# shanghong/Multiband-RF-pulse-Design

Measured on AMD Instinct MI355X. Metric: FIR designs/sec, n=512 taps m=16384 arbitrary-phase SOCP (fir_ap_cvx form), higher is better.
Workload: dtype f64

## Files before the change

### multiband-rf-pulse-design_amd/csrc/solver.hip

```cpp
#include "dev_common.h"
#include <functional>
#include <mutex>
#include <thread>
#include "cone_dev.h"
#include "dd_dev.h"
#include "program.h"
#include "solver.h"
#include <algorithm>
#include <chrono>
#include <cmath>
#include <cstdlib>
#include <cstring>
#include <vector>

#include <dlfcn.h>
#include <rccl/rccl.h>

namespace mbfir {

struct RcclApi {
    ncclResult_t (*GetUniqueId)(ncclUniqueId*) = nullptr;
    ncclResult_t (*CommInitRank)(ncclComm_t*, int, ncclUniqueId, int) = nullptr;
    ncclResult_t (*CommDestroy)(ncclComm_t) = nullptr;
    ncclResult_t (*AllReduce)(const void*, void*, size_t, ncclDataType_t, ncclRedOp_t, ncclComm_t, hipStream_t) = nullptr;
    const char* (*GetErrorString)(ncclResult_t) = nullptr;
    bool ok = false;
    std::string err;
};
static void rccl_bind(RcclApi& api);
static RcclApi& rccl() {
    static RcclApi api;
    static std::once_flag once;
    std::call_once(once, [] { rccl_bind(api); });
    return api;
}
static void rccl_bind(RcclApi& api) {
    void* h = nullptr;
    const char* hinted = std::getenv("MBFIR_RCCL_PATH");
    if (hinted && *hinted) {
        h = dlopen(hinted, RTLD_NOW | RTLD_NOLOAD);
        if (!h) h = dlopen(hinted, RTLD_NOW | RTLD_GLOBAL);
    }
    for (const char* name : {"librccl.so", "librccl.so.1", "/opt/rocm/lib/librccl.so.1"}) {
        if (h) break;
        h = dlopen(name, RTLD_NOW | RTLD_NOLOAD);
    }
    for (const char* name : {"librccl.so", "librccl.so.1", "/opt/rocm/lib/librccl.so.1"}) {
        if (h) break;
        h = dlopen(name, RTLD_NOW | RTLD_GLOBAL);
    }
    if (!h) { api.err = "librccl not found"; return; }
    api.GetUniqueId = reinterpret_cast<decltype(api.GetUniqueId)>(dlsym(h, "ncclGetUniqueId"));
    api.CommInitRank = reinterpret_cast<decltype(api.CommInitRank)>(dlsym(h, "ncclCommInitRank"));
    api.CommDestroy = reinterpret_cast<decltype(api.CommDestroy)>(dlsym(h, "ncclCommDestroy"));
    api.AllReduce = reinterpret_cast<decltype(api.AllReduce)>(dlsym(h, "ncclAllReduce"));
    api.GetErrorString = reinterpret_cast<decltype(api.GetErrorString)>(dlsym(h, "ncclGetErrorString"));
    api.ok = api.GetUniqueId && api.CommInitRank && api.CommDestroy && api.AllReduce;
    if (!api.ok) api.err = "librccl lacks the expected symbols";
}

enum {
    S_TAU = 0, S_KAPPA, S_MU, S_SIGMA, S_ALPHA, S_ALPHA_A, S_DTAU, S_DKAP, S_DTAU_A, S_DKAP_A,
    S_RT, S_PCOST, S_DCOST, S_GAP, S_RELGAP, S_PRES, S_DRES, S_PINF, S_DINF, S_CX, S_HZ, S_SZ,
    S_DEN, S_ETAB, S_NRMH, S_NRMC, S_DEG, S_DKC, S_WB0, S_TMAX, S_BAD,
    S_CHOLFIX ,
    S_TAU0 , S_KAP0,
    S_ALPHA0, S_DTAU_C, S_DKAP_C, S_PICK, S_NCORR, S_NPICK,
    S_RNA = 40 , S_RNB = 49 ,
    S_CG_RZ = 58 , S_CG_ALPHA = 60 , S_CG_BETA = 62 ,
    S_RNC = 64 , S_SIGMAX = 76 , S_COUNT = 80
};
constexpr double STEP = 0.99;
constexpr double SIGMA_MAX = 0.25;
constexpr double SIGMA_MAX_CORR = 0.05;
constexpr double CORR_DELTA = 0.5, CORR_BMIN = 0.1, CORR_BMAX = 10.0, CORR_ACCEPT = 1.01, CORR_ETA = 1.0;
constexpr double POLISH = 1e-2;
constexpr int POLISH_MAX = 3, POLISH_SWEEPS = 1;
constexpr double POLISH_APPROACH = 30.0;
constexpr int NPART = 1024;
constexpr int SCAL_T = 256;
constexpr int MAX_SWEEPS = 8;
enum { KKT_ST_WBZ = 0, KKT_ST_GTWBZ, KKT_ST_HSOLVE, KKT_ST_GDX, KKT_ST_RESID, KKT_ST_START, KKT_ST_GP, KKT_ST_HP, KKT_ST_STEP, KKT_ST_RESTART };
struct KktObserver {
    std::function<void(int, int)> fn;
    bool two_launch_cg = false;
    void operator()(int stage, int sweep) const { fn(stage, sweep); }
};
enum { DD_ST_R1 = 0, DD_ST_R2, DD_ST_WBZ, DD_ST_GTW, DD_ST_RHS, DD_ST_Y, DD_ST_CAPW, DD_ST_ZETAC, DD_ST_SOLVE, DD_ST_GBH, DD_ST_WBZ2, DD_ST_ZETA,
       DD_ST_ACCUM };
static_assert(S_NPICK < S_RNA, "scalar slots: the auto-numbered slots run into S_RNA");
static_assert(S_RNA + MAX_SWEEPS + 1 <= S_RNB && S_RNB + MAX_SWEEPS + 1 <= S_CG_RZ && S_RNC + MAX_SWEEPS + 1 <= S_SIGMAX,
              "scalar slots: a block of residual norms overlaps the next slot");
static_assert(S_SIGMAX < S_COUNT, "scalar slots: S_COUNT too small");
constexpr int CAP_KMAX = 1024;
constexpr int MAX_LANES = 64, MASK_ROWS = MAX_SWEEPS + 4;
constexpr int ROW_BEST = MAX_SWEEPS + 1;
constexpr int ROW_DD = MAX_SWEEPS + 2;
constexpr int ROW_PL = MAX_SWEEPS + 3;
constexpr int WALL_ITERS = 3;
constexpr double REFTOL = 1e-11, REFETA = 1e-1 , INACC_FEAS = 1e-6, INACC_GAP = 1.22e-4 ;

struct LaneDims { int Mf, R, l, nyrows, nfold, nchunk, Nt, N, nq3, big, D1, seg, useg, Mown ; double tmin ; };
static_assert(sizeof(LaneDims) == 64, "LaneDims: 14 ints + one double");
struct DProg {
    int Nt, Ne, N, Mf, R, l, nq3, big, quad;
    int ld, Mpad, LDV, Rp, np;
    int Mown;
    const double *w, *col_tau, *col_scale, *psign, *c;
    const int *col_kind, *pcol;
    const int *freq, *col;
    const double *alpha, *beta, *ey, *h;
    const int *f_ptr, *f_rows;
    const int *c_ptr, *c_rows;
    const int *yrows; int nyrows;
    const int* rep; int own;
    __device__ __forceinline__ double row_weight(int r) const { return (own || !rep[r]) ? 1.0 : 0.0; }
    int trig, D1, LDL, seg, useg, nchunk, LDM;
    double tmin;
    const int *lat;
    const int *lat_col, *lat_qcol;
    const double *lat_scale, *lat_qscale;
    const int *ch_start, *ch_count;
    const int *fold_pos, *fold_neg;
    const double* wf; int nfold;
    int cgrp;
    int seeds_shared;
    const double *ch_w0, *ch_dw;
    const double4* seed_tau;
    const double4* seed_h;
    const double4* seed_eval;
    size_t lane_bytes;
    const int* mask;
    const int* dd_lane;
    const double* dl_plain;
    __device__ __forceinline__ bool plain_weights() const { return dd_lane && !dd_lane[blockIdx.z]; }
    const LaneDims* dims;
    __device__ __forceinline__ void load_dims(int lane) {
        const LaneDims d = dims[lane];
        Mf = d.Mf; R = d.R; l = d.l; nyrows = d.nyrows; nfold = d.nfold; nchunk = d.nchunk;
        Nt = d.Nt; N = d.N; nq3 = d.nq3; big = d.big; D1 = d.D1; seg = d.seg; useg = d.useg; Mown = d.Mown;
        tmin = d.tmin;
    }
    template <class T>
    __device__ __forceinline__ static void sh(const T*& p, size_t off) { p = reinterpret_cast<const T*>(reinterpret_cast<const char*>(p) + off); }
    __device__ __forceinline__ void shift(size_t off) {
        sh(w, off); sh(col_tau, off); sh(col_scale, off); sh(psign, off); sh(c, off); sh(col_kind, off); sh(pcol, off);
        sh(freq, off); sh(col, off); sh(alpha, off); sh(beta, off); sh(ey, off); sh(h, off);
        sh(f_ptr, off); sh(f_rows, off); sh(c_ptr, off); sh(c_rows, off); sh(yrows, off); sh(rep, off);
        sh(lat, off); sh(lat_col, off); sh(lat_qcol, off); sh(lat_scale, off); sh(lat_qscale, off);
        sh(ch_start, off); sh(ch_count, off); sh(ch_w0, off); sh(ch_dw, off); sh(fold_pos, off); sh(fold_neg, off); sh(wf, off);
        if (!seeds_shared) { sh(seed_tau, off); sh(seed_h, off); sh(seed_eval, off); }
        if (dl_plain) sh(dl_plain, off);
    }
};
template <class... Ptr>
__device__ __forceinline__ void lane_shift(size_t off, Ptr&... p) {
    ((p = p ? (Ptr)((const char*)p + off) : p), ...);
}
#define LANES(P, ...)                                                \
    if ((P).mask && !(P).mask[blockIdx.z]) return;                    \
    if ((P).dims) (P).load_dims(blockIdx.z);                          \
    if (blockIdx.z) {                                                 \
        const size_t loff_ = (size_t)blockIdx.z * (P).lane_bytes;     \
        (P).shift(loff_);                                             \
        lane_shift(loff_, __VA_ARGS__);                               \
    }
#define LANES_RAW(lane_bytes, mask, ...)                              \
    if ((mask) && !(mask)[blockIdx.z]) return;                        \
    if (blockIdx.z) lane_shift((size_t)blockIdx.z * (lane_bytes), __VA_ARGS__);
inline dim3 lane_grid(dim3 g, int nlanes) { g.z = nlanes; return g; }

__global__ void k_build_A1(DProg P, double* __restrict__ A1) {
    LANES(P, A1);
    int j = blockIdx.x * blockDim.x + threadIdx.x, i = blockIdx.y;
    if (j >= P.Nt || i >= P.Mf) return;
    double sn, cs;
    sincos(P.w[i] * P.col_tau[j], &sn, &cs);
    A1[(long)i * P.ld + j] = P.col_scale[j] * (P.col_kind[j] ? sn : cs);
}

template <int NV>
__global__ void k_make_xx(DProg P, const double* __restrict__ v, double* __restrict__ XX) {
    LANES(P, v, XX);
    int j = blockIdx.x * blockDim.x + threadIdx.x;
    if (j >= P.Nt) return;
#pragma unroll
    for (int q = 0; q < NV; ++q) {
        double val = v[(long)q * P.LDV + j];
        XX[(long)q * P.LDV + j] = val;
        if (P.quad) XX[(long)(NV + q) * P.LDV + P.pcol[j]] = P.psign[j] * val;
    }
}

template <int NVV>
__global__ __launch_bounds__(256) void k_amulti(const double* __restrict__ A1, int ld, int Mf,
                                                const double* __restrict__ XX, int ldv,
                                                double* __restrict__ UU, int Mpad, size_t lane_bytes, const int* __restrict__ lane_mask,
                                                const LaneDims* __restrict__ dims) {
    LANES_RAW(lane_bytes, lane_mask, A1, XX, UU);
    if (dims) Mf = dims[blockIdx.z].Mf;
    const int lane = threadIdx.x & 63, wv = threadIdx.x >> 6;
    const int row = blockIdx.x * 4 + wv;
    if (row >= Mf) return;
    const double* a = A1 + (long)row * ld;
    double acc[NVV];
#pragma unroll
    for (int v = 0; v < NVV; ++v) acc[v] = 0;
#pragma unroll 8
    for (int j = 2 * lane; j < ld; j += 128) {
        double2 t = *reinterpret_cast<const double2*>(a + j);
#pragma unroll
        for (int v = 0; v < NVV; ++v) {
            double2 xv = *reinterpret_cast<const double2*>(XX + (long)v * ldv + j);
            acc[v] += t.x * xv.x + t.y * xv.y;
        }
    }
#pragma unroll
    for (int v = 0; v < NVV; ++v) {
        double s = wave_sum(acc[v]);
        if (lane == 0) UU[(long)v * Mpad + row] = s;
    }
}

template <int NV>
__device__ __forceinline__ double row_value(const DProg& P, const double* __restrict__ UU, const double* __restrict__ X,
                                            int r, int v) {
    const int f = P.freq[r], cl = P.col[r];
    const double al = P.alpha[r], be = P.beta[r];
    double val = 0;
    if (f >= 0) {
        const int NVV = P.quad ? 2 * NV : NV;
        double u1 = 0, u2 = 0;
        for (int sg = 0; sg < P.useg; ++sg) {
            u1 += UU[((long)sg * NVV + v) * P.Mpad + f];
            if (P.quad) u2 += UU[((long)sg * NVV + NV + v) * P.Mpad + f];
        }
        val = al * u1 + be * u2;
    } else if (cl >= 0) {
        val = al * X[(long)v * P.LDV + cl];
    }
    for (int e = 0; e < P.Ne; ++e) val += P.ey[3 * r + e] * X[(long)v * P.LDV + P.Nt + e];
    return val;
}
template <int NV>
__global__ void k_rows_G(DProg P, const double* __restrict__ UU, const double* __restrict__ X,
                         double* __restrict__ out) {
    LANES(P, UU, X, out);
    int r = blockIdx.x * blockDim.x + threadIdx.x;
    if (r >= P.R) return;
    const int f = P.freq[r], cl = P.col[r];
    const double al = P.alpha[r], be = P.beta[r];
#pragma unroll
    for (int v = 0; v < NV; ++v) {
        double val = 0;
        if (f >= 0) {
            const int NVV = P.quad ? 2 * NV : NV;
            double u1 = 0, u2 = 0;
            for (int sg = 0; sg < P.useg; ++sg) {
                u1 += UU[((long)sg * NVV + v) * P.Mpad + f];
                if (P.quad) u2 += UU[((long)sg * NVV + NV + v) * P.Mpad + f];
            }
            val = al * u1 + be * u2;
        } else if (cl >= 0) {
            val = al * X[(long)v * P.LDV + cl];
        }
        for (int e = 0; e < P.Ne; ++e) val += P.ey[3 * r + e] * X[(long)v * P.LDV + P.Nt + e];
        out[(long)v * P.Rp + r] = val;
    }
}

constexpr int AT_ROWS = 128;
template <int NVV, bool AGG>
__global__ __launch_bounds__(256) void k_atmulti(DProg P, const double* __restrict__ A1, const double* __restrict__ src,
                                                 double* __restrict__ partial) {
    LANES(P, A1, src, partial);
    __shared__ double sh[4][NVV][128];
    __shared__ double pp[NVV][AT_ROWS];
    const int lane = threadIdx.x, wq = threadIdx.y, tid = wq * 64 + lane;
    const int col0 = blockIdx.x * 128 + 2 * lane, split = blockIdx.y;
    const int ld = P.ld, Mpad = P.Mpad;
    const int r0 = split * AT_ROWS, r1 = min(r0 + AT_ROWS, Mpad);
    if (tid < AT_ROWS) {
        const int i = r0 + tid;
        if (AGG) {
            constexpr int NV = NVV;
            const int nv = P.quad ? NVV / 2 : NVV;
            double p1[NV], p2[NV];
#pragma unroll
            for (int v = 0; v < NV; ++v) p1[v] = p2[v] = 0;
            if (i < P.Mf)
                for (int q = P.f_ptr[i]; q < P.f_ptr[i + 1]; ++q) {
                    const int r = P.f_rows[q];
                    const double al = P.alpha[r], be = P.beta[r];
#pragma unroll
                    for (int v = 0; v < NV; ++v)
                        if (v < nv) {
                            const double x = src[(long)v * P.Rp + r];
                            p1[v] += al * x;
                            p2[v] += be * x;
                        }
                }
#pragma unroll
            for (int v = 0; v < NV; ++v)
                if (v < nv) {
                    pp[v][tid] = p1[v];
                    if (P.quad) pp[nv + v][tid] = p2[v];
                }
        } else {
#pragma unroll
            for (int v = 0; v < NVV; ++v) pp[v][tid] = i < Mpad ? src[(long)v * Mpad + i] : 0.0;
        }
    }
    __syncthreads();
    double2 acc[NVV];
#pragma unroll
    for (int v = 0; v < NVV; ++v) acc[v] = make_double2(0, 0);
#pragma unroll 16
    for (int i = r0 + wq; i < r1; i += 4) {
        double2 t = *reinterpret_cast<const double2*>(A1 + (long)i * ld + col0);
#pragma unroll
        for (int v = 0; v < NVV; ++v) {
            const double p = pp[v][i - r0];
            acc[v].x += t.x * p;
            acc[v].y += t.y * p;
        }
    }
#pragma unroll
    for (int v = 0; v < NVV; ++v) {
        sh[wq][v][2 * lane] = acc[v].x;
        sh[wq][v][2 * lane + 1] = acc[v].y;
    }
    __syncthreads();
    for (int e = tid; e < NVV * 128; e += 256) {
        int v = e >> 7, cc = e & 127;
        double t = sh[0][v][cc] + sh[1][v][cc] + sh[2][v][cc] + sh[3][v][cc];
        partial[((long)split * NVV + v) * ld + blockIdx.x * 128 + cc] = t;
    }
}

constexpr int FPC = 16;
__global__ __launch_bounds__(FPC * 16) void k_fold_partials(const double* __restrict__ partial, int nsplit, int nvv, int ld,
                                                        int ldo, double* __restrict__ TT, size_t lane_bytes, const int* lane_mask,
                                                        const LaneDims* __restrict__ dims, int cgrp) {
    LANES_RAW(lane_bytes, lane_mask, partial, TT);
    if (dims) nsplit = cgrp > 0 ? (dims[blockIdx.z].nchunk + cgrp - 1) / cgrp : (dims[blockIdx.z].Mown - cgrp - 1) / -cgrp;
    __shared__ double sh[16][FPC + 1];
    const int c = threadIdx.x, sg = threadIdx.y, j = blockIdx.x * FPC + c, v = blockIdx.y;
    double t = 0;
    if (j < ld) {
        const double* p = partial + (long)v * ld + j;
        const long ss = (long)nvv * ld;
        int s = sg;
        for (; s + 48 < nsplit; s += 64) {
            const double a0 = p[s * ss], a1 = p[(s + 16) * ss], a2 = p[(s + 32) * ss], a3 = p[(s + 48) * ss];
            t += (a0 + a1) + (a2 + a3);
        }
        for (; s < nsplit; s += 16) t += p[s * ss];
    }
    sh[sg][c] = t;
    __syncthreads();
    if (sg == 0 && j < ld) {
        double a = 0;
#pragma unroll
        for (int q = 0; q < 16; ++q) a += sh[q][c];
        TT[(long)v * ldo + j] = a;
    }
}

constexpr int GTC = 32, GTG = 8;
struct GtResid { const double* bx; double* r; double* Sc; int slot; int* cnt; };
template <int NV>
__device__ __forceinline__ void gt_resid_tail(const DProg& P, const GtResid& F, const double* __restrict__ t, double* red) {
    __shared__ int s_last;
    const int tid = threadIdx.y * GTC + threadIdx.x;
    drain_stores();
    __syncthreads();
    if (tid == 0) s_last = __hip_atomic_fetch_add(F.cnt, 1, __ATOMIC_RELAXED, __HIP_MEMORY_SCOPE_AGENT) == (int)gridDim.x - 1;
    __syncthreads();
    if (!s_last) return;
    double m = 0;
    for (int v = 0; v < NV; ++v) {
        double a = 0;
        for (int j = tid; j < P.N; j += GTC * GTG) {
            const long o = (long)v * P.LDV + j;
            const double r = F.bx[o] - __hip_atomic_load(t + o, __ATOMIC_RELAXED, __HIP_MEMORY_SCOPE_AGENT);
            F.r[o] = r;
            a += r * r;
        }
        a = wave_sum(a);
        __syncthreads();
        if ((tid & 63) == 0) red[tid >> 6] = a;
        __syncthreads();
        if (tid == 0) {
            double s = 0;
            for (int w = 0; w < GTC * GTG / 64; ++w) s += red[w];
            red[16] = s;
        }
        __syncthreads();
        m = fmax(m, sqrt(red[16]));
    }
    if (tid == 0) { F.Sc[F.slot] = m; __hip_atomic_store(F.cnt, 0, __ATOMIC_RELAXED, __HIP_MEMORY_SCOPE_AGENT); }
}
template <int NV>
__global__ __launch_bounds__(GTC * GTG) void k_gt_finish(DProg P, const double* __restrict__ partial, int nsplit,
                                                    const double* __restrict__ val, double* __restrict__ out, GtResid F) {
    LANES(P, partial, val, out, F.bx, F.r, F.Sc, F.cnt);
    if (P.dims) nsplit = P.trig ? (P.nchunk + P.cgrp - 1) / P.cgrp : (P.Mown + AT_ROWS - 1) / AT_ROWS;
    __shared__ double sh[2 * NV][GTG][GTC + 1];
    __shared__ double red[17];
    const int c = threadIdx.x, sg = threadIdx.y;
    const int NVV = P.quad ? 2 * NV : NV;
    if ((int)blockIdx.x == (int)gridDim.x - 1) {
        const int tid = sg * GTC + c;
        for (int v = 0; v < NV; ++v)
            for (int e = 0; e < P.Ne; ++e) {
                double a = 0;
                for (int q = tid; q < P.nyrows; q += GTC * GTG) {
                    const int r = P.yrows[q];
                    a += P.row_weight(r) * (P.ey[3 * r + e] * val[(long)v * P.Rp + r]);
                }
                a = wave_sum(a);
                __syncthreads();
                if ((tid & 63) == 0) red[tid >> 6] = a;
                __syncthreads();
                if (tid == 0) {
                    double t = 0;
                    for (int w = 0; w < GTC * GTG / 64; ++w) t += red[w];
                    if (F.bx) __hip_atomic_store(out + (long)v * P.LDV + P.Nt + e, t, __ATOMIC_RELAXED, __HIP_MEMORY_SCOPE_AGENT);
                    else out[(long)v * P.LDV + P.Nt + e] = t;
                }
            }
        if (F.bx) gt_resid_tail<NV>(P, F, out, red);
        return;
    }
    const int j = blockIdx.x * GTC + c;
    const bool ok = j < P.Nt;
    const int pj = (ok && P.quad) ? P.pcol[j] : 0;
    long o1 = j, o2 = pj, st1 = P.ld;
    double f1 = 1.0, f2 = 1.0;
    if (P.trig && ok) {
        o1 = (long)P.col_kind[j] * P.LDM + P.lat[j]; o2 = (long)P.col_kind[pj] * P.LDM + P.lat[pj];
        st1 = 2L * P.LDM;
        f1 = P.col_scale[j]; f2 = P.col_scale[pj];
    }
#pragma unroll
    for (int v = 0; v < NV; ++v) {
        double t1 = 0, t2 = 0;
        if (ok) {
            const double* p1 = partial + (long)v * st1 + o1;
            const double* p2 = partial + (long)(NV + v) * st1 + o2;
            const long ss = (long)NVV * st1;
            int s = sg;
            for (; s + 3 * GTG < nsplit; s += 4 * GTG) {
                const double a0 = p1[s * ss], a1 = p1[(s + GTG) * ss], a2 = p1[(s + 2 * GTG) * ss], a3 = p1[(s + 3 * GTG) * ss];
                t1 += (a0 + a1) + (a2 + a3);
                if (P.quad) {
                    const double b0 = p2[s * ss], b1 = p2[(s + GTG) * ss], b2 = p2[(s + 2 * GTG) * ss], b3 = p2[(s + 3 * GTG) * ss];
                    t2 += (b0 + b1) + (b2 + b3);
                }
            }
            for (; s < nsplit; s += GTG) {
                t1 += p1[s * ss];
                if (P.quad) t2 += p2[s * ss];
            }
        }
        sh[v][sg][c] = f1 * t1;
        sh[NV + v][sg][c] = f2 * t2;
    }
    __syncthreads();
    if (sg == 0 && ok) {
#pragma unroll
        for (int v = 0; v < NV; ++v) {
            double t1 = 0, t2 = 0;
#pragma unroll
            for (int q = 0; q < GTG; ++q) { t1 += sh[v][q][c]; t2 += sh[NV + v][q][c]; }
            double g = t1 + (P.quad ? P.psign[j] * t2 : 0.0);
            if (P.own)
            for (int q = P.c_ptr[j]; q < P.c_ptr[j + 1]; ++q) {
                const int r = P.c_rows[q];
                g += P.alpha[r] * val[(long)v * P.Rp + r];
            }
            if (F.bx) __hip_atomic_store(out + (long)v * P.LDV + j, g, __ATOMIC_RELAXED, __HIP_MEMORY_SCOPE_AGENT);
            else out[(long)v * P.LDV + j] = g;
        }
    }
    if (F.bx) gt_resid_tail<NV>(P, F, out, red);
}

constexpr int CHK = 64;

constexpr int SEGMAX = 128;
template <int NV>
__global__ __launch_bounds__(256) void k_trig_eval(DProg P, const double* __restrict__ vin, double* __restrict__ UU) {
    LANES(P, vin, UU);
    constexpr int NVVMAX = 2 * NV;
    __shared__ double2 cf[NVVMAX][SEGMAX];
    const int k = blockIdx.x * 256 + threadIdx.x, sg = blockIdx.y;
    const int m0 = sg * P.seg, m1 = min(m0 + P.seg, P.D1);
    const int NVV = P.quad ? 2 * NV : NV;
    for (int e = threadIdx.x; e < 2 * (m1 - m0); e += 256) {
        const int kind = e & 1, m = m0 + (e >> 1), le = kind * P.D1 + m;
        const int j = P.lat_col[le], qj = P.quad ? P.lat_qcol[le] : -1;
        const double sc = P.lat_scale[le], qs = P.quad ? P.lat_qscale[le] : 0.0;
#pragma unroll
        for (int q = 0; q < NV; ++q) {
            const double c1 = j >= 0 ? sc * vin[(long)q * P.LDV + j] : 0.0;
            if (kind) cf[q][e >> 1].y = c1; else cf[q][e >> 1].x = c1;
            if (P.quad) {
                const double c2 = qj >= 0 ? qs * vin[(long)q * P.LDV + qj] : 0.0;
                if (kind) cf[NV + q][e >> 1].y = c2; else cf[NV + q][e >> 1].x = c2;
            }
        }
    }
    __syncthreads();
// ... 66 lines not shown
    for (int m0 = 0; m0 < n; m0 += 16) {
        double2 x[NL][NVVMAX];
#pragma unroll
        for (int L = 0; L < NL; ++L)
#pragma unroll
        for (int v = 0; v < NVC; ++v) x[L][v] = cf[L][v][m0 + (threadIdx.x & 15)];
        eval_steps16<NVVMAX, NL, NVC, 0>(x, ac, as, c, s, sd4.z, sd4.w);
    }
}
template <int NVVMAX, int NL, int NVC>
__device__ __forceinline__ void trig_eval_sum(const double2 (*cf)[NVVMAX][SEGMAX], int n, int NVV, const double4 sd4, double (&ac)[NL][NVVMAX], double (&as)[NL][NVVMAX]) {
    double c = sd4.x, s = sd4.y;
    const double cw = sd4.z, sw = sd4.w;
#pragma unroll
    for (int L = 0; L < NL; ++L)
#pragma unroll
    for (int v = 0; v < NVVMAX; ++v) ac[L][v] = as[L][v] = 0;
#pragma unroll (NVVMAX == 2 ? 8 / NL : 8)
    for (int m = 0; m < n; ++m) {
#pragma unroll
        for (int L = 0; L < NL; ++L)
#pragma unroll
        for (int v = 0; v < NVVMAX; ++v)
            if (NVC ? v < NVC : v < NVV) { const double2 x = cf[L][v][m]; ac[L][v] += x.x * c; as[L][v] += x.y * s; }
        rotate<0>(c, s, cw, sw);
    }
}
template <int NV, int NL>
__device__ __forceinline__ void trig_eval_lanes(const DProg& P, const double* const (&vin)[NL], double* const (&UU)[NL], double2 (*cf)[2 * NV][SEGMAX]) {
    constexpr int NVVMAX = 2 * NV;
    const int k = blockIdx.x * 256 + threadIdx.x, sg = blockIdx.y;
    const int m0 = sg * P.seg, m1 = min(m0 + P.seg, P.D1);
    const int NVV = P.quad ? 2 * NV : NV;
    for (int e = threadIdx.x; e < 2 * (m1 - m0); e += 256) {
        const int kind = e & 1, m = m0 + (e >> 1), le = kind * P.D1 + m;
        const int j = P.lat_col[le], qj = P.quad ? P.lat_qcol[le] : -1;
        const double sc = P.lat_scale[le], qs = P.quad ? P.lat_qscale[le] : 0.0;
#pragma unroll
        for (int L = 0; L < NL; ++L)
#pragma unroll
        for (int q = 0; q < NV; ++q) {
            const double c1 = j >= 0 ? sc * vin[L][(long)q * P.LDV + j] : 0.0;
            if (kind) cf[L][q][e >> 1].y = c1; else cf[L][q][e >> 1].x = c1;
            if (P.quad) {
                const double c2 = qj >= 0 ? qs * vin[L][(long)q * P.LDV + qj] : 0.0;
                if (kind) cf[L][NV + q][e >> 1].y = c2; else cf[L][NV + q][e >> 1].x = c2;
            }
        }
    }
    constexpr bool ROWB = NL == 2;
    if (ROWB)
        for (int e = 2 * (m1 - m0) + threadIdx.x; e < 2 * ((m1 - m0 + 15) & ~15); e += 256)
#pragma unroll
            for (int L = 0; L < NL; ++L)
#pragma unroll
            for (int v = 0; v < 2 * NV; ++v) { if (e & 1) cf[L][v][e >> 1].y = 0.0; else cf[L][v][e >> 1].x = 0.0; }
    __syncthreads();
    if ((ROWB ? k - (int)(threadIdx.x & 63) : k) >= P.nfold) return;
    const double4 sd4 = k < P.nfold ? P.seed_eval[(long)sg * P.Mpad + k] : make_double4(0.0, 0.0, 0.0, 0.0);
    double ac[NL][NVVMAX], as[NL][NVVMAX];
    if constexpr (!ROWB) trig_eval_sum<NVVMAX, NL, 0>(cf, m1 - m0, NVV, sd4, ac, as);
    else if (P.quad) trig_eval_sum_rows<NVVMAX, NL, NVVMAX>(cf, m1 - m0, sd4, ac, as);
    else trig_eval_sum_rows<NVVMAX, NL, NV>(cf, m1 - m0, sd4, ac, as);
    if (k >= P.nfold) return;
    const int ip = P.fold_pos[k], in = P.fold_neg[k];
#pragma unroll
    for (int L = 0; L < NL; ++L)
#pragma unroll
    for (int v = 0; v < NVVMAX; ++v)
        if (v < NVV) {
            double* u = UU[L] + ((long)sg * NVV + v) * P.Mpad;
            if (ip >= 0) u[ip] = ac[L][v] + as[L][v];
            if (in >= 0) u[in] = ac[L][v] - as[L][v];
        }
}
template <int NV>
__global__ __launch_bounds__(256, NV == 1 ? 8 : 4) void k_trig_eval_pair(DProg P, const double* __restrict__ vin, double* __restrict__ UU, int nlanes) {
    __shared__ double2 cf[2][2 * NV][SEGMAX];
    bool live[2];
    size_t off0;
    if (!pair_prologue(P, nlanes, live, off0)) return;
    const bool both = live[0] && live[1];
    const size_t off1 = (both || !live[0]) ? P.lane_bytes : 0;
    if (both) {
        const double* const v2[2] = {byte_shift(vin, off0), byte_shift(vin, off0 + off1)};
        double* const u2[2] = {byte_shift(UU, off0), byte_shift(UU, off0 + off1)};
        trig_eval_lanes<NV, 2>(P, v2, u2, cf);
    } else {
        const double* const v1[1] = {byte_shift(vin, off0 + off1)};
        double* const u1[1] = {byte_shift(UU, off0 + off1)};
        trig_eval_lanes<NV, 1>(P, v1, u1, cf);
    }
}

__global__ void k_build_seeds_m(DProg P, double ka, int na, double kb, int nb, double4* __restrict__ seeds) {
    LANES(P, seeds);
    if (P.dims) { na = P.D1; nb = nb ? 2 * P.D1 - 1 : 0; }
    const double t0a = ka * P.tmin, t0b = kb * P.tmin;
    const int m = blockIdx.x * blockDim.x + threadIdx.x, ch = blockIdx.y;
    if (m >= na + nb || ch >= P.nchunk) return;
    const double t = m < na ? t0a + m : t0b + (m - na);
    double s, c, sd, cd;
    sincos(P.ch_w0[ch] * t, &s, &c);
    sincos(P.ch_dw[ch] * t, &sd, &cd);
    seeds[(long)ch * (na + nb) + m] = make_double4(c, s, cd, sd);
}
__global__ void k_build_seeds_e(DProg P, double4* __restrict__ seeds) {
    LANES(P, seeds);
    const int i = blockIdx.x * blockDim.x + threadIdx.x, sg = blockIdx.y;
    if (i >= P.nfold) return;
    const double w = P.wf[i];
    double s, c, sw, cw;
    sincos(w * (P.tmin + sg * P.seg), &s, &c);
    sincos(w, &sw, &cw);
    seeds[(long)sg * P.Mpad + i] = make_double4(c, s, cw, sw);
}

constexpr int CGRP = 4;
constexpr int MPTS = 256;
template <int NV, bool AGG>
__device__ __forceinline__ void freq_operands(const DProg& P, const double* __restrict__ src, int i, double (&out)[NV]) {
#pragma unroll
    for (int v = 0; v < NV; ++v) out[v] = 0;
    if (i < 0) return;
    if (AGG) {
        const int nv = P.quad ? NV / 2 : NV;
        for (int qq = P.f_ptr[i]; qq < P.f_ptr[i + 1]; ++qq) {
            const int r = P.f_rows[qq];
            const double al = P.alpha[r], be = P.beta[r];
#pragma unroll
            for (int v = 0; v < NV; ++v)
                if (v < nv) {
                    const double x = src[(long)v * P.Rp + r];
                    out[v] += al * x;
                    if (P.quad) out[nv + v] += be * x;
                }
        }
    } else {
#pragma unroll
        for (int v = 0; v < NV; ++v) out[v] = src[(long)v * P.Mpad + i];
    }
}
template <int NV, bool AGG>
__global__ __launch_bounds__(256) void k_freq_fold(DProg P, const double* __restrict__ src, double2* __restrict__ out) {
    LANES(P, src, out);
    const int k = blockIdx.x * 256 + threadIdx.x;
    if (k >= P.nfold) return;
    double a[NV], b[NV];
    freq_operands<NV, AGG>(P, src, P.fold_pos[k], a);
    freq_operands<NV, AGG>(P, src, P.fold_neg[k], b);
#pragma unroll
    for (int v = 0; v < NV; ++v) out[(long)v * P.Mpad + k] = make_double2(a[v] + b[v], a[v] - b[v]);
}
template <int NV, bool FOLD = false>
__global__ __launch_bounds__(256) void k_trig_moments(DProg P, const double2* __restrict__ src, const double4* __restrict__ seeds,
                                                      int na, int nb, double* __restrict__ partial, const double* __restrict__ rows = nullptr) {
    if (!P.seeds_shared && blockIdx.z) seeds = reinterpret_cast<const double4*>(reinterpret_cast<const char*>(seeds) + (size_t)blockIdx.z * P.lane_bytes);
    LANES(P, src, partial, rows);
    if (P.dims) { na = P.D1; nb = nb ? 2 * P.D1 - 1 : 0; }
    __shared__ double2 pp[NV][CGRP][CHK];
    const int tid = threadIdx.x;
    const int ch0 = blockIdx.y * P.cgrp;
    for (int e = tid; e < P.cgrp * CHK; e += 256) {
        const int cc = e / CHK, q = e - cc * CHK, ch = ch0 + cc;
        const bool live = ch < P.nchunk && q < P.ch_count[ch < P.nchunk ? ch : 0];
        const int k = live ? P.ch_start[ch] + q : 0;
        if constexpr (FOLD) {
            double a[NV], b[NV];
            freq_operands<NV, true>(P, rows, live ? P.fold_pos[k] : -1, a);
            freq_operands<NV, true>(P, rows, live ? P.fold_neg[k] : -1, b);
#pragma unroll
            for (int v = 0; v < NV; ++v) pp[v][cc][q] = make_double2(a[v] + b[v], a[v] - b[v]);
        } else {
#pragma unroll
        for (int v = 0; v < NV; ++v) pp[v][cc][q] = live ? src[(long)v * P.Mpad + k] : make_double2(0.0, 0.0);
        }
    }
    __syncthreads();
    const int m = blockIdx.x * MPTS + tid;
    if (m >= na + nb) return;
    double ag[NV], as[NV];
#pragma unroll
    for (int v = 0; v < NV; ++v) ag[v] = as[v] = 0;
    for (int cl = 0; cl < P.cgrp; cl += 2) {
        const int cha = ch0 + cl, chb = cha + 1;
        if (cha >= P.nchunk) break;
        const bool two = cl + 1 < P.cgrp && chb < P.nchunk;
        const double4 sa = seeds[(long)cha * (na + nb) + m];
        const double4 sb = two ? seeds[(long)chb * (na + nb) + m] : make_double4(0.0, 0.0, 0.0, 0.0);
        double c0 = sa.x, s0 = sa.y, c1 = sb.x, s1 = sb.y;
        const int cnt = max(P.ch_count[cha], two ? P.ch_count[chb] : 0);
        const int clb = two ? cl + 1 : cl;
#pragma unroll 4
        for (int q = 0; q < cnt; ++q) {
#pragma unroll
            for (int v = 0; v < NV; ++v) {
                const double2 pa = pp[v][cl][q], pb = pp[v][clb][q];
                ag[v] += pa.x * c0; as[v] += pa.y * s0;
                ag[v] += pb.x * c1; as[v] += pb.y * s1;
            }
            const double n0 = c0 * sa.z - s0 * sa.w, n1 = c1 * sb.z - s1 * sb.w;
            s0 = s0 * sa.z + c0 * sa.w; s1 = s1 * sb.z + c1 * sb.w;
            c0 = n0; c1 = n1;
        }
    }
#pragma unroll
    for (int v = 0; v < NV; ++v) {
        partial[(((long)blockIdx.y * NV + v) * 2) * P.LDM + m] = ag[v];
        partial[(((long)blockIdx.y * NV + v) * 2 + 1) * P.LDM + m] = as[v];
    }
}

__device__ __forceinline__ double mul_rounded(double a, double b) {
#pragma clang fp contract(off)
    return a * b;
}
__device__ __forceinline__ double add_rounded(double a, double b) {
#pragma clang fp contract(off)
    return a + b;
}
template <int NV, int NL>
__device__ __forceinline__ void freq_operands_lanes(const DProg* const (&PL)[NL], const double* const (&rows)[NL], int kp, int kn, double (&out)[NL][2][NV]) {
    static_assert(NV <= 2, "freq_operands_lanes: the sums are spelt out for one and two operands");
    constexpr int NS = 2 * NL;
    const bool quad = PL[0]->quad;
    const int nv = quad ? NV / 2 : NV;
    int q0[NS], cnt[NS], nmax = 0;
#pragma unroll
    for (int z = 0; z < NS; ++z) {
        const int i = (z & 1) ? kn : kp;
        const int* fp = PL[z >> 1]->f_ptr;
        q0[z] = i >= 0 ? fp[i] : 0;
        cnt[z] = i >= 0 ? fp[i + 1] - q0[z] : 0;
        nmax = max(nmax, cnt[z]);
#pragma unroll
        for (int v = 0; v < NV; ++v) out[z >> 1][z & 1][v] = 0;
    }
    if (nv == 0) return;
    for (int t = 0; t < nmax; ++t) {
        int r[NS];
#pragma unroll
        for (int z = 0; z < NS; ++z) r[z] = PL[z >> 1]->f_rows[t < cnt[z] ? q0[z] + t : 0];
        double al[NS], be[NS], x[NS][NV];
#pragma unroll
        for (int z = 0; z < NS; ++z) {
            const DProg& Q = *PL[z >> 1];
            al[z] = Q.alpha[r[z]]; be[z] = Q.beta[r[z]];
#pragma unroll
            for (int v = 0; v < NV; ++v) x[z][v] = v < nv ? rows[z >> 1][(long)v * Q.Rp + r[z]] : 0.0;
        }
#pragma unroll
        for (int z = 0; z < NS; ++z) {
            const bool on = t < cnt[z];
            double (&o)[NV] = out[z >> 1][z & 1];
            const double a0 = fma(al[z], x[z][0], o[0]);
            o[0] = on ? a0 : o[0];
            if constexpr (NV == 2) {
                const double p = quad ? mul_rounded(be[z], x[z][0]) : mul_rounded(al[z], x[z][1]);
                const double a1 = add_rounded(o[1], p);
                o[1] = on ? a1 : o[1];
            }
        }
    }
}
template <int NV, int NL, int I>
__device__ __forceinline__ void moment_steps16(const double2 (&pa)[NL][NV], const double2 (&pb)[NL][NV], double (&ag)[NL][NV], double (&as)[NL][NV],
                                               double& c0, double& s0, double& c1, double& s1, const double4& sa, const double4& sb) {
    if constexpr (I < 16) {
#pragma unroll
        for (int L = 0; L < NL; ++L)
#pragma unroll
        for (int v = 0; v < NV; ++v) {
            fmac_row<I>(ag[L][v], pa[L][v].x, c0); fmac_row<I>(as[L][v], pa[L][v].y, s0);
            fmac_row<I>(ag[L][v], pb[L][v].x, c1); fmac_row<I>(as[L][v], pb[L][v].y, s1);
        }
        rotate<1>(c0, s0, sa.z, sa.w);
        rotate<1>(c1, s1, sb.z, sb.w);
        moment_steps16<NV, NL, I + 1>(pa, pb, ag, as, c0, s0, c1, s1, sa, sb);
    }
}
template <int NV, int NL, bool FOLD>
__device__ __forceinline__ void trig_moments_lanes(const DProg& P, const DProg* const (&PL)[NL], const double2* const (&src)[NL], const double4* __restrict__ seeds, int na, int nb,
                                                   double* const (&partial)[NL], const double* const (&rows)[NL], double2 (*pp)[NV][CGRP][CHK]) {
    const int tid = threadIdx.x;
    const int ch0 = blockIdx.y * P.cgrp;
    const int m = blockIdx.x * MPTS + tid;
    const auto seed = [&](int cc) {
        return (m < na + nb && cc < P.cgrp && ch0 + cc < P.nchunk) ? seeds[(long)(ch0 + cc) * (na + nb) + m] : make_double4(0.0, 0.0, 0.0, 0.0);
    };
    double4 sa = seed(0), sb = seed(1);
    for (int e = tid; e < P.cgrp * CHK; e += 256) {
        const int cc = e / CHK, q = e - cc * CHK, ch = ch0 + cc;
        const bool live = ch < P.nchunk && q < P.ch_count[ch < P.nchunk ? ch : 0];
        const int k = live ? P.ch_start[ch] + q : 0;
        if constexpr (FOLD) {
            double ab[NL][2][NV];
            freq_operands_lanes<NV, NL>(PL, rows, live ? P.fold_pos[k] : -1, live ? P.fold_neg[k] : -1, ab);
#pragma unroll
            for (int L = 0; L < NL; ++L)
#pragma unroll
            for (int v = 0; v < NV; ++v) pp[L][v][cc][q] = make_double2(ab[L][0][v] + ab[L][1][v], ab[L][0][v] - ab[L][1][v]);
        } else {
#pragma unroll
            for (int L = 0; L < NL; ++L)
#pragma unroll
            for (int v = 0; v < NV; ++v) pp[L][v][cc][q] = live ? src[L][(long)v * P.Mpad + k] : make_double2(0.0, 0.0);
        }
    }
    __syncthreads();
    constexpr bool ROWB = NV <= 2;
    if ((ROWB ? m - (tid & 63) : m) >= na + nb) return;
    double ag[NL][NV], as[NL][NV];
#pragma unroll
    for (int L = 0; L < NL; ++L)
#pragma unroll
    for (int v = 0; v < NV; ++v) ag[L][v] = as[L][v] = 0;
    for (int cl = 0; cl < P.cgrp; cl += 2) {
        const int cha = ch0 + cl, chb = cha + 1;
        if (cha >= P.nchunk) break;
        const bool two = cl + 1 < P.cgrp && chb < P.nchunk;
        const double4 na4 = seed(cl + 2), nb4 = seed(cl + 3);
        double c0 = sa.x, s0 = sa.y, c1 = sb.x, s1 = sb.y;
        const int cnt = max(P.ch_count[cha], two ? P.ch_count[chb] : 0);
        const int clb = two ? cl + 1 : cl;
        if constexpr (ROWB) {
            for (int q0 = 0; q0 < cnt; q0 += 16) {
                double2 pa[NL][NV], pb[NL][NV];
#pragma unroll
                for (int L = 0; L < NL; ++L)
#pragma unroll
                for (int v = 0; v < NV; ++v) { pa[L][v] = pp[L][v][cl][q0 + (tid & 15)]; pb[L][v] = pp[L][v][clb][q0 + (tid & 15)]; }
                moment_steps16<NV, NL, 0>(pa, pb, ag, as, c0, s0, c1, s1, sa, sb);
            }
        } else {
#pragma unroll (NV * NL > 4 ? 2 : 4)
        for (int q = 0; q < cnt; ++q) {
#pragma unroll
            for (int L = 0; L < NL; ++L)
#pragma unroll
            for (int v = 0; v < NV; ++v) {
                const double2 pa = pp[L][v][cl][q], pb = pp[L][v][clb][q];
                ag[L][v] += pa.x * c0; as[L][v] += pa.y * s0;
                ag[L][v] += pb.x * c1; as[L][v] += pb.y * s1;
            }
            rotate<1>(c0, s0, sa.z, sa.w);
            rotate<1>(c1, s1, sb.z, sb.w);
        }
        }
        sa = na4; sb = nb4;
    }
    if (m >= na + nb) return;
#pragma unroll
    for (int L = 0; L < NL; ++L)
#pragma unroll
    for (int v = 0; v < NV; ++v) {
        partial[L][(((long)blockIdx.y * NV + v) * 2) * P.LDM + m] = ag[L][v];
        partial[L][(((long)blockIdx.y * NV + v) * 2 + 1) * P.LDM + m] = as[L][v];
    }
}
template <int NV, bool FOLD = true>
__global__ __launch_bounds__(256, 4) void k_trig_moments_pair(DProg P, const double2* __restrict__ src, const double4* __restrict__ seeds, int na, int nb,
                                                                       double* __restrict__ partial, const double* __restrict__ rows, int nlanes) {
    static_assert(!FOLD || NV <= 2, "k_trig_moments_pair: G'v of one or two operands");
    __shared__ double2 pp[2][NV][CGRP][CHK];
    bool live[2];
    size_t off0;
    if (!pair_prologue(P, nlanes, live, off0)) return;
    const bool both = live[0] && live[1];
    const size_t off1 = (both || !live[0]) ? P.lane_bytes : 0;
    DProg Q = P;
    Q.shift(off1);
    if (both) {
        const DProg* const p2[2] = {&P, &Q};
        const double2* const s2[2] = {FOLD ? nullptr : byte_shift(src, off0), FOLD ? nullptr : byte_shift(src, off0 + off1)};
        double* const o2[2] = {byte_shift(partial, off0), byte_shift(partial, off0 + off1)};
        const double* const r2[2] = {FOLD ? byte_shift(rows, off0) : nullptr, FOLD ? byte_shift(rows, off0 + off1) : nullptr};
        trig_moments_lanes<NV, 2, FOLD>(P, p2, s2, seeds, na, nb, o2, r2, pp);
    } else {
        const DProg* const p1[1] = {&Q};
        const double2* const s1[1] = {FOLD ? nullptr : byte_shift(src, off0 + off1)};
        double* const o1[1] = {byte_shift(partial, off0 + off1)};
        const double* const r1[1] = {FOLD ? byte_shift(rows, off0 + off1) : nullptr};
        trig_moments_lanes<NV, 1, FOLD>(P, p1, s1, seeds, na, nb, o1, r1, pp);
    }
}

template <int NC>
__device__ __forceinline__ void block_partials(double vals[NC], double* __restrict__ part, bool is_max) {
    __shared__ double sh[17];
#pragma unroll
    for (int c = 0; c < NC; ++c) {
        double s = is_max ? block_max(vals[c], sh) : block_sum(vals[c], sh);
        if (threadIdx.x == 0) part[(long)blockIdx.x * NC + c] = s;
    }
}
__device__ __forceinline__ double fold_partials(const double* part, int nb, int nc, int c, bool is_max, double* sh) {
    double a = is_max ? -1e300 : 0.0;
    for (int b = threadIdx.x; b < nb; b += blockDim.x) {
        double v = part[(long)b * nc + c];
        a = is_max ? fmax(a, v) : a + v;
    }
    return is_max ? block_max(a, sh) : block_sum(a, sh);
}

struct BigW {
    double eta, w0;
};
__device__ __forceinline__ double big_dot(const double* a, const double* b, int n, double* sh) {
    double t = 0;
    for (int i = threadIdx.x; i < n; i += blockDim.x) t += a[i] * b[i];
    return block_sum(t, sh);
}

__global__ __launch_bounds__(1024) void k_big_scaling(DProg P, const double* __restrict__ s,
                                                      const double* __restrict__ z, double* __restrict__ wbb,
                                                      double* __restrict__ lam, double* __restrict__ Sc) {
    LANES(P, s, z, wbb, lam, Sc);
    __shared__ double sh[17];
    const long ob = P.l + 3L * P.nq3;
    s += ob; z += ob; lam += ob;
    const int big = P.big, n1 = big - 1;
    double ns = sqrt(big_dot(s + 1, s + 1, n1, sh)), nz = sqrt(big_dot(z + 1, z + 1, n1, sh));
    double a = sqrt(jres(s[0], ns)), b = sqrt(jres(z[0], nz));
    double sz1 = big_dot(s + 1, z + 1, n1, sh);
    double gamma = sqrt((1.0 + (s[0] * z[0] + sz1) / (a * b)) / 2.0);
    double w0 = (s[0] / a + z[0] / b) / (2 * gamma);
    double eta = sqrt(a / b);
    for (int i = threadIdx.x; i < n1; i += blockDim.x) wbb[1 + i] = (s[1 + i] / a - z[1 + i] / b) / (2 * gamma);
    if (threadIdx.x == 0) { wbb[0] = w0; Sc[S_ETAB] = eta; Sc[S_WB0] = w0; }
    __syncthreads();
    double dot = big_dot(wbb + 1, z + 1, n1, sh);
    double f = z[0] + dot / (1 + w0);
    for (int i = threadIdx.x; i < n1; i += blockDim.x) lam[1 + i] = (z[1 + i] + f * wbb[1 + i]) * eta;
    if (threadIdx.x == 0) lam[0] = (w0 * z[0] + dot) * eta;
}

__device__ __forceinline__ void big_apply(int big, const double* wbb, double eta, const double* u, double* out,
                                          bool inverse, double* sh) {
    const int n1 = big - 1;
    const double w0 = wbb[0], u0 = u[0];
    double dot = big_dot(wbb + 1, u + 1, n1, sh);
    if (inverse) {
        double f = -u0 + dot / (1 + w0);
        for (int i = threadIdx.x; i < n1; i += blockDim.x) out[1 + i] = (u[1 + i] + f * wbb[1 + i]) / eta;
        __syncthreads();
        if (threadIdx.x == 0) out[0] = (w0 * u0 - dot) / eta;
    } else {
        double f = u0 + dot / (1 + w0);
        for (int i = threadIdx.x; i < n1; i += blockDim.x) out[1 + i] = (u[1 + i] + f * wbb[1 + i]) * eta;
        __syncthreads();
        if (threadIdx.x == 0) out[0] = (w0 * u0 + dot) * eta;
    }
    __syncthreads();
}
__device__ __forceinline__ void big_inv2(int big, const double* wbb, double eta, const double* v, const double* sub,
                                         double* out, int mode, double* sh) {
    const int n1 = big - 1;
    const double u0 = wbb[0], e2 = 1.0 / (eta * eta), v0 = v[0];
    double uv = u0 * v0 - big_dot(wbb + 1, v + 1, n1, sh);
    for (int i = threadIdx.x; i < n1; i += blockDim.x) {
        double t = (2 * (-wbb[1 + i]) * uv + v[1 + i]) * e2;
        if (mode == 0) out[1 + i] = t - (sub ? sub[1 + i] : 0.0);
        else out[1 + i] += t;
    }
    __syncthreads();
    if (threadIdx.x == 0) {
        double t = (2 * u0 * uv - v0) * e2;
        if (mode == 0) out[0] = t - (sub ? sub[0] : 0.0);
        else out[0] += t;
    }
    __syncthreads();
}
__device__ __forceinline__ double big_step(int big, const double* lam, const double* d, double* sh) {
    const int n1 = big - 1;
    double nl = sqrt(big_dot(lam + 1, lam + 1, n1, sh));
    double a = sqrt(jres(lam[0], nl));
    double lb0 = lam[0] / a;
    double dot = big_dot(lam + 1, d + 1, n1, sh) / a;
    double rho0 = (lb0 * d[0] - dot) / a;
    double f = -d[0] + dot / (1 + lb0);
    double t = 0;
    for (int i = threadIdx.x; i < n1; i += blockDim.x) {
        double r = (d[1 + i] + f * lam[1 + i] / a) / a;
        t += r * r;
    }
    t = block_sum(t, sh);
    return sqrt(t) - rho0;
}

__global__ void k_scaling(DProg P, const double* __restrict__ s, const double* __restrict__ z,
                          double* __restrict__ dl, double* __restrict__ wl, double* __restrict__ w3,
                          double* __restrict__ lam, const double* __restrict__ bz2, double* __restrict__ wbz2) {
    LANES(P, s, z, dl, wl, w3, lam, bz2, wbz2);
    int t = blockIdx.x * blockDim.x + threadIdx.x;
    if (t < P.l) {
        double sv = s[t], zv = z[t];
        const double dd = zv / sv;
        dl[t] = dd;
        wl[t] = sqrt(sv / zv);
        lam[t] = sqrt(sv * zv);
        if (bz2) { wbz2[t] = dd * bz2[t]; wbz2[P.Rp + t] = dd * bz2[P.Rp + t]; }
    } else if (t < P.l + P.nq3) {
        int c = t - P.l, r = P.l + 3 * c;
        double ss[3] = {s[r], s[r + 1], s[r + 2]}, zz[3] = {z[r], z[r + 1], z[r + 2]}, ll[3];
        Soc3 W = soc3_scaling(ss, zz);
        soc3_apply(W, zz, ll, false);
        w3[4 * c] = W.eta; w3[4 * c + 1] = W.w0; w3[4 * c + 2] = W.w1; w3[4 * c + 3] = W.w2;
        lam[r] = ll[0]; lam[r + 1] = ll[1]; lam[r + 2] = ll[2];
        if (bz2)
            for (int v = 0; v < 2; ++v) {
                const long o = (long)v * P.Rp + r;
                double vv[3] = {bz2[o], bz2[o + 1], bz2[o + 2]}, rr[3];
                soc3_inv2_apply(W, vv, rr);
                wbz2[o] = rr[0]; wbz2[o + 1] = rr[1]; wbz2[o + 2] = rr[2];
            }
    }
}
__device__ __forceinline__ Soc3 load_w3(const double* w3, int c) {
    Soc3 W;
    W.eta = w3[4 * c]; W.w0 = w3[4 * c + 1]; W.w1 = w3[4 * c + 2]; W.w2 = w3[4 * c + 3];
    return W;
}

template <int NV>
__global__ void k_winv2(DProg P, const double* __restrict__ dl, const double* __restrict__ w3,
                        const double* __restrict__ in, const double* __restrict__ sub, double* __restrict__ out,
                        int mode) {
    LANES(P, dl, w3, in, sub, out);
    int t = blockIdx.x * blockDim.x + threadIdx.x;
    if (t < P.l) {
#pragma unroll
        for (int v = 0; v < NV; ++v) {
            long o = (long)v * P.Rp + t;
            double val = dl[t] * in[o];
            if (mode == 0) out[o] = val - (sub ? sub[o] : 0.0);
            else out[o] += val;
        }
    } else if (t < P.l + P.nq3) {
        int c = t - P.l;
        Soc3 W = load_w3(w3, c);
#pragma unroll
        for (int v = 0; v < NV; ++v) {
            long o = (long)v * P.Rp + P.l + 3 * c;
            double vv[3] = {in[o], in[o + 1], in[o + 2]}, rr[3];
            soc3_inv2_apply(W, vv, rr);
            for (int a = 0; a < 3; ++a) {
                if (mode == 0) out[o + a] = rr[a] - (sub ? sub[o + a] : 0.0);
                else out[o + a] += rr[a];
            }
        }
    }
}
template <int NV>
__global__ void k_rows_winv2(DProg P, const double* __restrict__ UU, const double* __restrict__ X,
                             const double* __restrict__ dl, const double* __restrict__ w3,
                             const double* __restrict__ sub, double* __restrict__ gout, double* __restrict__ out) {
    LANES(P, UU, X, dl, w3, sub, gout, out);
    int t = blockIdx.x * blockDim.x + threadIdx.x;
    if (t < P.l) {
#pragma unroll
        for (int v = 0; v < NV; ++v) {
            const long o = (long)v * P.Rp + t;
            const double gv = row_value<NV>(P, UU, X, t, v);
            gout[o] = gv;
            out[o] = dl[t] * gv - (sub ? sub[o] : 0.0);
        }
    } else if (t < P.l + P.nq3) {
        const int c = t - P.l;
        const Soc3 W = load_w3(w3, c);
#pragma unroll
        for (int v = 0; v < NV; ++v) {
            const long o = (long)v * P.Rp + P.l + 3 * c;
            double vv[3], rr[3];
            for (int a = 0; a < 3; ++a) { vv[a] = row_value<NV>(P, UU, X, P.l + 3 * c + a, v); gout[o + a] = vv[a]; }
            soc3_inv2_apply(W, vv, rr);
            for (int a = 0; a < 3; ++a) out[o + a] = rr[a] - (sub ? sub[o + a] : 0.0);
        }
    }
}
template <int NV>
__global__ __launch_bounds__(1024) void k_big_winv2(DProg P, const double* __restrict__ wbb,
                                                    const double* __restrict__ Sc, const double* __restrict__ in,
                                                    const double* __restrict__ sub, double* __restrict__ out, int mode) {
    LANES(P, wbb, Sc, in, sub, out);
    __shared__ double sh[17];
    const long ob = P.l + 3L * P.nq3;
    for (int v = 0; v < NV; ++v) {
        long o = (long)v * P.Rp + ob;
        big_inv2(P.big, wbb, Sc[S_ETAB], in + o, sub ? sub + o : nullptr, out + o, mode, sh);
    }
}

__global__ __launch_bounds__(256) void k_resid_rows(DProg P, const double* __restrict__ Gx, const double* __restrict__ s,
                                                    const double* __restrict__ z, const double* __restrict__ Sc,
                                                    double* __restrict__ rz, double* __restrict__ bz2,
                                                    double* __restrict__ part, const double* __restrict__ UU,
                                                    const double* __restrict__ X) {
    LANES(P, Gx, s, z, Sc, rz, bz2, part, UU, X);
    int r = blockIdx.x * blockDim.x + threadIdx.x;
    double v[4] = {0, 0, 0, 0};
    if (r < P.R) {
        double tau = Sc[S_TAU], gx = UU ? row_value<1>(P, UU, X, r, 0) : Gx[r], sv = s[r], zv = z[r], hv = P.h[r];
        double res = gx + sv - hv * tau;
        rz[r] = res;
        bz2[r] = hv;
        bz2[P.Rp + r] = sv - res;
        const double wr = P.row_weight(r);
        v[0] = wr * (res * res); v[1] = wr * (sv * zv); v[2] = wr * (hv * zv); v[3] = wr * ((gx + sv) * (gx + sv));
    }
    block_partials<4>(v, part, false);
}
__global__ __launch_bounds__(1024) void k_scal_resid(DProg P, double* __restrict__ Sc, const double* __restrict__ GTz,
                                                     const double* __restrict__ x, double* __restrict__ rx,
                                                     double* __restrict__ bx2, const double* __restrict__ partR, int nbR,
                                                     double* __restrict__ RB, int phase, const int* __restrict__ flag) {
    LANES(P, Sc, GTz, x, rx, bx2, partR, RB, flag);
    __shared__ double sh[17];
    double rz2, sz, hz, gxs2;
    if (phase != 1) {
        rz2 = fold_partials(partR, nbR, 4, 0, false, sh);
        sz = fold_partials(partR, nbR, 4, 1, false, sh);
        hz = fold_partials(partR, nbR, 4, 2, false, sh);
        gxs2 = fold_partials(partR, nbR, 4, 3, false, sh);
        if (phase == 0) {
            if (threadIdx.x == 0) { RB[0] = rz2; RB[1] = sz; RB[2] = hz; RB[3] = gxs2; RB[4] = flag ? double(flag[0]) : 0.0; }
            return;
        }
    } else {
        rz2 = RB[0]; sz = RB[1]; hz = RB[2]; gxs2 = RB[3];
    }
    const double tau0 = Sc[S_TAU];
    double a0 = 0, a1 = 0, a2 = 0;
    for (int j = threadIdx.x; j < P.N; j += blockDim.x) {
        double g = GTz[j], cv = P.c[j];
        double res = g + cv * tau0;
        rx[j] = res;
        bx2[j] = -cv;
        bx2[P.LDV + j] = -res;
        a0 += res * res; a1 += cv * x[j]; a2 += g * g;
    }
    double rx2 = block_sum(a0, sh);
    double cx = block_sum(a1, sh);
    double gtz2 = block_sum(a2, sh);
    if (threadIdx.x == 0) {
        double tau = Sc[S_TAU], kap = Sc[S_KAPPA];
        Sc[S_RT] = kap + cx + hz;
        Sc[S_MU] = (sz + kap * tau) / (Sc[S_DEG] + 1.0);
        Sc[S_CX] = cx; Sc[S_HZ] = hz; Sc[S_SZ] = sz;
        double pcost = cx / tau, dcost = -hz / tau, gap = sz / (tau * tau);
        Sc[S_PCOST] = pcost; Sc[S_DCOST] = dcost; Sc[S_GAP] = gap;
        Sc[S_PRES] = sqrt(rz2) / tau / Sc[S_NRMH];
        Sc[S_DRES] = sqrt(rx2) / tau / Sc[S_NRMC];
        double den = fmax(fabs(pcost), fabs(dcost));
        Sc[S_RELGAP] = den > 0 ? gap / den : 1e300;
        Sc[S_PINF] = hz < 0 ? sqrt(gtz2) / (-hz) : 1e300;
        Sc[S_DINF] = cx < 0 ? sqrt(gxs2) / (-cx) : 1e300;
        Sc[S_CHOLFIX] = phase == 1 ? RB[4] : (flag ? double(flag[0]) : 0.0);
    }
}

template <int NV>
__global__ __launch_bounds__(1024) void k_resid_norm(DProg P, const double* __restrict__ bx, const double* __restrict__ t,
                                                     double* __restrict__ out, double* __restrict__ Sc, int slot) {
    LANES(P, bx, t, out, Sc);
    __shared__ double sh[17];
    double m = 0;
    for (int v = 0; v < NV; ++v) {
        double a = 0;
        for (int j = threadIdx.x; j < P.N; j += blockDim.x) {
            long o = (long)v * P.LDV + j;
            double r = bx[o] - t[o];
            out[o] = r;
            a += r * r;
        }
        m = fmax(m, sqrt(block_sum(a, sh)));
    }
    if (threadIdx.x == 0) Sc[slot] = m;
}
template <int NV>
__global__ __launch_bounds__(1024) void k_cg_start(DProg P, double* __restrict__ Sc, const double* __restrict__ r,
                                                   const double* __restrict__ z, double* __restrict__ p, int first) {
    LANES(P, Sc, r, z, p);
    __shared__ double sh[17];
    for (int v = 0; v < NV; ++v) {
        double a = 0;
        for (int j = threadIdx.x; j < P.N; j += blockDim.x) a += r[(long)v * P.LDV + j] * z[(long)v * P.LDV + j];
        const double rz_new = block_sum(a, sh);
        const double rz_old = Sc[S_CG_RZ + v];
        const double beta = first ? 0.0 : (rz_old > 0 ? rz_new / rz_old : 0.0);
        for (int j = threadIdx.x; j < P.N; j += blockDim.x) {
            long o = (long)v * P.LDV + j;
            p[o] = first ? z[o] : z[o] + beta * p[o];
        }
        __syncthreads();
        if (threadIdx.x == 0) Sc[S_CG_RZ + v] = rz_new;
    }
}
template <int NV>
__global__ __launch_bounds__(1024) void k_fold_cg_start(DProg P, double* __restrict__ Sc, const double* __restrict__ r,
                                                        const double* __restrict__ part, double* __restrict__ p, int first) {
    LANES(P, Sc, r, part, p);
    __shared__ double zs[NV][1024];
    __shared__ double sh[17];
    const int t = threadIdx.x;
#pragma unroll
    for (int v = 0; v < NV; ++v) {
        double x[HS_PARTS];
#pragma unroll
        for (int g = 0; g < HS_PARTS; ++g) x[g] = t < P.np ? part[((long)g * NV + v) * P.np + t] : 0.0;
        double s = 0;
#pragma unroll
        for (int g = 0; g < HS_PARTS; ++g) s += x[g];
        zs[v][t] = s;
    }
    __syncthreads();
    const bool act = t < SCAL_T;
    const int lane = t & 63, wv = t >> 6;
    for (int v = 0; v < NV; ++v) {
        double a = 0;
        if (act) for (int j = t; j < P.N; j += SCAL_T) a += r[(long)v * P.LDV + j] * zs[v][j];
        a = wave_sum(a);
        __syncthreads();
        if (act && lane == 0) sh[wv] = a;
        __syncthreads();
        if (t == 0) { double q = 0; for (int i = 0; i < SCAL_T / 64; ++i) q += sh[i]; sh[16] = q; }
        __syncthreads();
        const double rz_new = sh[16];
        const double rz_old = Sc[S_CG_RZ + v];
        const double beta = first ? 0.0 : (rz_old > 0 ? rz_new / rz_old : 0.0);
        if (act) for (int j = t; j < P.N; j += SCAL_T) {
            const long o = (long)v * P.LDV + j;
            p[o] = first ? zs[v][j] : zs[v][j] + beta * p[o];
        }
        __syncthreads();
        if (t == 0) Sc[S_CG_RZ + v] = rz_new;
    }
}
template <int NV>
__global__ __launch_bounds__(1024) void k_cg_step(DProg P, double* __restrict__ Sc, const double* __restrict__ p,
                                                  const double* __restrict__ Hp, double* __restrict__ dx,
                                                  double* __restrict__ r, int slot) {
    LANES(P, Sc, p, Hp, dx, r);
    __shared__ double sh[17];
    double m = 0;
    for (int v = 0; v < NV; ++v) {
        double a = 0;
        for (int j = threadIdx.x; j < P.N; j += blockDim.x) a += p[(long)v * P.LDV + j] * Hp[(long)v * P.LDV + j];
        const double pHp = block_sum(a, sh);
        const double al = pHp > 0 ? Sc[S_CG_RZ + v] / pHp : 0.0;
        double rr2 = 0;
        for (int j = threadIdx.x; j < P.N; j += blockDim.x) {
            long o = (long)v * P.LDV + j;
            dx[o] += al * p[o];
            double rr = r[o] - al * Hp[o];
            r[o] = rr;
            rr2 += rr * rr;
        }
        m = fmax(m, sqrt(block_sum(rr2, sh)));
        if (threadIdx.x == 0) Sc[S_CG_ALPHA + v] = al;
    }
    if (threadIdx.x == 0) Sc[slot] = m;
}
template <int NV>
__global__ void k_cg_update_r(DProg P, const double* __restrict__ Sc, const double* __restrict__ Gp,
                              const double* __restrict__ Wp, double* __restrict__ gdx, double* __restrict__ dz) {
    LANES(P, Sc, Gp, Wp, gdx, dz);
    int t = blockIdx.x * blockDim.x + threadIdx.x;
    if (t >= P.R) return;
#pragma unroll
    for (int q = 0; q < NV; ++q) {
        long o = (long)q * P.Rp + t;
        double al = Sc[S_CG_ALPHA + q];
        gdx[o] += al * Gp[o];
        dz[o] += al * Wp[o];
    }
}
template <int NV>
__global__ __launch_bounds__(256) void k_cg_step_update(DProg P, double* __restrict__ Sc, const double* __restrict__ p,
                                                        const double* __restrict__ Hp, double* __restrict__ dx,
                                                        double* __restrict__ r, int slot, const double* __restrict__ Gp,
                                                        const double* __restrict__ Wp, double* __restrict__ gdx,
                                                        double* __restrict__ dz) {
    LANES(P, Sc, p, Hp, dx, r, Gp, Wp, gdx, dz);
    __shared__ double sh[17];
    double al[NV];
#pragma unroll
    for (int v = 0; v < NV; ++v) {
        double a = 0;
        for (int j = threadIdx.x; j < P.N; j += blockDim.x) a += p[(long)v * P.LDV + j] * Hp[(long)v * P.LDV + j];
        const double pHp = block_sum(a, sh);
        al[v] = pHp > 0 ? Sc[S_CG_RZ + v] / pHp : 0.0;
    }
    const int t = blockIdx.x * blockDim.x + threadIdx.x;
    if (t < P.R) {
#pragma unroll
        for (int q = 0; q < NV; ++q) {
            const long o = (long)q * P.Rp + t;
            gdx[o] += al[q] * Gp[o];
            dz[o] += al[q] * Wp[o];
        }
    }
    if (blockIdx.x != 0) return;
    double m = 0;
#pragma unroll
    for (int v = 0; v < NV; ++v) {
        double rr2 = 0;
        for (int j = threadIdx.x; j < P.N; j += blockDim.x) {
            const long o = (long)v * P.LDV + j;
            dx[o] += al[v] * p[o];
            const double rr = r[o] - al[v] * Hp[o];
            r[o] = rr;
            rr2 += rr * rr;
        }
        m = fmax(m, sqrt(block_sum(rr2, sh)));
        if (threadIdx.x == 0) Sc[S_CG_ALPHA + v] = al[v];
    }
    if (threadIdx.x == 0) Sc[slot] = m;
}
__global__ __launch_bounds__(256) void k_dots_r(DProg P, const double* __restrict__ wl, const double* __restrict__ w3,
                                                const double* __restrict__ z1, const double* __restrict__ z2,
                                                double* __restrict__ part) {
    LANES(P, wl, w3, z1, z2, part);
    int t = blockIdx.x * blockDim.x + threadIdx.x;
    double v[3] = {0, 0, 0};
    if (t < P.l) {
        v[0] = P.h[t] * z1[t]; v[1] = P.h[t] * z2[t];
        double wz = wl[t] * z1[t];
        v[2] = wz * wz;
        if (!P.own && P.rep[t]) v[0] = v[1] = v[2] = 0.0;
    } else if (t < P.l + P.nq3) {
        int c = t - P.l, r = P.l + 3 * c;
        Soc3 W = load_w3(w3, c);
        double zz[3] = {z1[r], z1[r + 1], z1[r + 2]}, wz[3];
        soc3_apply(W, zz, wz, false);
        for (int a = 0; a < 3; ++a) { v[0] += P.h[r + a] * z1[r + a]; v[1] += P.h[r + a] * z2[r + a]; v[2] += wz[a] * wz[a]; }
        if (!P.own && P.rep[r]) v[0] = v[1] = v[2] = 0.0;
    }
    block_partials<3>(v, part + (P.big ? 3 : 0), false);
}
__global__ __launch_bounds__(1024) void k_big_dots(DProg P, const double* __restrict__ wbb, const double* __restrict__ Sc,
                                                   const double* __restrict__ z1, const double* __restrict__ z2,
                                                   double* __restrict__ scratch, double* __restrict__ part_row) {
    LANES(P, wbb, Sc, z1, z2, scratch, part_row);
    __shared__ double sh[17];
    const long ob = P.l + 3L * P.nq3;
    double a = big_dot(P.h + ob, z1 + ob, P.big, sh);
    double b = big_dot(P.h + ob, z2 + ob, P.big, sh);
    big_apply(P.big, wbb, Sc[S_ETAB], z1 + ob, scratch, false, sh);
    double c = big_dot(scratch, scratch, P.big, sh);
    if (threadIdx.x == 0) { const double wo = P.own ? 1.0 : 0.0; part_row[0] = wo * a; part_row[1] = wo * b; part_row[2] = wo * c; }
}

__global__ __launch_bounds__(1024) void k_scal_dtau(DProg P, double* __restrict__ Sc, const double* __restrict__ x1,
                                                    const double* __restrict__ x2, const double* __restrict__ partR,
                                                    int nbR, int mode, double* __restrict__ RB, int phase) {
    LANES(P, Sc, x1, x2, partR, RB);
    __shared__ double sh[17];
    double hz1, hz2, wz1;
    if (phase != 1) {
        hz1 = fold_partials(partR, nbR, 3, 0, false, sh);
        hz2 = fold_partials(partR, nbR, 3, 1, false, sh);
        wz1 = fold_partials(partR, nbR, 3, 2, false, sh);
        if (phase == 0) {
            if (threadIdx.x == 0) { RB[0] = hz1; RB[1] = hz2; RB[2] = wz1; }
            return;
        }
    } else {
        hz1 = RB[0]; hz2 = RB[1]; wz1 = RB[2];
    }
    double a1 = 0, a2 = 0;
    for (int j = threadIdx.x; j < P.N; j += blockDim.x) { a1 += P.c[j] * x1[j]; a2 += P.c[j] * x2[j]; }
    double cx1 = block_sum(a1, sh);
    double cx2 = block_sum(a2, sh);
    if (threadIdx.x == 0) {
        double tau = Sc[S_TAU], kap = Sc[S_KAPPA];
        double den = kap / tau + wz1;
        (void)cx1; (void)hz1;
        if (mode == 0) {
            double dkc = -kap * tau, bt = -Sc[S_RT];
            Sc[S_DTAU_A] = (dkc / tau - bt + cx2 + hz2) / den;
            Sc[S_DKAP_A] = (dkc - kap * Sc[S_DTAU_A]) / tau;
        } else {
            double sigma = Sc[S_SIGMA];
            double dkc = sigma * Sc[S_MU] - kap * tau - Sc[S_DKAP_A] * Sc[S_DTAU_A];
            double bt = -(1 - sigma) * Sc[S_RT];
            const double dt = (dkc / tau - bt + cx2 + hz2) / den;
            Sc[mode == 3 ? S_DTAU_C : S_DTAU] = dt;
            Sc[mode == 3 ? S_DKAP_C : S_DKAP] = (dkc - kap * dt) / tau;
        }
    }
}

__global__ __launch_bounds__(256) void k_dir_post(DProg P, const double* __restrict__ wl, const double* __restrict__ w3,
                                                  const double* __restrict__ lam, const double* __restrict__ z1,
                                                  const double* __restrict__ z2, const double* __restrict__ g1,
                                                  const double* __restrict__ g2, const double* __restrict__ rz,
                                                  double* __restrict__ Sc, double* __restrict__ outA,
                                                  double* __restrict__ outB, double* __restrict__ part, int mode,
                                                  const double* __restrict__ dpart, int ndp, const double* __restrict__ x2) {
    LANES(P, wl, w3, lam, z1, z2, g1, g2, rz, Sc, outA, outB, part, dpart, x2);
    int t = blockIdx.x * blockDim.x + threadIdx.x;
    double dtau;
    if (dpart) {
        __shared__ double sh[17];
        const double hz2 = fold_partials(dpart, ndp, 3, 1, false, sh);
        const double wz1 = fold_partials(dpart, ndp, 3, 2, false, sh);
        double a2 = 0;
        for (int j = threadIdx.x; j < P.N; j += blockDim.x) a2 += P.c[j] * x2[j];
        const double cx2 = block_sum(a2, sh);
        const double tau = Sc[S_TAU], kap = Sc[S_KAPPA], den = kap / tau + wz1;
        double dkc, bt;
        if (mode == 0) { dkc = -kap * tau; bt = -Sc[S_RT]; }
        else {
            const double sigma = Sc[S_SIGMA];
            dkc = sigma * Sc[S_MU] - kap * tau - Sc[S_DKAP_A] * Sc[S_DTAU_A];
            bt = -(1 - sigma) * Sc[S_RT];
        }
        dtau = (dkc / tau - bt + cx2 + hz2) / den;
        if (blockIdx.x == 0 && threadIdx.x == 0) {
            Sc[mode == 0 ? S_DTAU_A : mode == 3 ? S_DTAU_C : S_DTAU] = dtau;
            Sc[mode == 0 ? S_DKAP_A : mode == 3 ? S_DKAP_C : S_DKAP] = (dkc - kap * dtau) / tau;
            if (mode == 1) { Sc[S_TAU0] = tau; Sc[S_KAP0] = kap; }
        }
    } else {
        dtau = mode == 0 ? Sc[S_DTAU_A] : mode == 3 ? Sc[S_DTAU_C] : Sc[S_DTAU];
    }
    const double oms = mode == 0 ? 1.0 : 1.0 - Sc[S_SIGMA];
    double v[2] = {-1e300, -1e300};
    if (t < P.l) {
        double dz = z2[t] + dtau * z1[t], l = lam[t];
        double ds = -oms * rz[t] - g2[t] - dtau * (g1[t] - P.h[t]);
        double wdz = wl[t] * dz, dss = ds / wl[t];
        if (mode == 0) { outA[t] = dss; outB[t] = wdz; } else { outA[t] = ds; outB[t] = dz; }
        v[0] = -dss / l; v[1] = -wdz / l;
    } else if (t < P.l + P.nq3) {
        int c = t - P.l, r = P.l + 3 * c;
        Soc3 W = load_w3(w3, c);
        double dz[3], ds[3], wdz[3], dss[3], ll[3];
        for (int a = 0; a < 3; ++a) {
            dz[a] = z2[r + a] + dtau * z1[r + a];
            ds[a] = -oms * rz[r + a] - g2[r + a] - dtau * (g1[r + a] - P.h[r + a]);
            ll[a] = lam[r + a];
        }
        soc3_apply(W, dz, wdz, false);
        soc3_apply(W, ds, dss, true);
        for (int a = 0; a < 3; ++a) {
            if (mode == 0) { outA[r + a] = dss[a]; outB[r + a] = wdz[a]; } else { outA[r + a] = ds[a]; outB[r + a] = dz[a]; }
        }
        v[0] = soc3_step(ll, dss); v[1] = soc3_step(ll, wdz);
    }
    block_partials<2>(v, part + (P.big ? 2 : 0), true);
}
__global__ __launch_bounds__(1024) void k_big_dir_post(DProg P, const double* __restrict__ wbb, const double* __restrict__ lam,
                                                       const double* __restrict__ z1, const double* __restrict__ z2,
                                                       const double* __restrict__ g1, const double* __restrict__ g2,
                                                       const double* __restrict__ rz, const double* __restrict__ Sc,
                                                       double* __restrict__ outA, double* __restrict__ outB,
                                                       double* __restrict__ scratch, double* __restrict__ part_row, int mode) {
    LANES(P, wbb, lam, z1, z2, g1, g2, rz, Sc, outA, outB, scratch, part_row);
    __shared__ double sh[17];
    const long ob = P.l + 3L * P.nq3;
    const double dtau = mode == 0 ? Sc[S_DTAU_A] : mode == 3 ? Sc[S_DTAU_C] : Sc[S_DTAU];
    const double oms = mode == 0 ? 1.0 : 1.0 - Sc[S_SIGMA];
    double* dzv = scratch;
    double* dsv = scratch + P.big;
    double* wdz = scratch + 2 * P.big;
    double* dss = scratch + 3 * P.big;
    for (int i = threadIdx.x; i < P.big; i += blockDim.x) {
        dzv[i] = z2[ob + i] + dtau * z1[ob + i];
        dsv[i] = -oms * rz[ob + i] - g2[ob + i] - dtau * (g1[ob + i] - P.h[ob + i]);
    }
    __syncthreads();
    big_apply(P.big, wbb, Sc[S_ETAB], dzv, wdz, false, sh);
    big_apply(P.big, wbb, Sc[S_ETAB], dsv, dss, true, sh);
    for (int i = threadIdx.x; i < P.big; i += blockDim.x) {
        if (mode == 0) { outA[ob + i] = dss[i]; outB[ob + i] = wdz[i]; } else { outA[ob + i] = dsv[i]; outB[ob + i] = dzv[i]; }
    }
    __syncthreads();
    double a = big_step(P.big, lam + ob, dss, sh);
    double b = big_step(P.big, lam + ob, wdz, sh);
    if (threadIdx.x == 0) { part_row[0] = a; part_row[1] = b; }
}
__global__ __launch_bounds__(1024) void k_scal_step(DProg P, double* __restrict__ Sc, const double* __restrict__ part, int nb,
                                                    int mode, const double* __restrict__ rx, double* __restrict__ bxc,
                                                    double* __restrict__ RB, int phase) {
    LANES(P, Sc, part, rx, bxc, RB);
    __shared__ double sh[17];
    double ts, tz;
    if (phase != 1) {
        ts = fold_partials(part, nb, 2, 0, true, sh);
        tz = fold_partials(part, nb, 2, 1, true, sh);
        if (phase == 0) {
            if (threadIdx.x == 0) { RB[0] = ts; RB[1] = tz; }
            return;
        }
    } else {
        ts = RB[0]; tz = RB[1];
    }
    if (threadIdx.x == 0) {
        double tau = Sc[S_TAU], kap = Sc[S_KAPPA];
        double dtau = mode == 0 ? Sc[S_DTAU_A] : mode >= 3 ? Sc[S_DTAU_C] : Sc[S_DTAU];
        double dkap = mode == 0 ? Sc[S_DKAP_A] : mode >= 3 ? Sc[S_DKAP_C] : Sc[S_DKAP];
        double t = fmax(0.0, fmax(fmax(ts, tz), fmax(-dtau / tau, -dkap / kap)));
        Sc[S_TMAX] = t;
        if (mode == 0) {
            double a = t == 0.0 ? 1.0 : fmin(1.0, 1.0 / t);
            Sc[S_ALPHA_A] = a;
            Sc[S_SIGMA] = fmin((1 - a) * (1 - a) * (1 - a), Sc[S_SIGMAX]);
            sh[16] = Sc[S_SIGMA];
        } else if (mode == 2) {
            Sc[S_ALPHA0] = t == 0.0 ? 1.0 : fmin(1.0, STEP / t);
        } else {
            double a = t == 0.0 ? 1.0 : fmin(1.0, STEP / t);
            if (mode >= 3) {
                const double a0 = Sc[S_ALPHA0];
                const double tolk = fmax(REFTOL * Sc[S_NRMC], CORR_ETA * Sc[S_DRES] * tau * Sc[S_NRMC]);
                const bool pick = a >= CORR_ACCEPT * a0 && (mode == 4 || Sc[S_RNC] <= tolk);
                Sc[S_PICK] = pick ? 1.0 : 0.0;
                Sc[S_NCORR] += 1.0;
                if (pick) { Sc[S_DTAU] = dtau; Sc[S_DKAP] = dkap; Sc[S_NPICK] += 1.0; }
                else { a = a0; dtau = Sc[S_DTAU]; dkap = Sc[S_DKAP]; }
            }
            Sc[S_ALPHA] = a;
            Sc[S_TAU] = tau + a * dtau;
            Sc[S_KAPPA] = kap + a * dkap;
        }
    }
    if (mode == 0) {
        __syncthreads();
        const double oms = 1.0 - sh[16];
        for (int j = threadIdx.x; j < P.N; j += blockDim.x) bxc[j] = -oms * rx[j];
    }
}

__global__ __launch_bounds__(256) void k_comb_rhs(DProg P, const double* __restrict__ wl, const double* __restrict__ w3,
                           const double* __restrict__ lam, const double* __restrict__ dssa,
                           const double* __restrict__ wdza, const double* __restrict__ rz,
                           double* __restrict__ Sc, double* __restrict__ lds, double* __restrict__ bz,
                           const double* __restrict__ spart, int nsp, const double* __restrict__ rx,
                           double* __restrict__ bxc, const double* __restrict__ dl, double* __restrict__ wbz) {
    LANES(P, wl, w3, lam, dssa, wdza, rz, Sc, lds, bz, spart, rx, bxc, dl, wbz);
    int t = blockIdx.x * blockDim.x + threadIdx.x;
    double sigma;
    if (spart) {
        __shared__ double sh[17];
        const double ts = fold_partials(spart, nsp, 2, 0, true, sh);
        const double tz = fold_partials(spart, nsp, 2, 1, true, sh);
        const double tau = Sc[S_TAU], kap = Sc[S_KAPPA];
        const double tt = fmax(0.0, fmax(fmax(ts, tz), fmax(-Sc[S_DTAU_A] / tau, -Sc[S_DKAP_A] / kap)));
        const double a = tt == 0.0 ? 1.0 : fmin(1.0, 1.0 / tt);
        sigma = fmin((1 - a) * (1 - a) * (1 - a), Sc[S_SIGMAX]);
        if (blockIdx.x == 0) {
            if (threadIdx.x == 0) { Sc[S_TMAX] = tt; Sc[S_ALPHA_A] = a; Sc[S_SIGMA] = sigma; }
            for (int j = threadIdx.x; j < P.N; j += blockDim.x) bxc[j] = -(1.0 - sigma) * rx[j];
        }
    } else {
        sigma = Sc[S_SIGMA];
    }
    const double smu = sigma * Sc[S_MU];
    if (t < P.l) {
        double l = lam[t];
        double dsc = smu - l * l - dssa[t] * wdza[t];
        double q = dsc / l;
        lds[t] = q;
        const double b = -(1 - sigma) * rz[t] - wl[t] * q;
        bz[t] = b;
        if (wbz) wbz[t] = dl[t] * b;
    } else if (t < P.l + P.nq3) {
        int c = t - P.l, r = P.l + 3 * c;
        Soc3 W = load_w3(w3, c);
        double ll[3] = {lam[r], lam[r + 1], lam[r + 2]}, a3[3] = {dssa[r], dssa[r + 1], dssa[r + 2]},
               b3[3] = {wdza[r], wdza[r + 1], wdza[r + 2]}, p1[3], p2[3], dsc[3], q[3], wq[3];
        soc3_prod(ll, ll, p1);
        soc3_prod(a3, b3, p2);
        dsc[0] = smu - p1[0] - p2[0]; dsc[1] = -p1[1] - p2[1]; dsc[2] = -p1[2] - p2[2];
        soc3_div(ll, dsc, q);
        soc3_apply(W, q, wq, false);
        double bb[3], wb[3];
        for (int a = 0; a < 3; ++a) { lds[r + a] = q[a]; bb[a] = -(1 - sigma) * rz[r + a] - wq[a]; bz[r + a] = bb[a]; }
        if (wbz) {
            soc3_inv2_apply(W, bb, wb);
            for (int a = 0; a < 3; ++a) wbz[r + a] = wb[a];
        }
    }
}
__global__ __launch_bounds__(1024) void k_big_comb_rhs(DProg P, const double* __restrict__ wbb, const double* __restrict__ lam,
                                                       const double* __restrict__ dssa, const double* __restrict__ wdza,
                                                       const double* __restrict__ rz, const double* __restrict__ Sc,
                                                       double* __restrict__ lds, double* __restrict__ bz,
                                                       double* __restrict__ scratch) {
    LANES(P, wbb, lam, dssa, wdza, rz, Sc, lds, bz, scratch);
    __shared__ double sh[17];
    const long ob = P.l + 3L * P.nq3;
    const int n1 = P.big - 1;
    const double sigma = Sc[S_SIGMA], smu = sigma * Sc[S_MU];
    const double* L = lam + ob;
    const double* A = dssa + ob;
    const double* B = wdza + ob;
    double ll = big_dot(L, L, P.big, sh), ab = big_dot(A, B, P.big, sh);
    double l0 = L[0], a0 = A[0], b0 = B[0];
    for (int i = threadIdx.x; i < n1; i += blockDim.x)
        scratch[1 + i] = -(2 * l0 * L[1 + i]) - (a0 * B[1 + i] + b0 * A[1 + i]);
    if (threadIdx.x == 0) scratch[0] = smu - ll - ab;
    __syncthreads();
    double nl = sqrt(big_dot(L + 1, L + 1, n1, sh));
    double a = jres(l0, nl);
    double ld = big_dot(L + 1, scratch + 1, n1, sh);
    double q0 = (l0 * scratch[0] - ld) / a;
    for (int i = threadIdx.x; i < n1; i += blockDim.x) lds[ob + 1 + i] = (scratch[1 + i] - q0 * L[1 + i]) / l0;
    if (threadIdx.x == 0) lds[ob] = q0;
    __syncthreads();
    big_apply(P.big, wbb, Sc[S_ETAB], lds + ob, scratch, false, sh);
    for (int i = threadIdx.x; i < P.big; i += blockDim.x) bz[ob + i] = -(1 - sigma) * rz[ob + i] - scratch[i];
}
__global__ __launch_bounds__(256) void k_update(DProg P, double* __restrict__ Sc, const double* __restrict__ x1,
                         const double* __restrict__ x2, double* __restrict__ x, const double* __restrict__ ds,
                         const double* __restrict__ dz, double* __restrict__ s, double* __restrict__ z,
                         const double* __restrict__ part, int nb) {
    LANES(P, Sc, x1, x2, x, ds, dz, s, z, part);
    int t = blockIdx.x * blockDim.x + threadIdx.x;
    if (part) {
        __shared__ double sh[17];
        const double ts = fold_partials(part, nb, 2, 0, true, sh), tz = fold_partials(part, nb, 2, 1, true, sh);
        const double tau = Sc[S_TAU0], kap = Sc[S_KAP0], dtau = Sc[S_DTAU], dkap = Sc[S_DKAP];
        const double tm = fmax(0.0, fmax(fmax(ts, tz), fmax(-dtau / tau, -dkap / kap)));
        const double a = tm == 0.0 ? 1.0 : fmin(1.0, STEP / tm);
        if (blockIdx.x == 0 && threadIdx.x == 0) { Sc[S_TMAX] = tm; Sc[S_ALPHA] = a; Sc[S_TAU] = tau + a * dtau; Sc[S_KAPPA] = kap + a * dkap; }
        if (t < P.N) x[t] += a * (x2[t] + dtau * x1[t]);
        if (t < P.R) { s[t] += a * ds[t]; z[t] += a * dz[t]; }
        return;
    }
    const double a = Sc[S_ALPHA], dtau = Sc[S_DTAU];
    if (t < P.N) x[t] += a * (x2[t] + dtau * x1[t]);
    if (t < P.R) { s[t] += a * ds[t]; z[t] += a * dz[t]; }
}
__global__ __launch_bounds__(256) void k_update_pick(DProg P, const double* __restrict__ Sc, const double* __restrict__ x1,
                         const double* __restrict__ x2, const double* __restrict__ x2k, double* __restrict__ x,
                         const double* __restrict__ ds, const double* __restrict__ dz, const double* __restrict__ dsk,
                         const double* __restrict__ dzk, double* __restrict__ s, double* __restrict__ z) {
    LANES(P, Sc, x1, x2, x2k, x, ds, dz, dsk, dzk, s, z);
    int t = blockIdx.x * blockDim.x + threadIdx.x;
    const double a = Sc[S_ALPHA], dtau = Sc[S_DTAU];
    const bool pick = Sc[S_PICK] != 0.0;
    if (t < P.N) x[t] += a * ((pick ? x2k[t] : x2[t]) + dtau * x1[t]);
    if (t < P.R) { s[t] += a * (pick ? dsk[t] : ds[t]); z[t] += a * (pick ? dzk[t] : dz[t]); }
}
__device__ __forceinline__ void corr_target(double e1, double e2, double mut, double& d1, double& d2) {
    d1 = fmax(fmin(fmax(e1, CORR_BMIN * mut), CORR_BMAX * mut) - e1, -CORR_BMAX * mut);
    d2 = fmax(fmin(fmax(e2, CORR_BMIN * mut), CORR_BMAX * mut) - e2, -CORR_BMAX * mut);
}
__global__ __launch_bounds__(256) void k_corr_rhs(DProg P, const double* __restrict__ wl, const double* __restrict__ dl,
                                                  const double* __restrict__ lam, const double* __restrict__ ds,
                                                  const double* __restrict__ dz, const double* __restrict__ Sc,
                                                  double* __restrict__ bz, double* __restrict__ wbz) {
    LANES(P, wl, dl, lam, ds, dz, Sc, bz, wbz);
    int t = blockIdx.x * blockDim.x + threadIdx.x;
    if (t < P.l) {
        const double at = fmin(1.0, Sc[S_ALPHA0] + CORR_DELTA), mut = Sc[S_SIGMA] * Sc[S_MU];
        const double l = lam[t], w = wl[t];
        const double dss = ds[t] / w, wdz = w * dz[t];
        const double v = (l + at * dss) * (l + at * wdz);
        double tt = fmin(fmax(v, CORR_BMIN * mut), CORR_BMAX * mut) - v;
        tt = fmax(tt, -CORR_BMAX * mut);
        const double b = -w * (tt / l);
        bz[t] = b; wbz[t] = dl[t] * b;
    } else if (t < P.l + P.nq3) {
        const int r = P.l + 3 * (t - P.l);
        for (int a = 0; a < 3; ++a) { bz[r + a] = 0.0; wbz[r + a] = 0.0; }
    }
}
__global__ __launch_bounds__(1024) void k_big_corr_rhs(DProg P, const double* __restrict__ wbb, const double* __restrict__ lam,
                                                       const double* __restrict__ ds, const double* __restrict__ dz,
                                                       const double* __restrict__ Sc, double* __restrict__ bz,
                                                       double* __restrict__ scratch, int on, const int* __restrict__ dd_mask) {
    LANES(P, wbb, lam, ds, dz, Sc, bz, scratch);
    __shared__ double sh[17];
    const long ob = P.l + 3L * P.nq3;
    const int big = P.big, n1 = big - 1;
    if (!on || (dd_mask && dd_mask[blockIdx.z])) {
        for (int i = threadIdx.x; i < big; i += blockDim.x) bz[ob + i] = 0.0;
        return;
    }
    const double at = fmin(1.0, Sc[S_ALPHA0] + CORR_DELTA), mut = Sc[S_SIGMA] * Sc[S_MU];
    const double* L = lam + ob;
    double* u = scratch;
    double* w = scratch + big;
    double* v = scratch + 2 * big;
    double* q = scratch + 3 * big;
    big_apply(big, wbb, Sc[S_ETAB], ds + ob, u, true, sh);
    big_apply(big, wbb, Sc[S_ETAB], dz + ob, w, false, sh);
    for (int i = threadIdx.x; i < big; i += blockDim.x) { u[i] = L[i] + at * u[i]; w[i] = L[i] + at * w[i]; }
    __syncthreads();
    const double v0 = big_dot(u, w, big, sh), u0 = u[0], w0 = w[0];
    for (int i = threadIdx.x; i < n1; i += blockDim.x) v[1 + i] = u0 * w[1 + i] + w0 * u[1 + i];
    __syncthreads();
    const double nv = sqrt(big_dot(v + 1, v + 1, n1, sh));
    double d1, d2;
    corr_target(v0 + nv, v0 - nv, mut, d1, d2);
    const double f = 0.5 * (d1 - d2) / (nv > 0 ? nv : 1.0), t0 = 0.5 * (d1 + d2);
    for (int i = threadIdx.x; i < n1; i += blockDim.x) v[1 + i] *= f;
    __syncthreads();
    const double l0 = L[0], nl = sqrt(big_dot(L + 1, L + 1, n1, sh)), a = jres(l0, nl), ld = big_dot(L + 1, v + 1, n1, sh);
    const double q0 = (l0 * t0 - ld) / a;
    for (int i = threadIdx.x; i < n1; i += blockDim.x) q[1 + i] = (v[1 + i] - q0 * L[1 + i]) / l0;
    if (threadIdx.x == 0) q[0] = q0;
    __syncthreads();
    big_apply(big, wbb, Sc[S_ETAB], q, v, false, sh);
    for (int i = threadIdx.x; i < big; i += blockDim.x) bz[ob + i] = -v[i];
}
__global__ __launch_bounds__(256) void k_corr_add(DProg P, const double* __restrict__ x2, const double* __restrict__ z2,
                                                  const double* __restrict__ g2, double* __restrict__ xk, double* __restrict__ zk,
                                                  double* __restrict__ gk) {
    LANES(P, x2, z2, g2, xk, zk, gk);
    int t = blockIdx.x * blockDim.x + threadIdx.x;
    if (t < P.N) xk[t] = x2[t] + xk[t];
    if (t < P.R) { zk[t] = z2[t] + zk[t]; gk[t] = g2[t] + gk[t]; }
}

__device__ __forceinline__ void load_m3(const double* __restrict__ w3, const double* __restrict__ m3c, int c, double m[6]) {
    if (m3c) { for (int q = 0; q < 6; ++q) m[q] = m3c[6L * c + q]; }
    else soc3_inv2(load_w3(w3, c), m);
}
__device__ __forceinline__ void freq_block_at(const DProg& P, const double* __restrict__ dl, const double* __restrict__ w3,
                                              const double* __restrict__ m3c, int i, double (&v)[9]) {
    double d11 = 0, d12 = 0, d22 = 0, b1[3] = {0, 0, 0}, b2[3] = {0, 0, 0};
    if (i >= 0)
    for (int q = P.f_ptr[i]; q < P.f_ptr[i + 1]; ++q) {
        int r = P.f_rows[q];
        if (r < P.l) {
            double d = dl[r], al = P.alpha[r], be = P.beta[r];
            d11 += d * al * al; d12 += d * al * be; d22 += d * be * be;
            for (int e = 0; e < P.Ne; ++e) { b1[e] += d * al * P.ey[3 * r + e]; b2[e] += d * be * P.ey[3 * r + e]; }
        } else {
            int c = (r - P.l) / 3, a = (r - P.l) - 3 * c;
            if (a != 1) continue;
            int r0 = P.l + 3 * c;
            double m[6];
            load_m3(w3, m3c, c, m);
            double al[3] = {0, P.alpha[r0 + 1], P.alpha[r0 + 2]}, be[3] = {0, P.beta[r0 + 1], P.beta[r0 + 2]};
            for (int p = 1; p < 3; ++p)
                for (int s = 1; s < 3; ++s) {
                    double mm = sym3(m, p, s);
                    d11 += mm * al[p] * al[s]; d12 += mm * al[p] * be[s]; d22 += mm * be[p] * be[s];
                }
            for (int e = 0; e < P.Ne; ++e) {
                for (int p = 1; p < 3; ++p) {
                    double t = 0;
                    for (int s = 0; s < 3; ++s) t += sym3(m, p, s) * P.ey[3 * (r0 + s) + e];
                    b1[e] += al[p] * t; b2[e] += be[p] * t;
                }
            }
        }
    }
    int o = 0;
    v[o++] = d11;
    if (P.quad) { v[o++] = d12; v[o++] = d22; }
    for (int e = 0; e < P.Ne; ++e) v[o++] = b1[e];
    if (P.quad) for (int e = 0; e < P.Ne; ++e) v[o++] = b2[e];
}
__global__ void k_freq_blocks(DProg P, const double* __restrict__ dl, const double* __restrict__ w3,
                              double* __restrict__ Dw, double* __restrict__ BB, const double* __restrict__ m3c) {
    LANES(P, dl, w3, Dw, BB, m3c);
    if (P.plain_weights()) { dl = P.dl_plain; m3c = nullptr; }
    int i = blockIdx.x * blockDim.x + threadIdx.x;
    if (i >= P.Mf) return;
    double v[9];
    freq_block_at(P, dl, w3, m3c, i, v);
    int o = 0;
    Dw[i] = v[o++];
    if (P.quad) { Dw[P.Mpad + i] = v[o++]; Dw[2L * P.Mpad + i] = v[o++]; }
    for (int e = 0; e < P.Ne; ++e) BB[(long)e * P.Mpad + i] = v[o++];
    if (P.quad) for (int e = 0; e < P.Ne; ++e) BB[(long)(P.Ne + e) * P.Mpad + i] = v[o++];
}
__global__ __launch_bounds__(256) void k_freq_blocks_fold(DProg P, const double* __restrict__ dl, const double* __restrict__ w3,
                                                          const double* __restrict__ m3c, int nv, double2* __restrict__ out) {
    LANES(P, dl, w3, m3c, out);
    if (P.plain_weights()) { dl = P.dl_plain; m3c = nullptr; }
    const int k = blockIdx.x * 256 + threadIdx.x;
    if (k >= P.nfold) return;
    double a[9], b[9];
    freq_block_at(P, dl, w3, m3c, P.fold_pos[k], a);
    freq_block_at(P, dl, w3, m3c, P.fold_neg[k], b);
    for (int v = 0; v < nv; ++v) out[(long)v * P.Mpad + k] = make_double2(a[v] + b[v], a[v] - b[v]);
}

__global__ void k_assemble_H(DProg P, const double* __restrict__ T, const double* __restrict__ TT,
                             double* __restrict__ H, double pad_diag) {
    LANES(P, T, TT, H);
    int k = blockIdx.x * blockDim.x + threadIdx.x, j = blockIdx.y;
    if (k >= P.np || j >= P.np) return;
    double v = 0;
    const long ld = P.ld, ld2 = ld * ld;
    if (j < P.Nt && k < P.Nt) {
        v = T[j * ld + k];
        if (P.quad) {
            int pj = P.pcol[j], pk = P.pcol[k];
            double sj = P.psign[j], sk = P.psign[k];
            v += sj * sk * T[2 * ld2 + pj * ld + pk] + sk * T[ld2 + j * ld + pk] + sj * T[ld2 + pj * ld + k];
        }
    } else if (j < P.N && k < P.N) {
        int jj = j < k ? j : k, kk = j < k ? k : j;
        if (jj < P.Nt) {
            int e = kk - P.Nt;
            v = TT[(long)e * P.LDV + jj];
            if (P.quad) v += P.psign[jj] * TT[(long)(P.Ne + e) * P.LDV + P.pcol[jj]];
        }
    } else if (j == k) {
        v = pad_diag;
    }
    H[(long)j * P.np + k] = v;
}
// ... 559 lines not shown
    double *XX, *UU, *PP, *partial, *TT, *TT2, *Dw, *BB, *qv;
    double2* PPf = nullptr;
    double *Mom, *MomB;
    double *tmpN, *tmpN2, *rhsN, *yN, *tmpR, *wbz, *pN, *wpR;
    double *bx2, *bz2, *dx2, *dz2, *gdx2, *gdxc, *xbest, *rx, *rz, *GTz, *Gx;
    double *dssa, *wdza, *lds, *bxc, *bzc, *dxc, *dzc, *ds, *dz, *scratch;
    double *kbx, *kbz, *kx, *kz, *kg, *kds, *kdz;
    SolveSwitches sw;
    bool ar_overlap = false;
    std::vector<GramChunk> gchunks;
    const int* chunk_tab = nullptr;
    double* Tp = nullptr;
    hipStream_t st2 = nullptr;
    std::vector<hipEvent_t> ovev;
    double *partR, *partR2, *partN, *xout, *hout, *sfwork;
    int nbR = 0, nbN = 0, nbC = 0;
    DDev D{};
    double *ddB = nullptr, *ddtS = nullptr, *ddzeta = nullptr, *ddri = nullptr, *ddd0 = nullptr;
    double* ddinv = nullptr;
    int* ddflags = nullptr;
    int dd_epoch = 0;
    bool cap_form = true;
    int dd_passes = 2;
    double *capYt = nullptr, *capZt = nullptr, *capS = nullptr, *capMs = nullptr, *capW1 = nullptr, *capw = nullptr, *capPart = nullptr;
    int* capflag = nullptr;
    int dd_k = 0;

    void ensure_arena(size_t bytes) {
        if (bytes <= ar.cap) { ar.reset(); return; }
        if (ar.base) MBFIR_HIP(hipFree(ar.base));
        ar.base = nullptr; ar.cap = 0;
        if (hipMalloc(&ar.base, bytes) != hipSuccess) {
            (void)hipGetLastError();
            ar.base = nullptr;
            throw ResourceError("arena of " + std::to_string(bytes >> 20) + " MiB not available on the device");
        }
        ar.cap = bytes;
        ar.reset();
    }
    char* stage = nullptr;
    size_t stage_cap = 0, stage_lo = 0, stage_hi = 0;
    size_t meas_lo = 0, meas_hi = 0;
    template <class T, class F>
    T* upload(F get) {
        size_t n0 = 0;
        for (int b = 0; b < nlanes; ++b) n0 = std::max(n0, get(b).size());
        T* p = ar.get<T>(std::max<size_t>(n0, 1));
        const size_t off = size_t(reinterpret_cast<char*>(p) - ar.base), bytes = n0 * sizeof(T);
        if (ar.measuring) {
            if (meas_hi == meas_lo) meas_lo = meas_hi = off;
            meas_hi = std::max(meas_hi, off + std::max<size_t>(bytes, sizeof(T)));
            return p;
        }
        if (stage_hi == stage_lo) {
            stage_lo = stage_hi = off;
            if (off != meas_lo) throw HipError("upload: the layout differs from its measuring pass");
        }
        if (off < stage_hi || off + bytes > meas_hi) throw HipError("upload: arrays out of order");
        pend.push_back({off, bytes, stage_hi, [get](int b, size_t& nb) -> const void* { nb = get(b).size() * sizeof(T); return get(b).data(); }});
        stage_hi = off + bytes;
        return p;
    }
    struct Pend { size_t off, bytes, prev_end; std::function<const void*(int, size_t&)> src; };
    std::vector<Pend> pend;
    void flush_uploads() {
        if (pend.empty()) return;
        const size_t region = meas_hi - meas_lo, need = region * nlanes;
        if (need > stage_cap) {
            if (stage) hipHostFree(stage);
            stage_cap = std::max(need * 2, size_t(1) << 22);
            MBFIR_HIP(hipHostMalloc(reinterpret_cast<void**>(&stage), stage_cap));
        }
        const int nth = need >= (size_t(4) << 20) ? std::min(nlanes, 4) : 1;
        std::vector<hipError_t> rc(nth, hipSuccess);
        auto fill = [&](int t) {
            if (t > 0) rc[t] = hipSetDevice(device);
            for (int b = t; b < nlanes && rc[t] == hipSuccess; b += nth) {
                char* img = stage + region * b;
                for (const Pend& q : pend) {
                    if (q.off > q.prev_end) std::memset(img + (q.prev_end - stage_lo), 0, q.off - q.prev_end);
                    if (q.bytes) {
                        size_t nb = 0;
                        const void* src = q.src(b, nb);
                        if (nb > q.bytes) nb = q.bytes;
                        if (nb) std::memcpy(img + (q.off - stage_lo), src, nb);
                        if (nb < q.bytes) std::memset(img + (q.off - stage_lo) + nb, 0, q.bytes - nb);
                    }
                }
                const size_t filled = stage_hi - stage_lo;
                if (region > filled) std::memset(img + filled, 0, region - filled);
                rc[t] = hipMemcpyAsync(ar.base + stage_lo + (size_t)b * lane_bytes, img, region, hipMemcpyHostToDevice, st);
            }
        };
        std::vector<std::thread> th;
        for (int t = 1; t < nth; ++t) th.emplace_back(fill, t);
        fill(0);
        for (auto& t : th) t.join();
        for (hipError_t e : rc) MBFIR_HIP(e);
        pend.clear();
        stage_lo = stage_hi = 0;
    }
    void memset_lanes(void* p, size_t bytes) {
        if ((bytes & 15) == 0 && (reinterpret_cast<size_t>(p) & 15) == 0 && (lane_bytes & 15) == 0)
            hipLaunchKernelGGL(k_zero_lanes, dim3(std::min<size_t>(2048, cdiv((long)(bytes / 16), 256)), nlanes), dim3(256), 0, st,
                               reinterpret_cast<double2*>(p), bytes / 16, lane_bytes);
        else if (nlanes > 1) hipMemset2DAsync(p, lane_bytes, 0, bytes, nlanes, st);
        else hipMemsetAsync(p, 0, bytes, st);
    }
    void copy_lanes(void* dst, const void* src, size_t bytes) {
        if (nlanes > 1) MBFIR_HIP(hipMemcpy2DAsync(dst, lane_bytes, src, lane_bytes, bytes, nlanes, hipMemcpyDeviceToDevice, st));
        else MBFIR_HIP(hipMemcpyAsync(dst, src, bytes, hipMemcpyDeviceToDevice, st));
    }

    bool lane_pairs() const { return sw.lanepair && nlanes >= 2 && P.seeds_shared && !P.dims && shard_size == 1 && !dd_unit; }
    template <int NV>
    void trig_eval(const double* v) {
        const dim3 g(cdiv(P.nfold, 256), P.useg);
        if (lane_pairs()) {
            ++n_pair;
            hipLaunchKernelGGL(k_trig_eval_pair<NV>, lane_grid(g, cdiv(nlanes, 2)), dim3(256), 0, st, P, v, UU, nlanes);
        } else hipLaunchKernelGGL(k_trig_eval<NV>, lane_grid(g, nlanes), dim3(256), 0, st, P, v, UU);
    }
    template <int NV>
    void apply_G(const double* v, double* out) {
        const int NVV = P.quad ? 2 * NV : NV;
        ++n_gv;
        if (P.trig) {
            trig_eval<NV>(v);
            hipLaunchKernelGGL(k_rows_G<NV>, lane_grid(dim3(cdiv(P.R, 256)), nlanes), dim3(256), 0, st, P, UU, v, out);
            return;
        }
        const double* xx = v;
        if (P.quad) {
            hipLaunchKernelGGL(k_make_xx<NV>, lane_grid(dim3(cdiv(P.Nt, 256)), nlanes), dim3(256), 0, st, P, v, XX);
            xx = XX;
        }
        dim3 g(cdiv(P.Mf, 4));
        if (NVV == 1) hipLaunchKernelGGL(k_amulti<1>, lane_grid(g, nlanes), dim3(256), 0, st, A1, P.ld, P.Mf, xx, P.LDV, UU, P.Mpad, lane_bytes, P.mask, P.dims);
        else if (NVV == 2) hipLaunchKernelGGL(k_amulti<2>, lane_grid(g, nlanes), dim3(256), 0, st, A1, P.ld, P.Mf, xx, P.LDV, UU, P.Mpad, lane_bytes, P.mask, P.dims);
        else hipLaunchKernelGGL(k_amulti<4>, lane_grid(g, nlanes), dim3(256), 0, st, A1, P.ld, P.Mf, xx, P.LDV, UU, P.Mpad, lane_bytes, P.mask, P.dims);
        hipLaunchKernelGGL(k_rows_G<NV>, lane_grid(dim3(cdiv(P.R, 256)), nlanes), dim3(256), 0, st, P, UU, v, out);
    }
    template <int NV>
    void apply_G_winv2(const double* v, double* gout, const double* sub, double* wout) {
        if (P.trig && !P.big) {
            ++n_gv;
            trig_eval<NV>(v);
            hipLaunchKernelGGL(k_rows_winv2<NV>, lane_grid(dim3(cdiv(P.l + P.nq3, 256)), nlanes), dim3(256), 0, st, P, UU, v, dl, w3, sub, gout, wout);
            return;
        }
        apply_G<NV>(v, gout);
        winv2<NV>(gout, sub, wout, 0);
    }
    void moments_array(int nv, const double* pp, const double4* seeds, int na, int nb, double* out) {
        dim3 g(cdiv(na + nb, MPTS), cdiv(P.nchunk, P.cgrp)), b(256), gf(cdiv(P.nfold, 256));
        const bool pair = lane_pairs();
        if (pair) ++n_pair;
        switch (nv) {
#define MOM_CASE(NVX)                                                                                                          \
            case NVX:                                                                                                          \
                if (pp) hipLaunchKernelGGL((k_freq_fold<NVX, false>), lane_grid(gf, nlanes), b, 0, st, P, pp, PPf);            \
                if (pair) hipLaunchKernelGGL((k_trig_moments_pair<NVX, false>), lane_grid(g, cdiv(nlanes, 2)), b, 0, st, P, PPf, seeds, na, nb, partial, (const double*)nullptr, nlanes); \
                else hipLaunchKernelGGL((k_trig_moments<NVX>), lane_grid(g, nlanes), b, 0, st, P, PPf, seeds, na, nb, partial); \
                break;
            MOM_CASE(1) MOM_CASE(2) MOM_CASE(3) MOM_CASE(4) MOM_CASE(6)
#undef MOM_CASE
            default: throw HipError("moments: unsupported vector count");
        }
        hipLaunchKernelGGL(k_fold_partials, lane_grid(dim3(cdiv(P.LDM, FPC), 2 * nv), nlanes), dim3(FPC, 16), 0, st, partial, cdiv(P.nchunk, P.cgrp), 2 * nv, P.LDM, P.LDM, out, lane_bytes, P.mask, P.dims, P.cgrp);
    }
    void atmulti_array(int nvv, const double* pp) {
        dim3 g(P.ld / 128, nsplit_at), b(64, 4);
        switch (nvv) {
            case 1: hipLaunchKernelGGL((k_atmulti<1, false>), lane_grid(g, nlanes), b, 0, st, P, A1, pp, partial); break;
            case 2: hipLaunchKernelGGL((k_atmulti<2, false>), lane_grid(g, nlanes), b, 0, st, P, A1, pp, partial); break;
            case 3: hipLaunchKernelGGL((k_atmulti<3, false>), lane_grid(g, nlanes), b, 0, st, P, A1, pp, partial); break;
            case 4: hipLaunchKernelGGL((k_atmulti<4, false>), lane_grid(g, nlanes), b, 0, st, P, A1, pp, partial); break;
            case 6: hipLaunchKernelGGL((k_atmulti<6, false>), lane_grid(g, nlanes), b, 0, st, P, A1, pp, partial); break;
            default: throw HipError("atmulti: unsupported vector count");
        }
    }
    template <int NV>
    void apply_GT(const double* val, double* out, int tail = 0, const double* rn_bx = nullptr, double* rn_r = nullptr, int rn_slot = 0) {
        ++n_gtv;
        if (P.trig) {
            dim3 g(cdiv(P.D1, MPTS), cdiv(P.nchunk, P.cgrp)), b(256);
            const dim3 gf(cdiv(P.nfold, 256));
            constexpr bool PAIR1 = NV <= 2, PAIR2 = 2 * NV <= 2;
            if (sw.fuse && lane_pairs() && (P.quad ? PAIR2 : PAIR1)) {
                const dim3 g2 = lane_grid(g, cdiv(nlanes, 2));
                ++n_pair;
                if constexpr (PAIR2) if (P.quad) hipLaunchKernelGGL(k_trig_moments_pair<2 * NV>, g2, b, 0, st, P, (const double2*)nullptr, P.seed_tau, P.D1, 0, partial, val, nlanes);
                if constexpr (PAIR1) if (!P.quad) hipLaunchKernelGGL(k_trig_moments_pair<NV>, g2, b, 0, st, P, (const double2*)nullptr, P.seed_tau, P.D1, 0, partial, val, nlanes);
            } else if (sw.fuse) {
                if (P.quad) hipLaunchKernelGGL((k_trig_moments<2 * NV, true>), lane_grid(g, nlanes), b, 0, st, P, (const double2*)nullptr, P.seed_tau, P.D1, 0, partial, val);
                else hipLaunchKernelGGL((k_trig_moments<NV, true>), lane_grid(g, nlanes), b, 0, st, P, (const double2*)nullptr, P.seed_tau, P.D1, 0, partial, val);
            } else if (P.quad) {
                hipLaunchKernelGGL((k_freq_fold<2 * NV, true>), lane_grid(gf, nlanes), b, 0, st, P, val, PPf);
                hipLaunchKernelGGL((k_trig_moments<2 * NV>), lane_grid(g, nlanes), b, 0, st, P, PPf, P.seed_tau, P.D1, 0, partial);
            } else {
                hipLaunchKernelGGL((k_freq_fold<NV, true>), lane_grid(gf, nlanes), b, 0, st, P, val, PPf);
                hipLaunchKernelGGL((k_trig_moments<NV>), lane_grid(g, nlanes), b, 0, st, P, PPf, P.seed_tau, P.D1, 0, partial);
            }
        } else {
            dim3 g(P.ld / 128, nsplit_at), b(64, 4);
            if (P.quad) hipLaunchKernelGGL((k_atmulti<2 * NV, true>), lane_grid(g, nlanes), b, 0, st, P, A1, val, partial);
            else hipLaunchKernelGGL((k_atmulti<NV, true>), lane_grid(g, nlanes), b, 0, st, P, A1, val, partial);
        }
        hipLaunchKernelGGL(k_gt_finish<NV>, lane_grid(dim3(cdiv(P.Nt, GTC) + 1), nlanes), dim3(GTC, GTG), 0, st, P, partial, P.trig ? cdiv(P.nchunk, P.cgrp) : nsplit_at, val, out,
                           GtResid{rn_bx, rn_r, Sc, rn_slot, gt_cnt});
        allreduce(out, (long)NV * P.LDV + tail, 0);
    }
    template <int NV>
    void winv2(const double* in, const double* sub, double* out, int mode) {
        hipLaunchKernelGGL(k_winv2<NV>, lane_grid(dim3(cdiv(P.l + P.nq3, 256)), nlanes), dim3(256), 0, st, P, dl, w3, in, sub, out, mode);
        if (P.big) hipLaunchKernelGGL(k_big_winv2<NV>, lane_grid(dim3(1), nlanes), dim3(1024), 0, st, P, wbb, Sc, in, sub, out, mode);
    }
    bool lead_factor() const { return shard_size > 1 && P.trig; }
    int* gt_cnt = nullptr;
    template <int NV>
    void hsolve(const double* rhs, double* out, const double* rhs2 = nullptr) {
        if (fused_hsolve) {
            hsolve_launch(M, P.np, rhs, rhs2, out, partial, NV, P.LDV, st, nlanes, lane_bytes, P.mask);
        } else {
            trigemv_launch(M, P.np, 0, rhs, yN, NV, P.LDV, st, rhs2, nlanes, lane_bytes, P.mask);
            trigemv_launch(Mt, P.np, 1, yN, out, NV, P.LDV, st, nullptr, nlanes, lane_bytes, P.mask);
        }
    }
    template <int NV>
    void kkt_solve(const double* bx, const double* bz, double* dx, double* dz, double* gdx, int nsweep, int slot,
                   bool wbz_ready = false, const KktObserver* obs = nullptr) {
        const dim3 gR = lane_grid(dim3(cdiv(P.R, 256)), nlanes), g1 = lane_grid(dim3(1), nlanes), b256(256);
        if (!wbz_ready) winv2<NV>(bz, nullptr, wbz, 0);
        else if (P.big) hipLaunchKernelGGL(k_big_winv2<NV>, g1, dim3(1024), 0, st, P, wbb, Sc, bz, nullptr, wbz, 0);
        if (obs) (*obs)(KKT_ST_WBZ, 0);
        apply_GT<NV>(wbz, tmpN);
        if (obs) (*obs)(KKT_ST_GTWBZ, 0);
        hsolve<NV>(bx, dx, tmpN);
        if (obs) (*obs)(KKT_ST_HSOLVE, 0);
        apply_G_winv2<NV>(dx, gdx, wbz, dz);
        if (obs) (*obs)(KKT_ST_GDX, 0);
        double* r = rhsN;
        if (sw.fuse && shard_size <= 1) apply_GT<NV>(dz, tmpN, 0, bx, r, slot);
        else {
        apply_GT<NV>(dz, tmpN);
        hipLaunchKernelGGL(k_resid_norm<NV>, g1, dim3(SCAL_T), 0, st, P, bx, tmpN, r, Sc, slot);
        }
        if (obs) (*obs)(KKT_ST_RESID, 0);
        if (nsweep <= 0) return;
        const int* live = P.mask;
        P.mask = mask_row(1);
        auto z_and_start = [&](int first) {
            if (sw.fuse && fused_hsolve) {
                hsolve_launch(M, P.np, r, nullptr, tmpN2, partial, NV, P.LDV, st, nlanes, lane_bytes, P.mask, false);
                hipLaunchKernelGGL(k_fold_cg_start<NV>, g1, dim3(1024), 0, st, P, Sc, r, partial, pN, first);
            } else {
                hsolve<NV>(r, tmpN2);
                hipLaunchKernelGGL(k_cg_start<NV>, g1, dim3(SCAL_T), 0, st, P, Sc, r, tmpN2, pN, first);
            }
        };
        z_and_start(1);
        if (obs) (*obs)(KKT_ST_START, 0);
        const bool one_launch = shard_size == 1 && !(obs && obs->two_launch_cg);
        for (int it = 0; it < nsweep; ++it) {
            P.mask = mask_row(it + 1);
            apply_G_winv2<NV>(pN, tmpR, nullptr, wpR);
            if (obs) (*obs)(KKT_ST_GP, it);
            apply_GT<NV>(wpR, tmpN);
            if (obs) (*obs)(KKT_ST_HP, it);
            if (one_launch) {
                hipLaunchKernelGGL(k_cg_step_update<NV>, gR, b256, 0, st, P, Sc, pN, tmpN, dx, r, slot + it + 1, tmpR, wpR, gdx, dz);
            } else {
                hipLaunchKernelGGL(k_cg_step<NV>, g1, dim3(SCAL_T), 0, st, P, Sc, pN, tmpN, dx, r, slot + it + 1);
                hipLaunchKernelGGL(k_cg_update_r<NV>, gR, b256, 0, st, P, Sc, tmpR, wpR, gdx, dz);
            }
            if (obs) (*obs)(KKT_ST_STEP, it);
            if (it + 1 < nsweep) { P.mask = mask_row(it + 2); z_and_start(0); if (obs) (*obs)(KKT_ST_RESTART, it); }
        }
        P.mask = live;
    }
    int dd_prep_launch() {
        hipLaunchKernelGGL(k_dd_prep, lane_grid(dim3(std::max(nbC, 1)), nlanes), dim3(256), 0, st, P, dl, w3, D, partR);
        if (P.big) hipLaunchKernelGGL(k_dd_prep_big, lane_grid(dim3(1), nlanes), dim3(1024), 0, st, P, wbb, Sc, D, partR);
        return std::max(nbC, 1) + (P.big ? 1 : 0);
    }
    int dd_prepare_lanes(const double theta0, int* ks, const bool* live) {
        const int nb = std::max(nbC, 1), nbp = dd_prep_launch();
        for (int b = 0; b < nlanes; ++b) hostTheta[b] = theta0;
        const int kmax_fit = cap_form ? CAP_KMAX : DD_KMAX;
        for (int attempt = 0; attempt < 8; ++attempt) {
            if (attempt > 0) memset_lanes(D.kcnt, sizeof(int));
            MBFIR_HIP(hipMemcpyAsync(ddtheta, hostTheta, sizeof(double) * nlanes, hipMemcpyHostToDevice, st));
            hipLaunchKernelGGL(k_dd_select, lane_grid(dim3(nb), nlanes), dim3(256), 0, st, P, dl, D, partR, nbp, theta0, (const double*)ddtheta);
            hipLaunchKernelGGL(k_dd_order, lane_grid(dim3(1), nlanes), dim3(1024), 0, st, P, D);
            MBFIR_HIP(hipMemcpy2DAsync(hostFlag + MAX_LANES, sizeof(int), D.kcnt, lane_bytes, sizeof(int), nlanes, hipMemcpyDeviceToHost, st));
            MBFIR_HIP(hipStreamSynchronize(st));
            bool fits = true;
            int kmax = 0;
            for (int b = 0; b < nlanes; ++b) {
                ks[b] = live[b] ? hostFlag[MAX_LANES + b] : 0;
                if (ks[b] > kmax_fit) { fits = false; hostTheta[b] *= 100.0; }
                kmax = std::max(kmax, ks[b]);
            }
            dd_attempts = attempt + 1;
            if (fits) return kmax;
        }
        throw HipError("extended-precision solve: strong set does not fit");
    }
    double hostTheta[MAX_LANES];
    int dd_attempts = 0;
    double* ddtheta = nullptr;
    bool dd_unit = false;
    int dd_kp = 0;
    int dd_prepare(double theta) {
        const int nb = std::max(nbC, 1), nbp = dd_prep_launch();
        for (int attempt = 0; attempt < 8; ++attempt) {
            if (attempt > 0) hipMemsetAsync(D.kcnt, 0, sizeof(int), st);
            hipLaunchKernelGGL(k_dd_select, lane_grid(dim3(nb), nlanes), dim3(256), 0, st, P, dl, D, partR, nbp, theta, (const double*)nullptr);
            hipLaunchKernelGGL(k_dd_order, dim3(1), dim3(1024), 0, st, P, D);
            MBFIR_HIP(hipMemcpyAsync(hostFlag + 1, D.kcnt, sizeof(int), hipMemcpyDeviceToHost, st));
            MBFIR_HIP(hipStreamSynchronize(st));
            hostTheta[0] = theta; dd_attempts = attempt + 1;
            if (hostFlag[1] <= (cap_form ? CAP_KMAX : DD_KMAX)) return hostFlag[1];
            theta *= 100.0;
        }
        throw HipError("extended-precision solve: strong set does not fit");
    }
    template <int NV>
    void kkt_solve_dd(const double* bx, const double* bz, double* dx, double* dz, double* gdx, int slot, const KktObserver* obs = nullptr) {
        const dim3 gC(std::max(nbC, 1)), b256(256);
        const int k = dd_unit ? dd_kp : dd_k;
        const int* kcnt = dd_unit ? D.kcnt : nullptr;
        double *Bh = ddB, *Bl = ddB + 2L * P.LDV;
        hipLaunchKernelGGL(k_zero3, lane_grid(dim3(cdiv(NV * std::max<long>(P.LDV, P.Rp), 256)), nlanes), dim3(256), 0, st, dx, long(NV) * P.LDV, dz, long(NV) * P.Rp, gdx, long(NV) * P.Rp,
                           lane_bytes, P.mask);
        for (int it = 0; it < dd_passes; ++it) {
            apply_GT<NV>(dz, tmpN);
            hipLaunchKernelGGL(k_resid_norm<NV>, lane_grid(dim3(1), nlanes), dim3(SCAL_T), 0, st, P, bx, tmpN, rhsN, Sc, slot + it);
            if (obs) (*obs)(DD_ST_R1, it);
            hipLaunchKernelGGL(k_dd_r2<NV>, lane_grid(gC, nlanes), b256, 0, st, P, D, dl, bz, gdx, dz, tmpR, ddtS);
            if (P.big) hipLaunchKernelGGL(k_dd_r2_big<NV>, lane_grid(dim3(1), nlanes), dim3(1024), 0, st, P, D, bz, gdx, dz, tmpR, ddtS, scratch);
            if (obs) (*obs)(DD_ST_R2, it);
            hipLaunchKernelGGL(k_dd_winv2c<NV>, lane_grid(gC, nlanes), b256, 0, st, P, D, tmpR, (const double*)nullptr, wbz);
            if (P.big) hipLaunchKernelGGL(k_dd_winv2c_big<NV>, lane_grid(dim3(1), nlanes), dim3(1024), 0, st, P, D, tmpR, (const double*)nullptr, wbz, scratch);
            if (obs) (*obs)(DD_ST_WBZ, it);
            apply_GT<NV>(wbz, tmpN2);
            if (obs) (*obs)(DD_ST_GTW, it);
            if (cap_form) {
                int kp = int(round_up(k, 64));
                if (!dd_unit) kp = std::max(kp, sw.test_cap_kp);
                cap_add_launch(rhsN, tmpN2, Bl, P.N, P.np, P.LDV, NV, st, nlanes, lane_bytes, P.mask);
                if (obs) (*obs)(DD_ST_RHS, it);
                double* yv = tmpN2;
                hsolve<NV>(Bl, yv);
                if (obs) (*obs)(DD_ST_Y, it);
                cap_uy_launch(D.U, k, kp, P.N, P.np, yv, P.LDV, ddtS, capw, DD_KMAX, NV, st, nlanes, lane_bytes, P.mask, kcnt);
                if (obs) (*obs)(DD_ST_CAPW, it);
                hsolve_launch(capMs, kp, capw, nullptr, ddzeta, partial, NV, DD_KMAX, st, nlanes, lane_bytes, P.mask);
                if (obs) (*obs)(DD_ST_ZETAC, it);
                cap_dx_launch(capZt, k, P.N, P.np, ddzeta, DD_KMAX, yv, Bh, P.LDV, NV, st, nlanes, lane_bytes, P.mask, kcnt);
            } else {
            hipLaunchKernelGGL(k_dd_rhs<NV>, lane_grid(dim3(cdiv(P.np, 16)), nlanes), b256, 0, st, P, D, k, rhsN, tmpN2, ddtS, Bh, Bl);
            if (obs) (*obs)(DD_ST_RHS, it);
            dd_trsv_launch(H, M, Mt, W1, ddri, ddri + P.np, P.np, Bh, Bl, NV, P.LDV, st, ddflags, ++dd_epoch, flag, ddinv);
            }
            if (obs) (*obs)(DD_ST_SOLVE, it);
            apply_G<NV>(Bh, wpR);
            if (obs) (*obs)(DD_ST_GBH, it);
            hipLaunchKernelGGL(k_dd_winv2c<NV>, lane_grid(gC, nlanes), b256, 0, st, P, D, wpR, tmpR, wbz);
            if (P.big) hipLaunchKernelGGL(k_dd_winv2c_big<NV>, lane_grid(dim3(1), nlanes), dim3(1024), 0, st, P, D, wpR, tmpR, wbz, scratch);
            if (obs) (*obs)(DD_ST_WBZ2, it);
            if (!cap_form) hipLaunchKernelGGL(k_dd_zeta<NV>, lane_grid(dim3(k), nlanes), dim3(64), 0, st, P, D, Bh, Bl, ddtS, ddzeta);
            if (obs && !cap_form) (*obs)(DD_ST_ZETA, it);
            hipLaunchKernelGGL(k_dd_accum<NV>, lane_grid(gC, nlanes), b256, 0, st, P, D, wbz, wpR, ddzeta, dz, gdx);
            if (P.big) hipLaunchKernelGGL(k_dd_accum_big<NV>, lane_grid(dim3(1), nlanes), dim3(1024), 0, st, P, D, wbz, wpR, ddzeta, dz, gdx);
            hipLaunchKernelGGL(k_dd_accum_x<NV>, lane_grid(dim3(nbN), nlanes), b256, 0, st, P, Bh, dx);
            if (obs) (*obs)(DD_ST_ACCUM, it);
        }
    }
    bool timing = true;
    std::vector<hipEvent_t> evpool;
    size_t evused = 0;
    std::vector<hipEvent_t> capev;
    size_t capev_used = 0;
    double cap_flop_sum = 0;
    hipEvent_t next_cap_event() {
        if (capev_used == capev.size()) {
            hipEvent_t e;
            MBFIR_HIP(hipEventCreate(&e));
            capev.push_back(e);
        }
        return capev[capev_used++];
    }
    hipEvent_t next_event() {
        if (evused == evpool.size()) {
            hipEvent_t e;
            MBFIR_HIP(hipEventCreate(&e));
            evpool.push_back(e);
        }
        return evpool[evused++];
    }
    double* H_keep = nullptr;
    bool h_one_pass = false;
    double* capS_keep = nullptr;
    void build_H(int ddk = 0) {
        double* yy_sum = nullptr;
        const double* dlw = ddk > 0 ? D.dlc : dl;
        const double* m3c = ddk > 0 ? D.m3c : nullptr;
        const int* live_mask = P.mask;
        P.dd_lane = (dd_unit && ddk > 0) ? mask_row(ROW_DD) : nullptr;
        P.dl_plain = P.dd_lane ? dl : nullptr;
        const int nwv = P.quad ? 3 : 1, nvb = P.quad ? 2 * P.Ne : P.Ne;
        const bool one_pass = P.trig && P.Ne > 0 && P.tmin == 0.0 && nwv + nvb <= 4;
        h_one_pass = one_pass;
        if (!one_pass) hipLaunchKernelGGL(k_freq_blocks, lane_grid(dim3(cdiv(P.Mf, 256)), nlanes), dim3(256), 0, st, P, dlw, w3, Dw, BB, m3c);
        hipEvent_t g0 = timing ? next_event() : nullptr, g1 = timing ? next_event() : nullptr;
        if (P.trig) {
            if (g0) hipEventRecord(g0, st);
            const double* momb = MomB;
            if (one_pass) {
                hipLaunchKernelGGL(k_freq_blocks_fold, lane_grid(dim3(cdiv(P.nfold, 256)), nlanes), dim3(256), 0, st, P, dlw, w3, m3c, nwv + nvb, PPf);
                moments_array(nwv + nvb, nullptr, P.seed_h, P.D1, 2 * P.D1 - 1, Mom);
                momb = Mom + 2L * nwv * P.LDM;
            } else {
                moments_array(nwv, Dw, P.seed_h, P.D1, 2 * P.D1 - 1, Mom);
                if (P.Ne > 0) moments_array(nvb, BB, P.seed_tau, P.D1, 0, MomB);
            }
            if (lead_factor()) {
                yy_sum = nullptr;
                if (momb == MomB) {
                    allreduce(Mom, 2L * nwv * P.LDM, 0);
                    if (P.Ne > 0) allreduce(MomB, 2L * nvb * P.LDM, 0);
                } else {
                    long cnt = 2L * (nwv + nvb) * P.LDM;
                    if (P.Ne > 0 && cnt + 16 <= 18L * P.LDM) {
                        yy_sum = Mom + cnt;
                        hipMemsetAsync(yy_sum, 0, sizeof(double) * 9, st);
                        if (P.nyrows > 0) hipLaunchKernelGGL(k_H_yy, lane_grid(dim3(1), nlanes), dim3(256), 0, st, P, dlw, w3, yy_sum, 3L, 0L, m3c);
                        cnt += 9;
                    }
                    allreduce(Mom, cnt, 0);
                }
            }
            hipLaunchKernelGGL(k_assemble_H_lat, lane_grid(dim3((P.np / 64) * (P.np / 64 + 1) / 2, 16), nlanes), dim3(256), 0, st, P, Mom, momb, H, 1.0);
            if (g1) hipEventRecord(g1, st);
        } else {
        if (ar_overlap) {
            if (g0) hipEventRecord(g0, st);
            if (!st2) MBFIR_HIP(hipStreamCreateWithFlags(&st2, hipStreamNonBlocking));
            while (ovev.size() < 2 * gchunks.size()) { hipEvent_t e; MBFIR_HIP(hipEventCreateWithFlags(&e, hipEventDisableTiming)); ovev.push_back(e); }
            for (size_t c = 0; c < gchunks.size(); ++c) {
                const GramChunk& ck = gchunks[c];
                gram_chunk_launch(gps[0], ck, A1, Dw, slab, tile_ij, chunk_tab, Tp, st);
                if (shard_size > 1) {
                    MBFIR_HIP(hipEventRecord(ovev[2 * c], st));
                    MBFIR_HIP(hipStreamWaitEvent(st2, ovev[2 * c], 0));
                    allreduce(Tp + (size_t)ck.plo * 16384, (long)(ck.phi - ck.plo) * 16384, 0, st2);
                    MBFIR_HIP(hipEventRecord(ovev[2 * c + 1], st2));
                }
            }
            if (g1) hipEventRecord(g1, st);
        } else if (nlanes == 1) gram_launch(gps[0], A1, Dw, slab, T, tile_ij, st, g0, g1, P.Mpad);
        else {
        if (g0) hipEventRecord(g0, st);
        for (int b = 0; b < nlanes; ++b) {
            if (nlanes > 1 && !lane_live[b]) continue;
            const size_t off = (size_t)b * lane_bytes;
            auto at = [&](double* p) { return reinterpret_cast<double*>(reinterpret_cast<char*>(p) + off); };
            gram_launch(gps[b], at(A1), at(Dw), at(slab), at(T), reinterpret_cast<const int*>(reinterpret_cast<const char*>(tile_ij) + off), st, nullptr, nullptr, P.Mpad);
        }
        if (g1) hipEventRecord(g1, st);
        }
        if (P.Ne > 0) {
            int nvv = P.quad ? 2 * P.Ne : P.Ne;
            atmulti_array(nvv, BB);
            hipLaunchKernelGGL(k_fold_partials, lane_grid(dim3(cdiv(P.ld, FPC), nvv), nlanes), dim3(FPC, 16), 0, st, partial, nsplit_at, nvv, P.ld, P.LDV, TT, lane_bytes, P.mask, P.dims, -AT_ROWS);
        }
        if (ar_overlap) {
            if (P.Ne > 0) {
                yy_sum = TT + (size_t)P.Ne * P.LDV;
                hipMemsetAsync(yy_sum, 0, sizeof(double) * 9, st);
                if (P.nyrows > 0) hipLaunchKernelGGL(k_H_yy, lane_grid(dim3(1), nlanes), dim3(256), 0, st, P, dlw, w3, yy_sum, 3L, 0L, m3c);
            }
            if (shard_size > 1) {
                MBFIR_HIP(hipStreamWaitEvent(st, ovev[2 * gchunks.size() - 1], 0));
                if (P.Ne > 0) allreduce(TT, (long)P.Ne * P.LDV + 9, 0);
            }
            gram_unpack_launch(gps[0], Tp, tile_ij, chunk_tab, T, st);
        }
        hipLaunchKernelGGL(k_assemble_H, lane_grid(dim3(cdiv(P.np, 256), P.np), nlanes), dim3(256), 0, st, P, T, TT, H, (ar_overlap || shard_rank == 0) ? 1.0 : 0.0);
        }
        const bool summed = shard_size > 1 && !lead_factor() && !ar_overlap;
        if (ar_overlap && P.Ne > 0) hipLaunchKernelGGL(k_H_yy_add, lane_grid(dim3(1), nlanes), dim3(16), 0, st, P, yy_sum, H);
        if (lead_factor() && P.Ne > 0) {
            const double* yy = yy_sum;
            if (!yy) {
                hipMemsetAsync(RB, 0, sizeof(double) * 9, st);
                if (P.nyrows > 0) hipLaunchKernelGGL(k_H_yy, lane_grid(dim3(1), nlanes), dim3(256), 0, st, P, dlw, w3, RB, 3L, 0L, m3c);
                allreduce(RB, 9, 0);
                yy = RB;
            }
            hipLaunchKernelGGL(k_H_yy_add, lane_grid(dim3(1), nlanes), dim3(16), 0, st, P, yy, H);
        }
        {
            const int yy_too = (!lead_factor() && !ar_overlap && P.Ne > 0 && P.nyrows > 0) ? 1 : 0;
            hipLaunchKernelGGL(k_H_identity, lane_grid(dim3(cdiv(P.Nt, 256) + yy_too), nlanes), dim3(256), 0, st, P, dlw, w3, H, m3c, yy_too, summed ? 1 : 0);
            if (P.big && (!summed || shard_rank == 0)) {
                memset_lanes(qv, sizeof(double) * 3 * P.LDV);
                if (ddk > 0) {
                    if (dd_unit) P.mask = mask_row(ROW_DD);
                    hipLaunchKernelGGL(k_big_q_dd, lane_grid(dim3(cdiv(P.big, 256)), nlanes), dim3(256), 0, st, P, D, qv, qv + P.LDV, qv + 2L * P.LDV);
                    hipLaunchKernelGGL(k_H_big_dd, lane_grid(dim3(cdiv(P.N, 256), P.N), nlanes), dim3(256), 0, st, P, D, qv, qv + P.LDV, qv + 2L * P.LDV, H);
                }
                if (ddk <= 0 || dd_unit) {
                    if (dd_unit && ddk > 0) P.mask = mask_row(ROW_PL);
                    hipLaunchKernelGGL(k_big_q, lane_grid(dim3(cdiv(P.big, 256)), nlanes), dim3(256), 0, st, P, wbb, qv, qv + P.LDV);
                    hipLaunchKernelGGL(k_H_big, lane_grid(dim3(cdiv(P.N, 256), P.N), nlanes), dim3(256), 0, st, P, qv, qv + P.LDV, Sc, H);
                }
                P.mask = live_mask;
            }
        }
        if (!lead_factor() && !ar_overlap && shard_size > 1) {
            const long nb = P.np / 64, ntile = nb * (nb + 1) / 2;
            hipLaunchKernelGGL(k_pack_tril, dim3((unsigned)ntile), dim3(256), 0, st, H, P.np, M, 0);
            const int chunks = int(std::min<long>(sw.ar_chunks > 0 ? sw.ar_chunks : 4, ntile));
            for (int c = 0; c < chunks; ++c) {
                const long lo = ntile * c / chunks, hi = ntile * (c + 1) / chunks;
                allreduce(M + lo * 4096, (hi - lo) * 4096, 0);
            }
            hipLaunchKernelGGL(k_pack_tril, dim3((unsigned)ntile), dim3(256), 0, st, H, P.np, M, 1);
        }
        if (H_keep) MBFIR_HIP(hipMemcpy2DAsync(H_keep, sizeof(double) * P.np * P.np, H, nlanes > 1 ? lane_bytes : sizeof(double) * P.np * P.np,
                                               sizeof(double) * P.np * P.np, nlanes, hipMemcpyDeviceToDevice, st));
        hipEvent_t c0 = timing ? next_event() : nullptr, c1 = timing ? next_event() : nullptr;
        P.dd_lane = nullptr; P.dl_plain = nullptr;
        if (ddk > 0 && cap_form) {
            const int kp = dd_unit ? dd_kp : std::max(int(round_up(ddk, 64)), sw.test_cap_kp);
            const size_t lb = dd_unit ? lane_bytes : 0;
            const int* mdd = mask_row(ROW_DD);
            chol_launch_count += chol_inv_launch(H, M, fused_hsolve ? nullptr : Mt, W1, P.np, flag, st, sw.chol_split, sw.poison, nullptr, c0, nullptr, nlanes, lb, P.mask);
            P.mask = mdd;
            hipLaunchKernelGGL(k_dd_rows, lane_grid(dim3(kp), nlanes), dim3(256), 0, st, P, D, P.np, dd_unit ? -1 : ddk);
            P.mask = live_mask;
            hipEvent_t b0 = timing ? next_cap_event() : nullptr, b1 = timing ? next_cap_event() : nullptr;
            if (b0) hipEventRecord(b0, st);
            cap_build_launch(D.U, dd_unit ? kp : ddk, kp, P.np, M, D.sX, capYt, capZt, capS, capPart, st, nlanes, lb, mdd, dd_unit ? D.kcnt : nullptr);
            if (b1) hipEventRecord(b1, st);
            if (capS_keep) MBFIR_HIP(hipMemcpy2DAsync(capS_keep, sizeof(double) * kp * kp, capS, nlanes > 1 ? lane_bytes : sizeof(double) * kp * kp,
                                                      sizeof(double) * kp * kp, nlanes, hipMemcpyDeviceToDevice, st));
            cap_flop_sum += 2.0 * (double(kp) * P.np * P.np + 0.5 * double(kp) * kp * P.np);
            chol_inv_launch(capS, capMs, nullptr, capW1, kp, capflag, st, sw.chol_split, sw.poison, nullptr, nullptr, c1, nlanes, lb, mdd);
            cap_flag_add_launch(flag, capflag, st, nlanes, lb, mdd);
        } else if (ddk > 0) {
            if (c0) hipEventRecord(c0, st);
            hipLaunchKernelGGL(k_dd_rows, lane_grid(dim3(ddk), nlanes), dim3(256), 0, st, P, D, P.np, ddk);
            dd_syrk_launch(D.U, P.np, D.sX, D.kcnt, P.np, H, M, st);
            dd_chol_launch(H, M, Mt, W1, ddri, ddri + P.np, ddd0, P.np, DD_PIVTOL, flag, st, ddinv);
            if (c1) hipEventRecord(c1, st);
        } else {
            chol_launch_count += chol_inv_launch(H, M, fused_hsolve ? nullptr : Mt, W1, P.np, flag, st, sw.chol_split, sw.poison, nullptr, c0, c1, nlanes, lane_bytes, P.mask);
        }
    }
    void prepare_lanes(const std::vector<const TrigProgram*>& Qs, const SolveOpts& o, std::vector<LaneHost>& LH) {
        shard_rank = o.shard_size > 1 ? o.shard_rank : 0;
        shard_size = o.shard_size > 1 ? o.shard_size : 1;
        if (shard_size > 1 && !ar_fn && !comm) throw HipError("row-sharded solve without a communicator or an all-reduce hook");
        if (comm && shard_size > 1 && (comm_size != shard_size || comm_rank != shard_rank))
            throw HipError("row-sharded solve: shard_rank / shard_size differ from the RCCL communicator's");
        n_collectives = 0; collective_bytes = 0;
        n_gv = 0; n_gtv = 0; n_pair = 0;
        if (shard_size > 1 && nlanes > 1) throw ShapeError("row-sharded solves run one design at a time");
        for (int b = 0; b < nlanes; ++b) {
            LaneHost& L = LH[b];
            const TrigProgram& Qfull = *Qs[b];
            if (shard_size > 1) { L.local = shard_program(Qfull, shard_rank, shard_size); L.Q = &L.local; }
// ... 174 lines not shown
            D.kcnt = ar.get<int>(1); D.skind = ar.get<int>(DD_KMAX); D.sidx = ar.get<int>(DD_KMAX); D.sdir = ar.get<int>(DD_KMAX);
            ddtheta = ar.get<double>(MAX_LANES);
            D.sX = ar.get<double>(DD_KMAX); D.U = ar.get<double>((size_t)DD_KMAX * np);
            ddB = ar.get<double>(4 * LDV); ddtS = ar.get<double>(2 * (size_t)DD_KMAX); ddzeta = ar.get<double>(2 * (size_t)DD_KMAX);
            ddri = ar.get<double>(2 * np); ddd0 = ar.get<double>(np);
            ddflags = ar.get<int>(2 * np / 32 + 8);
            ddinv = ar.get<double>(2 * np * 64);
            if (!sw.dd_blockinv) ddinv = nullptr;
            if (cap_form) {
                capYt = ar.get<double>((size_t)CAP_KMAX * np); capZt = ar.get<double>((size_t)CAP_KMAX * np);
                capS = ar.get<double>((size_t)CAP_KMAX * CAP_KMAX); capMs = ar.get<double>((size_t)CAP_KMAX * CAP_KMAX);
                capW1 = ar.get<double>((size_t)CAP_KMAX * CAP_KMAX + 65 * (size_t)CAP_KMAX); capw = ar.get<double>(2 * (size_t)DD_KMAX);
                capflag = ar.get<int>(4);
                capPart = ar.get<double>(cap_part_doubles(CAP_KMAX, int(np)));
            }
        }
        hout = ar.get<double>(2 * (size_t)U.n_max + 8);
        sfwork = ar.get<double>(6 * (size_t)std::max(U.lp, 1));
        zero_bytes = size_t(ar.base + ar.off - zero_from);
        slab = ar.get<double>(P.trig ? 0 : gp.slab_doubles);
        };
        ar.measuring = true; ar.reset(); meas_lo = meas_hi = 0;
        { char* keep = ar.base; ar.base = nullptr; place(); ar.base = keep; }
        lane_bytes = (ar.off + 4095) & ~size_t(4095); ar.measuring = false;
        ensure_arena(lane_bytes * nlanes + 4096);
        pend.clear(); stage_lo = stage_hi = 0;
        place();
        P.lane_bytes = lane_bytes;
        memset_lanes(zero_from, zero_bytes);
    }
    std::vector<int> mask_dev, mask_new;
    void push_masks(const std::vector<LaneHost>& LH) {
        if (nlanes == 1) return;
        for (int b = 0; b < nlanes; ++b) {
            mask_new[b] = LH[b].live ? 1 : 0;
            lane_live[b] = LH[b].live;
            for (int q = 1; q <= MAX_SWEEPS; ++q) mask_new[q * MAX_LANES + b] = (LH[b].live && LH[b].dd_k == 0 && LH[b].nsweep >= q) ? 1 : 0;
            mask_new[ROW_DD * MAX_LANES + b] = (LH[b].live && LH[b].dd_k > 0) ? 1 : 0;
            mask_new[ROW_PL * MAX_LANES + b] = (LH[b].live && LH[b].dd_k == 0) ? 1 : 0;
        }
        auto send = [&](size_t off, size_t ints) {
            if (std::memcmp(mask_new.data() + off, mask_dev.data() + off, sizeof(int) * ints) == 0) return;
            std::memcpy(hostMask + off, mask_new.data() + off, sizeof(int) * ints);
            MBFIR_HIP(hipMemcpyAsync(maskT + off, hostMask + off, sizeof(int) * ints, hipMemcpyHostToDevice, st));
            std::memcpy(mask_dev.data() + off, mask_new.data() + off, sizeof(int) * ints);
        };
        send(0, size_t(MAX_SWEEPS + 1) * MAX_LANES);
        if (dd_unit) send(size_t(ROW_DD) * MAX_LANES, 2 * size_t(MAX_LANES));
    }
    void start_lanes(const std::vector<LaneHost>& LH) {
        if (!P.trig) hipLaunchKernelGGL(k_build_A1, lane_grid(dim3(cdiv(P.Nt, 256), P.Mf), nlanes), dim3(256), 0, st, P, A1);
        else {
            const int seed_lanes = P.seeds_shared ? 1 : nlanes;
            hipLaunchKernelGGL(k_build_seeds_m, lane_grid(dim3(cdiv(P.D1, 256), P.nchunk), seed_lanes), dim3(256), 0, st, P, 1.0, P.D1, 0.0, 0,
                               const_cast<double4*>(P.seed_tau));
            hipLaunchKernelGGL(k_build_seeds_m, lane_grid(dim3(cdiv(3 * P.D1 - 1, 256), P.nchunk), seed_lanes), dim3(256), 0, st, P, 0.0, P.D1, 2.0,
                               2 * P.D1 - 1, const_cast<double4*>(P.seed_h));
            hipLaunchKernelGGL(k_build_seeds_e, lane_grid(dim3(cdiv(P.nfold, 256), P.useg), seed_lanes), dim3(256), 0, st, P, const_cast<double4*>(P.seed_eval));
        }
        std::vector<double> sc0((size_t)S_COUNT * nlanes, 0.0);
        for (int b = 0; b < nlanes; ++b) {
            double* q = sc0.data() + (size_t)b * S_COUNT;
            q[S_NRMH] = LH[b].nrm_h; q[S_NRMC] = LH[b].nrm_c; q[S_DEG] = LH[b].degree; q[S_TAU] = 1.0; q[S_KAPPA] = 1.0;
            q[S_SIGMAX] = (sw.corrector && LH[b].Q->l > 0 && LH[b].Q->big == 0) ? SIGMA_MAX_CORR : SIGMA_MAX;
            MBFIR_HIP(hipMemcpyAsync(reinterpret_cast<char*>(Sc) + (size_t)b * lane_bytes, q, sizeof(double) * S_COUNT, hipMemcpyHostToDevice, st));
        }
    }
    UnitPlan setup_unit(const std::vector<const TrigProgram*>& Qs, const SolveOpts& o, std::vector<LaneHost>& LH) {
        nlanes = int(Qs.size());
        sw = read_switches();
        chol_set_lose_step(sw.test_lose_flag, st);
        prepare_lanes(Qs, o, LH);
        const UnitPlan U = plan_unit(LH, o);
        layout_arena(LH, U);
        mask_dev.assign(size_t(MASK_ROWS) * MAX_LANES, -1); mask_new.assign(size_t(MASK_ROWS) * MAX_LANES, 0);
        push_masks(LH);
        P.mask = mask_row(0);
        start_lanes(LH);
        return U;
    }
    void cone_shift(double* v) {
        const int nb = std::max(nbC, 1);
        hipLaunchKernelGGL(k_cone_resid, lane_grid(dim3(nb), nlanes), dim3(256), 0, st, P, v, partR);
        if (P.big) hipLaunchKernelGGL(k_big_cone_resid, lane_grid(dim3(1), nlanes), dim3(1024), 0, st, P, v, partR);
        hipLaunchKernelGGL(k_cone_fold, lane_grid(dim3(1), nlanes), dim3(256), 0, st, partR, nb + (P.big ? 1 : 0), RB, lane_bytes, P.mask);
        allreduce(RB, 1, 1);
        allreduce(RB + 1, 1, 0);
        hipLaunchKernelGGL(k_cone_shift, lane_grid(dim3(64), nlanes), dim3(256), 0, st, P, v, RB);
    }
    void initial_point(int nsweep, const KktObserver* obs = nullptr) {
        hipLaunchKernelGGL(k_unit_scaling, lane_grid(dim3(cdiv(std::max(std::max(P.l, P.nq3), std::max(P.big, 1)), 256)), nlanes), dim3(256), 0, st,
                           P, dl, wl, w3, wbb, Sc);
        build_H();
        hipLaunchKernelGGL(k_init_rhs, lane_grid(dim3(cdiv(std::max(P.N, P.R), 256)), nlanes), dim3(256), 0, st, P, bx2, bz2);
        kkt_solve<2>(bx2, bz2, dx2, dz2, gdx2, nsweep, S_RNA, false, obs);
        copy_lanes(x, dx2, sizeof(double) * P.LDV);
        hipLaunchKernelGGL(k_neg_copy_r, lane_grid(dim3(cdiv(P.R, 256)), nlanes), dim3(256), 0, st, P, dz2, s, -1.0);
        cone_shift(s);
        hipLaunchKernelGGL(k_neg_copy_r, lane_grid(dim3(cdiv(P.R, 256)), nlanes), dim3(256), 0, st, P, dz2 + P.Rp, z, 1.0);
        cone_shift(z);
    }
    void launch_residuals(int two = -1) {
        const bool sharded = two_phase(two);
        double* rmail = sharded ? GTz + P.LDV : RB;
        if (P.trig) {
            ++n_gv;
            trig_eval<1>(x);
            hipLaunchKernelGGL(k_resid_rows, lane_grid(dim3(nbR), nlanes), dim3(256), 0, st, P, nullptr, s, z, Sc, rz, bz2, partR, UU, x);
        } else {
            apply_G<1>(x, Gx);
            hipLaunchKernelGGL(k_resid_rows, lane_grid(dim3(nbR), nlanes), dim3(256), 0, st, P, Gx, s, z, Sc, rz, bz2, partR, nullptr, nullptr);
        }
        if (sharded) hipLaunchKernelGGL(k_scal_resid, lane_grid(dim3(1), nlanes), dim3(SCAL_T), 0, st, P, Sc, GTz, x, rx, bx2, partR, nbR, rmail, 0, (const int*)flag);
        apply_GT<1>(z, GTz, sharded ? 5 : 0);
        hipLaunchKernelGGL(k_scal_resid, lane_grid(dim3(1), nlanes), dim3(SCAL_T), 0, st, P, Sc, GTz, x, rx, bx2, partR, nbR, rmail, sharded ? 1 : 2, (const int*)flag);
    }
    void launch_scaling() {
        hipLaunchKernelGGL(k_scaling, lane_grid(dim3(std::max(nbC, 1)), nlanes), dim3(256), 0, st, P, s, z, dl, wl, w3, lam, bz2, wbz);
        if (P.big) hipLaunchKernelGGL(k_big_scaling, lane_grid(dim3(1), nlanes), dim3(1024), 0, st, P, s, z, wbb, lam, Sc);
    }
    void launch_head(std::vector<LaneHost>& LH, const SolveOpts& o) {
        launch_scaling();
        int ks[MAX_LANES];
        if (dd_unit) {
            bool lv[MAX_LANES];
            for (int b = 0; b < nlanes; ++b) lv[b] = LH[b].live;
            dd_k = dd_prepare_lanes(o.ddkkt_theta, ks, lv);
            dd_kp = int(round_up(std::max(dd_k, 1), 64));
        } else {
            ks[0] = dd_k = (o.ddkkt_theta > 0 && shard_size <= 1) ? dd_prepare(o.ddkkt_theta) : 0;
        }
        for (int b = 0; b < (dd_unit ? nlanes : 1); ++b) {
            LH[b].dd_k = ks[b];
            if (ks[b] > 0) { LH[b].dd_iters += 1; LH[b].dd_kmax = std::max(LH[b].dd_kmax, ks[b]); }
        }
        if (dd_unit) push_masks(LH);
        build_H(dd_k);
    }
    template <int NV>
    void solve_modes(bool dd_any, bool pl_any, const double* bx, const double* bz, double* dx, double* dz, double* gdx, int slot, int nsweep,
                     const KktObserver* dd_obs = nullptr) {
        const int* live_row = P.mask;
        if (dd_any) {
            if (dd_unit) P.mask = mask_row(ROW_DD);
            kkt_solve_dd<NV>(bx, bz, dx, dz, gdx, slot, dd_obs);
        }
        if (pl_any) {
            if (dd_unit) P.mask = mask_row(ROW_PL);
            kkt_solve<NV>(bx, bz, dx, dz, gdx, nsweep, slot, true);
        }
        P.mask = live_row;
    }
    bool two_phase(int two) const { return two < 0 ? shard_size > 1 : two != 0; }
    int dots(const double* xx2, const double* zz2, int mode, int two = -1) {
        hipLaunchKernelGGL(k_dots_r, lane_grid(dim3(std::max(nbC, 1)), nlanes), dim3(256), 0, st, P, wl, w3, dz2, zz2, partR);
        int nb = std::max(nbC, 1);
        if (P.big) {
            hipLaunchKernelGGL(k_big_dots, lane_grid(dim3(1), nlanes), dim3(1024), 0, st, P, wbb, Sc, dz2, zz2, scratch, partR);
            nb += 1;
        }
        if (two_phase(two)) {
            hipLaunchKernelGGL(k_scal_dtau, lane_grid(dim3(1), nlanes), dim3(SCAL_T), 0, st, P, Sc, dx2, xx2, partR, nb, mode, RB, 0);
            allreduce(RB, 3, 0);
            hipLaunchKernelGGL(k_scal_dtau, lane_grid(dim3(1), nlanes), dim3(SCAL_T), 0, st, P, Sc, dx2, xx2, partR, nb, mode, RB, 1);
        }
        return nb;
    }
    int dir_post(const double* xx2, const double* zz2, const double* gg2, double* outA, double* outB, int mode, int ndots, int two = -1) {
        int nb = std::max(nbC, 1);
        hipLaunchKernelGGL(k_dir_post, lane_grid(dim3(nb), nlanes), dim3(256), 0, st, P, wl, w3, lam, dz2, zz2, gdx2, gg2, rz, Sc, outA, outB,
                           partR2, mode, two_phase(two) ? nullptr : partR, ndots, xx2);
        if (P.big) {
            hipLaunchKernelGGL(k_big_dir_post, lane_grid(dim3(1), nlanes), dim3(1024), 0, st, P, wbb, lam, dz2, zz2, gdx2, gg2, rz, Sc, outA, outB,
                               scratch, partR2, mode);
            nb += 1;
        }
        return nb;
    }
    void scal_step(int mode, int nb, bool unsharded, int two = -1) {
        if (two_phase(two)) {
            hipLaunchKernelGGL(k_scal_step, lane_grid(dim3(1), nlanes), dim3(SCAL_T), 0, st, P, Sc, partR2, nb, mode, rx, bxc, RB, 0);
            allreduce(RB, 2, 1);
            hipLaunchKernelGGL(k_scal_step, lane_grid(dim3(1), nlanes), dim3(SCAL_T), 0, st, P, Sc, partR2, nb, mode, rx, bxc, RB, 1);
        } else if (unsharded) {
            hipLaunchKernelGGL(k_scal_step, lane_grid(dim3(1), nlanes), dim3(SCAL_T), 0, st, P, Sc, partR2, nb, mode, rx, bxc, RB, 2);
        }
    }
    int stage_pred_tail(bool two) {
        double *x2a = dx2 + P.LDV, *z2a = dz2 + P.Rp, *g2a = gdx2 + P.Rp;
        const int nd0 = dots(x2a, z2a, 0, two);
        const int ns0 = dir_post(x2a, z2a, g2a, dssa, wdza, 0, nd0, two);
        scal_step(0, ns0, false, two);
        return ns0;
    }
    void stage_comb_rhs(int ns0, bool two) {
        hipLaunchKernelGGL(k_comb_rhs, lane_grid(dim3(std::max(nbC, 1)), nlanes), dim3(256), 0, st, P, wl, w3, lam, dssa, wdza, rz, Sc,
                           lds, bzc, two ? nullptr : partR2, ns0, rx, bxc, dl, wbz);
        if (P.big)
            hipLaunchKernelGGL(k_big_comb_rhs, lane_grid(dim3(1), nlanes), dim3(1024), 0, st, P, wbb, lam, dssa, wdza, rz, Sc, lds, bzc, scratch);
    }
    int stage_comb_tail(bool two) {
        const int nd1 = dots(dxc, dzc, 1, two);
        return dir_post(dxc, dzc, gdxc, ds, dz, 1, nd1, two);
    }
    int unknown_blocks() const { return cdiv(std::max(P.N, P.R), 256); }
    void stage_update(int ns1, bool two) {
        scal_step(1, ns1, !sw.fuse, two);
        hipLaunchKernelGGL(k_update, lane_grid(dim3(unknown_blocks()), nlanes), dim3(256), 0, st, P, Sc, dx2, dxc, x, ds, dz, s, z,
                           (!two && sw.fuse) ? (const double*)partR2 : (const double*)nullptr, ns1);
    }
    void stage_corr_rhs(int ns1, int corr_cones, const int* corr_ddm, bool two) {
        scal_step(2, ns1, true, two);
        hipLaunchKernelGGL(k_corr_rhs, lane_grid(dim3(std::max(nbC, 1)), nlanes), dim3(256), 0, st, P, wl, dl, lam, ds, dz, Sc, kbz, wbz);
        if (P.big) hipLaunchKernelGGL(k_big_corr_rhs, lane_grid(dim3(1), nlanes), dim3(1024), 0, st, P, wbb, lam, ds, dz, Sc, kbz, scratch, corr_cones, corr_ddm);
    }
    void stage_corr_tail(bool two) {
        hipLaunchKernelGGL(k_corr_add, lane_grid(dim3(unknown_blocks()), nlanes), dim3(256), 0, st, P, dxc, dzc, gdxc, kx, kz, kg);
        const int ndC = dots(kx, kz, 3, two);
        const int nsC = dir_post(kx, kz, kg, kds, kdz, 3, ndC, two);
        scal_step(3, nsC, true, two);
        hipLaunchKernelGGL(k_update_pick, lane_grid(dim3(unknown_blocks()), nlanes), dim3(256), 0, st, P, Sc, dx2, dxc, kx, x, ds, dz, kds, kdz, s, z);
    }
    void launch_iteration(std::vector<LaneHost>& LH, const SolveOpts& o, bool head_out, int nsweep, bool use_corr) {
        if (!head_out) launch_head(LH, o);
        const bool two = two_phase(-1);
        bool dd_any = dd_k > 0, pl_any = dd_k == 0;
        if (dd_unit) {
            pl_any = false;
            for (int b = 0; b < nlanes; ++b) pl_any = pl_any || (LH[b].live && LH[b].dd_k == 0);
        }
        solve_modes<2>(dd_any, pl_any, bx2, bz2, dx2, dz2, gdx2, S_RNA, nsweep);
        const int ns0 = stage_pred_tail(two);
        stage_comb_rhs(ns0, two);
        solve_modes<1>(dd_any, pl_any, bxc, bzc, dxc, dzc, gdxc, S_RNB, nsweep);
        const int ns1 = stage_comb_tail(two);
        if (!use_corr) { stage_update(ns1, two); return; }
        const int corr_cones = (!sw.corr_big || (!dd_unit && dd_any)) ? 0 : 1;
        const int* corr_ddm = (dd_unit && dd_any) ? mask_row(ROW_DD) : nullptr;
        stage_corr_rhs(ns1, corr_cones, corr_ddm, two);
        solve_modes<1>(dd_any, pl_any, kbx, kbz, kx, kz, kg, S_RNC, 0);
        stage_corr_tail(two);
    }
    bool judge_lanes(std::vector<LaneHost>& LH, const SolveOpts& o, int it) {
        bool any_live = false, any_best = false;
        for (int b = 0; b < nlanes; ++b) hostMask[ROW_BEST * MAX_LANES + b] = 0;
        for (int b = 0; b < nlanes; ++b) {
            LaneHost& L = LH[b];
            if (!L.live) continue;
            const double* hs = hostSc + (size_t)b * S_COUNT;
            const int chol_fixes = int(hs[S_CHOLFIX]);
            if (chol_fixes >= CHOL_SYNC_LOST) throw HipError("internal error: an in-launch hand-off of the KKT factorisation timed out (device flag never raised)");
            if (o.verbose)
                fprintf(stderr, "%s%3d pcost % .10e dcost % .10e gap %.2e pres %.1e dres %.1e k/t %.1e mu %.1e a %.3f sig %.1e sweeps %d chol %d%s\n",
                        nlanes > 1 ? ("[" + std::to_string(b) + "] ").c_str() : "", it, hs[S_PCOST], hs[S_DCOST], hs[S_GAP], hs[S_PRES],
                        hs[S_DRES], hs[S_KAPPA] / hs[S_TAU], hs[S_MU], hs[S_ALPHA], hs[S_SIGMA], L.nsweep, chol_fixes,
                        L.dd_k > 0 ? [&] { char bf[200]; std::snprintf(bf, sizeof(bf), " | k %d refinement norms %.2e -> %.2e -> %.2e , %.2e -> %.2e -> %.2e", L.dd_k,
                                       hs[S_RNA], hs[S_RNA + 1], dd_passes > 2 ? hs[S_RNA + 2] : 0.0, hs[S_RNB], hs[S_RNB + 1], dd_passes > 2 ? hs[S_RNB + 2] : 0.0);
                                       return std::string(bf); }().c_str() : "");
            if (lane_verdict(L, hs, o, it)) {
                hostMask[ROW_BEST * MAX_LANES + b] = 1;
                any_best = true;
            }
            any_live = any_live || L.live;
        }
        if (any_best) {
            if (nlanes > 1) {
                MBFIR_HIP(hipMemcpyAsync(maskT + ROW_BEST * MAX_LANES, hostMask + ROW_BEST * MAX_LANES, sizeof(int) * MAX_LANES,
                                         hipMemcpyHostToDevice, st));
                P.mask = mask_row(ROW_BEST);
            }
            hipLaunchKernelGGL(k_finish_x, lane_grid(dim3(nbN), nlanes), dim3(256), 0, st, P, x, Sc, xbest);
            P.mask = mask_row(0);
        }
        return any_live;
    }
    void finish_lanes(std::vector<LaneHost>& LH, const SolveOpts& o, std::vector<std::vector<double>>& xouts, std::vector<SolveInfo>& infos,
                      double t_begin, double t_assembled) {
        P.mask = nullptr;
        hipLaunchKernelGGL(k_finish_x, lane_grid(dim3(nbN), nlanes), dim3(256), 0, st, P, x, Sc, xout);
        xouts.assign(nlanes, std::vector<double>());
        infos.assign(nlanes, SolveInfo());
        for (int b = 0; b < nlanes; ++b) {
            LaneHost& L = LH[b];
            if (L.live) L.status = ST_MAXIT;
            char* xo = reinterpret_cast<char*>(xout) + (size_t)b * lane_bytes;
            if (L.first_opt >= 0) {
                const SolveInfo last = L.info;
                L.info = L.opt_info; L.info.iters = last.iters; L.info.correctors = last.correctors; L.info.correctors_taken = last.correctors_taken;
                L.status = ST_OPTIMAL;
                MBFIR_HIP(hipMemcpyAsync(xo, reinterpret_cast<char*>(xbest) + (size_t)b * lane_bytes, sizeof(double) * P.LDV, hipMemcpyDeviceToDevice, st));
            } else if ((L.status == ST_MAXIT || L.status == ST_NUMERICAL) && L.have_best && L.best_info.pres <= INACC_FEAS &&
                L.best_info.dres <= INACC_FEAS && (L.best_info.relgap <= INACC_GAP || L.best_info.gap <= o.abstol)) {
                const int keep_it = L.info.iters;
                L.info = L.best_info; L.info.iters = keep_it;
                L.status = ST_OPTIMAL_INACCURATE;
                MBFIR_HIP(hipMemcpyAsync(xo, reinterpret_cast<char*>(xbest) + (size_t)b * lane_bytes, sizeof(double) * P.LDV, hipMemcpyDeviceToDevice, st));
            }
            const int Nb = L.Q->N();
            xouts[b].assign(Nb, 0.0);
            MBFIR_HIP(hipMemcpyAsync(xouts[b].data(), xo, sizeof(double) * Nb, hipMemcpyDeviceToHost, st));
        }
        MBFIR_HIP(hipStreamSynchronize(st));
        const double t_end = now_ms();
        double ms_gram = 0, ms_chol = 0;
        int builds = 0;
        for (size_t i = 0; i + 3 < evused; i += 4, ++builds) {
            float a = 0, b = 0;
            if (hipEventElapsedTime(&a, evpool[i], evpool[i + 1]) == hipSuccess) ms_gram += a;
            if (hipEventElapsedTime(&b, evpool[i + 2], evpool[i + 3]) == hipSuccess) ms_chol += b;
        }
        double ms_cap = 0;
        for (size_t i = 0; i + 1 < capev_used; i += 2) { float t = 0; hipEventElapsedTime(&t, capev[i], capev[i + 1]); ms_cap += t; }
        const int nw = P.quad ? 3 : 1;
        for (int b = 0; b < nlanes; ++b) {
            SolveInfo& info = infos[b];
            info = LH[b].info;
            info.status = LH[b].status;
            info.ms_assemble = t_assembled - t_begin;
            info.ms_solve = t_end - t_assembled;
            info.ms_gram = ms_gram; info.ms_chol = ms_chol; info.h_builds = builds;
            info.n_freq = LH[b].Q->Mf; info.n_rows = LH[b].Q->R; info.n_unknowns = LH[b].Q->N();
            info.lattice = P.trig;
            info.lanes = nlanes;
            info.collectives = int(n_collectives);
            info.collective_bytes = collective_bytes;
            info.gv_passes = int(n_gv); info.gtv_passes = int(n_gtv); info.pair_passes = int(n_pair);
            info.dd_iters = LH[b].dd_iters; info.dd_kmax = LH[b].dd_kmax;
            info.dd_form = cap_form ? 0 : 1; info.cap_flop = cap_flop_sum; info.ms_cap = ms_cap;
            info.chol_launches = int(chol_launch_count);
            info.chol_flop = 2.0 / 3.0 * double(P.np) * double(P.np) * double(P.np);
            info.gram_flop = P.trig ? double(3 * P.D1 - 1) * double(LH[b].Q->Mf) * (4.0 + 4.0 * nw)
                                    : double(nw) * double(P.Mf) * double(P.Nt) * double(P.Nt + 1);
        }
        nlanes_last = nlanes; taps_valid = false;
    }
};

Solver::Solver(int device) : impl(new Impl()) {
    impl->device = device;
    int ndev = 0;
    if (hipGetDeviceCount(&ndev) != hipSuccess || ndev <= 0) throw HipError("no HIP device available");
    MBFIR_HIP(hipSetDevice(device));
    {
        static std::mutex warm_mu;
        static std::vector<char> warmed;
        std::lock_guard<std::mutex> lk(warm_mu);
        if (device < 0 || device >= ndev) throw HipError("no such HIP device");
        if ((int)warmed.size() < ndev) warmed.resize(ndev, 0);
        if (!warmed[device]) { dd_warm_kernels(); chol_warm_kernels(); warmed[device] = 1; }
    }
    MBFIR_HIP(hipStreamCreate(&impl->st));
    MBFIR_HIP(hipEventCreate(&impl->ev0));
    MBFIR_HIP(hipEventCreate(&impl->ev1));
    MBFIR_HIP(hipHostMalloc(&impl->hostSc, sizeof(double) * S_COUNT * MAX_LANES));
    MBFIR_HIP(hipHostMalloc(&impl->hostFlag, sizeof(int) * 4 * MAX_LANES));
    MBFIR_HIP(hipHostMalloc(&impl->hostMask, sizeof(int) * MASK_ROWS * MAX_LANES));
    MBFIR_HIP(hipMalloc(&impl->maskT, sizeof(int) * MASK_ROWS * MAX_LANES));
    MBFIR_HIP(hipMalloc(&impl->dimsT, sizeof(LaneDims) * MAX_LANES));
    MBFIR_HIP(hipHostMalloc(&impl->hostDims, sizeof(LaneDims) * MAX_LANES));
    std::memset(impl->hostMask, 0, sizeof(int) * MASK_ROWS * MAX_LANES);
}
Solver::~Solver() {
    if (!impl) return;
    hipSetDevice(impl->device);
    comm_destroy();
    if (impl->ar.base) hipFree(impl->ar.base);
    if (impl->hostSc) hipHostFree(impl->hostSc);
    if (impl->stage) hipHostFree(impl->stage);
    if (impl->hostFlag) hipHostFree(impl->hostFlag);
    if (impl->hostMask) hipHostFree(impl->hostMask);
    if (impl->maskT) hipFree(impl->maskT);
    if (impl->dimsT) hipFree(impl->dimsT);
    if (impl->hostDims) hipHostFree(impl->hostDims);
    for (hipEvent_t e : impl->evpool) hipEventDestroy(e);
// ... 1123 lines not shown
```

Before: 330.3.

## Fuse step-size scalars into corrector kernels and trim unused moment vectors

```diff
diff --git a/multiband-rf-pulse-design_amd/csrc/solver.hip b/multiband-rf-pulse-design_amd/csrc/solver.hip
--- a/multiband-rf-pulse-design_amd/csrc/solver.hip
+++ b/multiband-rf-pulse-design_amd/csrc/solver.hip
@@ -68,7 +68,9 @@
     S_ALPHA0, S_DTAU_C, S_DKAP_C, S_PICK, S_NCORR, S_NPICK,
     S_RNA = 40 , S_RNB = 49 ,
     S_CG_RZ = 58 , S_CG_ALPHA = 60 , S_CG_BETA = 62 ,
-    S_RNC = 64 , S_SIGMAX = 76 , S_COUNT = 80
+    S_RNC = 64 ,
+    S_DTAU0 = 73 , S_DKAP0 = 74,
+    S_SIGMAX = 76 , S_COUNT = 80
 };
 constexpr double STEP = 0.99;
 constexpr double SIGMA_MAX = 0.25;
@@ -91,7 +93,9 @@
 static_assert(S_NPICK < S_RNA, "scalar slots: the auto-numbered slots run into S_RNA");
 static_assert(S_RNA + MAX_SWEEPS + 1 <= S_RNB && S_RNB + MAX_SWEEPS + 1 <= S_CG_RZ && S_RNC + MAX_SWEEPS + 1 <= S_SIGMAX,
               "scalar slots: a block of residual norms overlaps the next slot");
-static_assert(S_SIGMAX < S_COUNT, "scalar slots: S_COUNT too small");
+static_assert(S_RNC + MAX_SWEEPS + 1 <= S_DTAU0 && S_DTAU0 < S_DKAP0 && S_DKAP0 < S_SIGMAX, "scalar slots: S_DTAU0 / S_DKAP0 overlap their neighbours");
+static_assert(S_RNA < S_COUNT && S_RNB < S_COUNT && S_CG_BETA + 2 <= S_COUNT && S_RNC < S_COUNT && S_DKAP0 < S_COUNT && S_SIGMAX < S_COUNT,
+              "scalar slots: S_COUNT too small");
 constexpr int CAP_KMAX = 1024;
 constexpr int MAX_LANES = 64, MASK_ROWS = MAX_SWEEPS + 4;
 constexpr int ROW_BEST = MAX_SWEEPS + 1;
@@ -341,13 +345,16 @@
 constexpr int FPC = 16;
 __global__ __launch_bounds__(FPC * 16) void k_fold_partials(const double* __restrict__ partial, int nsplit, int nvv, int ld,
                                                         int ldo, double* __restrict__ TT, size_t lane_bytes, const int* lane_mask,
-                                                        const LaneDims* __restrict__ dims, int cgrp) {
+                                                        const LaneDims* __restrict__ dims, int cgrp, int vtrim = 1 << 30, int jtrim = 0) {
     LANES_RAW(lane_bytes, lane_mask, partial, TT);
     if (dims) nsplit = cgrp > 0 ? (dims[blockIdx.z].nchunk + cgrp - 1) / cgrp : (dims[blockIdx.z].Mown - cgrp - 1) / -cgrp;
+    if (dims && vtrim < nvv) jtrim = dims[blockIdx.z].D1;
     __shared__ double sh[16][FPC + 1];
     const int c = threadIdx.x, sg = threadIdx.y, j = blockIdx.x * FPC + c, v = blockIdx.y;
+    if (v >= vtrim && blockIdx.x * FPC >= jtrim) return;
+    const bool on = j < ld && (v < vtrim || j < jtrim);
     double t = 0;
-    if (j < ld) {
+    if (on) {
         const double* p = partial + (long)v * ld + j;
         const long ss = (long)nvv * ld;
         int s = sg;
@@ -359,7 +366,7 @@
     }
     sh[sg][c] = t;
     __syncthreads();
-    if (sg == 0 && j < ld) {
+    if (sg == 0 && on) {
         double a = 0;
 #pragma unroll
         for (int q = 0; q < 16; ++q) a += sh[q][c];
@@ -732,13 +739,12 @@
 #pragma unroll
     for (int v = 0; v < NV; ++v) out[(long)v * P.Mpad + k] = make_double2(a[v] + b[v], a[v] - b[v]);
 }
-template <int NV, bool FOLD = false>
-__global__ __launch_bounds__(256) void k_trig_moments(DProg P, const double2* __restrict__ src, const double4* __restrict__ seeds,
-                                                      int na, int nb, double* __restrict__ partial, const double* __restrict__ rows = nullptr) {
-    if (!P.seeds_shared && blockIdx.z) seeds = reinterpret_cast<const double4*>(reinterpret_cast<const char*>(seeds) + (size_t)blockIdx.z * P.lane_bytes);
-    LANES(P, src, partial, rows);
-    if (P.dims) { na = P.D1; nb = nb ? 2 * P.D1 - 1 : 0; }
-    __shared__ double2 pp[NV][CGRP][CHK];
+template <int NV>
+__device__ __forceinline__ bool trim_border(int nfull, int na) { return NV > 1 && nfull == 1 && int(blockIdx.x) * MPTS >= na; }
+template <int NV, int NVA, bool FOLD>
+__device__ __forceinline__ void trig_moments_body(const DProg& P, const double2* __restrict__ src, const double4* __restrict__ seeds, int na, int nb,
+                                                  double* __restrict__ partial, const double* __restrict__ rows, double2 (*pp)[CGRP][CHK]) {
+    static_assert(NVA == NV || !FOLD, "trig_moments_body: the trimmed form is the H-build's");
     const int tid = threadIdx.x;
     const int ch0 = blockIdx.y * P.cgrp;
     for (int e = tid; e < P.cgrp * CHK; e += 256) {
@@ -750,18 +756,18 @@
             freq_operands<NV, true>(P, rows, live ? P.fold_pos[k] : -1, a);
             freq_operands<NV, true>(P, rows, live ? P.fold_neg[k] : -1, b);
 #pragma unroll
-            for (int v = 0; v < NV; ++v) pp[v][cc][q] = make_double2(a[v] + b[v], a[v] - b[v]);
+            for (int v = 0; v < NVA; ++v) pp[v][cc][q] = make_double2(a[v] + b[v], a[v] - b[v]);
         } else {
 #pragma unroll
-        for (int v = 0; v < NV; ++v) pp[v][cc][q] = live ? src[(long)v * P.Mpad + k] : make_double2(0.0, 0.0);
+        for (int v = 0; v < NVA; ++v) pp[v][cc][q] = live ? src[(long)v * P.Mpad + k] : make_double2(0.0, 0.0);
         }
     }
     __syncthreads();
     const int m = blockIdx.x * MPTS + tid;
     if (m >= na + nb) return;
-    double ag[NV], as[NV];
-#pragma unroll
-    for (int v = 0; v < NV; ++v) ag[v] = as[v] = 0;
+    double ag[NVA], as[NVA];
+#pragma unroll
+    for (int v = 0; v < NVA; ++v) ag[v] = as[v] = 0;
     for (int cl = 0; cl < P.cgrp; cl += 2) {
         const int cha = ch0 + cl, chb = cha + 1;
         if (cha >= P.nchunk) break;
@@ -774,21 +780,34 @@
 #pragma unroll 4
         for (int q = 0; q < cnt; ++q) {
 #pragma unroll
-            for (int v = 0; v < NV; ++v) {
+            for (int v = 0; v < NVA; ++v) {
                 const double2 pa = pp[v][cl][q], pb = pp[v][clb][q];
                 ag[v] += pa.x * c0; as[v] += pa.y * s0;
                 ag[v] += pb.x * c1; as[v] += pb.y * s1;
             }
-            const double n0 = c0 * sa.z - s0 * sa.w, n1 = c1 * sb.z - s1 * sb.w;
-            s0 = s0 * sa.z + c0 * sa.w; s1 = s1 * sb.z + c1 * sb.w;
-            c0 = n0; c1 = n1;
-        }
-    }
-#pragma unroll
-    for (int v = 0; v < NV; ++v) {
+            rotate<1>(c0, s0, sa.z, sa.w);
+            rotate<1>(c1, s1, sb.z, sb.w);
+        }
+    }
+#pragma unroll
+    for (int v = 0; v < NVA; ++v) {
         partial[(((long)blockIdx.y * NV + v) * 2) * P.LDM + m] = ag[v];
         partial[(((long)blockIdx.y * NV + v) * 2 + 1) * P.LDM + m] = as[v];
     }
+}
+
+template <int NV, bool FOLD = false>
+__global__ __launch_bounds__(256) void k_trig_moments(DProg P, const double2* __restrict__ src, const double4* __restrict__ seeds,
+                                                      int na, int nb, double* __restrict__ partial, const double* __restrict__ rows = nullptr,
+                                                      int nfull = NV) {
+    if (!P.seeds_shared && blockIdx.z) seeds = reinterpret_cast<const double4*>(reinterpret_cast<const char*>(seeds) + (size_t)blockIdx.z * P.lane_bytes);
+    LANES(P, src, partial, rows);
+    if (P.dims) { na = P.D1; nb = nb ? 2 * P.D1 - 1 : 0; }
+    __shared__ double2 pp[NV][CGRP][CHK];
+    if constexpr (!FOLD && NV > 1) {
+        if (trim_border<NV>(nfull, na)) { trig_moments_body<NV, 1, FOLD>(P, src, seeds, na, nb, partial, rows, pp); return; }
+    }
+    trig_moments_body<NV, NV, FOLD>(P, src, seeds, na, nb, partial, rows, pp);
 }
 
 __device__ __forceinline__ double mul_rounded(double a, double b) {
@@ -859,9 +878,10 @@
         moment_steps16<NV, NL, I + 1>(pa, pb, ag, as, c0, s0, c1, s1, sa, sb);
     }
 }
-template <int NV, int NL, bool FOLD>
+template <int NV, int NL, bool FOLD, int NVA = NV>
 __device__ __forceinline__ void trig_moments_lanes(const DProg& P, const DProg* const (&PL)[NL], const double2* const (&src)[NL], const double4* __restrict__ seeds, int na, int nb,
                                                    double* const (&partial)[NL], const double* const (&rows)[NL], double2 (*pp)[NV][CGRP][CHK]) {
+    static_assert(NVA == NV || !FOLD, "trig_moments_lanes: the trimmed form is the H-build's");
     const int tid = threadIdx.x;
     const int ch0 = blockIdx.y * P.cgrp;
     const int m = blockIdx.x * MPTS + tid;
@@ -884,17 +904,17 @@
 #pragma unroll
             for (int L = 0; L < NL; ++L)
 #pragma unroll
-            for (int v = 0; v < NV; ++v) pp[L][v][cc][q] = live ? src[L][(long)v * P.Mpad + k] : make_double2(0.0, 0.0);
+            for (int v = 0; v < NVA; ++v) pp[L][v][cc][q] = live ? src[L][(long)v * P.Mpad + k] : make_double2(0.0, 0.0);
         }
     }
     __syncthreads();
     constexpr bool ROWB = NV <= 2;
     if ((ROWB ? m - (tid & 63) : m) >= na + nb) return;
-    double ag[NL][NV], as[NL][NV];
+    double ag[NL][NVA], as[NL][NVA];
 #pragma unroll
     for (int L = 0; L < NL; ++L)
 #pragma unroll
-    for (int v = 0; v < NV; ++v) ag[L][v] = as[L][v] = 0;
+    for (int v = 0; v < NVA; ++v) ag[L][v] = as[L][v] = 0;
     for (int cl = 0; cl < P.cgrp; cl += 2) {
         const int cha = ch0 + cl, chb = cha + 1;
         if (cha >= P.nchunk) break;
@@ -905,12 +925,12 @@
         const int clb = two ? cl + 1 : cl;
         if constexpr (ROWB) {
             for (int q0 = 0; q0 < cnt; q0 += 16) {
-                double2 pa[NL][NV], pb[NL][NV];
+                double2 pa[NL][NVA], pb[NL][NVA];
 #pragma unroll
                 for (int L = 0; L < NL; ++L)
 #pragma unroll
-                for (int v = 0; v < NV; ++v) { pa[L][v] = pp[L][v][cl][q0 + (tid & 15)]; pb[L][v] = pp[L][v][clb][q0 + (tid & 15)]; }
-                moment_steps16<NV, NL, 0>(pa, pb, ag, as, c0, s0, c1, s1, sa, sb);
+                for (int v = 0; v < NVA; ++v) { pa[L][v] = pp[L][v][cl][q0 + (tid & 15)]; pb[L][v] = pp[L][v][clb][q0 + (tid & 15)]; }
+                moment_steps16<NVA, NL, 0>(pa, pb, ag, as, c0, s0, c1, s1, sa, sb);
             }
         } else {
 #pragma unroll (NV * NL > 4 ? 2 : 4)
@@ -918,7 +938,7 @@
 #pragma unroll
             for (int L = 0; L < NL; ++L)
 #pragma unroll
-            for (int v = 0; v < NV; ++v) {
+            for (int v = 0; v < NVA; ++v) {
                 const double2 pa = pp[L][v][cl][q], pb = pp[L][v][clb][q];
                 ag[L][v] += pa.x * c0; as[L][v] += pa.y * s0;
                 ag[L][v] += pb.x * c1; as[L][v] += pb.y * s1;
@@ -933,14 +953,15 @@
 #pragma unroll
     for (int L = 0; L < NL; ++L)
 #pragma unroll
-    for (int v = 0; v < NV; ++v) {
+    for (int v = 0; v < NVA; ++v) {
         partial[L][(((long)blockIdx.y * NV + v) * 2) * P.LDM + m] = ag[L][v];
         partial[L][(((long)blockIdx.y * NV + v) * 2 + 1) * P.LDM + m] = as[L][v];
     }
 }
 template <int NV, bool FOLD = true>
 __global__ __launch_bounds__(256, 4) void k_trig_moments_pair(DProg P, const double2* __restrict__ src, const double4* __restrict__ seeds, int na, int nb,
-                                                                       double* __restrict__ partial, const double* __restrict__ rows, int nlanes) {
+                                                                       double* __restrict__ partial, const double* __restrict__ rows, int nlanes,
+                                                                       int nfull = NV) {
     static_assert(!FOLD || NV <= 2, "k_trig_moments_pair: G'v of one or two operands");
     __shared__ double2 pp[2][NV][CGRP][CHK];
     bool live[2];
@@ -955,12 +976,18 @@
         const double2* const s2[2] = {FOLD ? nullptr : byte_shift(src, off0), FOLD ? nullptr : byte_shift(src, off0 + off1)};
         double* const o2[2] = {byte_shift(partial, off0), byte_shift(partial, off0 + off1)};
         const double* const r2[2] = {FOLD ? byte_shift(rows, off0) : nullptr, FOLD ? byte_shift(rows, off0 + off1) : nullptr};
+        if constexpr (!FOLD && NV > 1) {
+            if (trim_border<NV>(nfull, na)) { trig_moments_lanes<NV, 2, FOLD, 1>(P, p2, s2, seeds, na, nb, o2, r2, pp); return; }
+        }
         trig_moments_lanes<NV, 2, FOLD>(P, p2, s2, seeds, na, nb, o2, r2, pp);
     } else {
         const DProg* const p1[1] = {&Q};
         const double2* const s1[1] = {FOLD ? nullptr : byte_shift(src, off0 + off1)};
         double* const o1[1] = {byte_shift(partial, off0 + off1)};
         const double* const r1[1] = {FOLD ? byte_shift(rows, off0 + off1) : nullptr};
+        if constexpr (!FOLD && NV > 1) {
+            if (trim_border<NV>(nfull, na)) { trig_moments_lanes<NV, 1, FOLD, 1>(P, p1, s1, seeds, na, nb, o1, r1, pp); return; }
+        }
         trig_moments_lanes<NV, 1, FOLD>(P, p1, s1, seeds, na, nb, o1, r1, pp);
     }
 }
@@ -981,6 +1008,43 @@
         a = is_max ? fmax(a, v) : a + v;
     }
     return is_max ? block_max(a, sh) : block_sum(a, sh);
+}
+template <int K>
+__device__ __forceinline__ void block_reduce_k(double (&v)[K], bool is_max, double (*sh)[17]) {
+    const int lane = threadIdx.x & 63, wv = threadIdx.x >> 6, nw = (blockDim.x + 63) >> 6;
+#pragma unroll
+    for (int k = 0; k < K; ++k) v[k] = is_max ? wave_max(v[k]) : wave_sum(v[k]);
+    __syncthreads();
+    if (lane == 0) {
+#pragma unroll
+        for (int k = 0; k < K; ++k) sh[k][wv] = v[k];
+    }
+    __syncthreads();
+    if (threadIdx.x < K) {
+        double* q = sh[threadIdx.x];
+        double t = is_max ? q[0] : 0.0 + q[0];
+        for (int i = 1; i < nw; ++i) t = is_max ? fmax(t, q[i]) : t + q[i];
+        q[16] = t;
+    }
+    __syncthreads();
+#pragma unroll
+    for (int k = 0; k < K; ++k) v[k] = sh[k][16];
+}
+template <int K>
+__device__ __forceinline__ void fold_partials_k(const double* part, int nb, int nc, int c0, bool is_max, double (&a)[K], double (*sh)[17]) {
+#pragma unroll
+    for (int k = 0; k < K; ++k) a[k] = is_max ? -1e300 : 0.0;
+    for (int b = threadIdx.x; b < nb; b += blockDim.x) {
+#pragma unroll
+        for (int k = 0; k < K; ++k) {
+            const double v = part[(long)b * nc + c0 + k];
+            a[k] = is_max ? fmax(a[k], v) : a[k] + v;
+        }
+    }
+    block_reduce_k<K>(a, is_max, sh);
+}
+__device__ __forceinline__ double step_bound(double ts, double tz, double tau, double kap, double dtau, double dkap) {
+    return fmax(0.0, fmax(fmax(ts, tz), fmax(-dtau / tau, -dkap / kap)));
 }
 
 struct BigW {
@@ -1280,25 +1344,23 @@
 __global__ __launch_bounds__(1024) void k_fold_cg_start(DProg P, double* __restrict__ Sc, const double* __restrict__ r,
                                                         const double* __restrict__ part, double* __restrict__ p, int first) {
     LANES(P, Sc, r, part, p);
-    __shared__ double zs[NV][1024];
+    __shared__ double zs[1024];
     __shared__ double sh[17];
     const int t = threadIdx.x;
-#pragma unroll
-    for (int v = 0; v < NV; ++v) {
+    const bool act = t < SCAL_T;
+    const int lane = t & 63, wv = t >> 6;
+    const int v0 = gridDim.x > 1 ? blockIdx.x : 0, v1 = gridDim.x > 1 ? blockIdx.x + 1 : NV;
+    for (int v = v0; v < v1; ++v) {
         double x[HS_PARTS];
 #pragma unroll
         for (int g = 0; g < HS_PARTS; ++g) x[g] = t < P.np ? part[((long)g * NV + v) * P.np + t] : 0.0;
         double s = 0;
 #pragma unroll
         for (int g = 0; g < HS_PARTS; ++g) s += x[g];
-        zs[v][t] = s;
-    }
-    __syncthreads();
-    const bool act = t < SCAL_T;
-    const int lane = t & 63, wv = t >> 6;
-    for (int v = 0; v < NV; ++v) {
+        zs[t] = s;
+        __syncthreads();
         double a = 0;
-        if (act) for (int j = t; j < P.N; j += SCAL_T) a += r[(long)v * P.LDV + j] * zs[v][j];
+        if (act) for (int j = t; j < P.N; j += SCAL_T) a += r[(long)v * P.LDV + j] * zs[j];
         a = wave_sum(a);
         __syncthreads();
         if (act && lane == 0) sh[wv] = a;
@@ -1310,7 +1372,7 @@
         const double beta = first ? 0.0 : (rz_old > 0 ? rz_new / rz_old : 0.0);
         if (act) for (int j = t; j < P.N; j += SCAL_T) {
             const long o = (long)v * P.LDV + j;
-            p[o] = first ? zs[v][j] : zs[v][j] + beta * p[o];
+            p[o] = first ? zs[j] : zs[j] + beta * p[o];
         }
         __syncthreads();
         if (t == 0) Sc[S_CG_RZ + v] = rz_new;
@@ -1397,23 +1459,32 @@
     }
     if (threadIdx.x == 0) Sc[slot] = m;
 }
+template <bool ADD>
 __global__ __launch_bounds__(256) void k_dots_r(DProg P, const double* __restrict__ wl, const double* __restrict__ w3,
                                                 const double* __restrict__ z1, const double* __restrict__ z2,
-                                                double* __restrict__ part) {
-    LANES(P, wl, w3, z1, z2, part);
+                                                double* __restrict__ part, const double* __restrict__ x2c,
+                                                const double* __restrict__ z2c, const double* __restrict__ g2c,
+                                                double* __restrict__ xk, double* __restrict__ zk, double* __restrict__ gk) {
+    LANES(P, wl, w3, z1, z2, part, x2c, z2c, g2c, xk, zk, gk);
     int t = blockIdx.x * blockDim.x + threadIdx.x;
     double v[3] = {0, 0, 0};
+    if (ADD) for (int j = t; j < P.N; j += gridDim.x * blockDim.x) xk[j] = x2c[j] + xk[j];
     if (t < P.l) {
-        v[0] = P.h[t] * z1[t]; v[1] = P.h[t] * z2[t];
+        double zt;
+        if (ADD) { zt = z2c[t] + zk[t]; zk[t] = zt; gk[t] = g2c[t] + gk[t]; } else zt = z2[t];
+        v[0] = P.h[t] * z1[t]; v[1] = P.h[t] * zt;
         double wz = wl[t] * z1[t];
         v[2] = wz * wz;
         if (!P.own && P.rep[t]) v[0] = v[1] = v[2] = 0.0;
     } else if (t < P.l + P.nq3) {
         int c = t - P.l, r = P.l + 3 * c;
         Soc3 W = load_w3(w3, c);
-        double zz[3] = {z1[r], z1[r + 1], z1[r + 2]}, wz[3];
+        double zz[3] = {z1[r], z1[r + 1], z1[r + 2]}, wz[3], zt[3];
+        for (int a = 0; a < 3; ++a) {
+            if (ADD) { zt[a] = z2c[r + a] + zk[r + a]; zk[r + a] = zt[a]; gk[r + a] = g2c[r + a] + gk[r + a]; } else zt[a] = z2[r + a];
+        }
         soc3_apply(W, zz, wz, false);
-        for (int a = 0; a < 3; ++a) { v[0] += P.h[r + a] * z1[r + a]; v[1] += P.h[r + a] * z2[r + a]; v[2] += wz[a] * wz[a]; }
+        for (int a = 0; a < 3; ++a) { v[0] += P.h[r + a] * z1[r + a]; v[1] += P.h[r + a] * zt[a]; v[2] += wz[a] * wz[a]; }
         if (!P.own && P.rep[r]) v[0] = v[1] = v[2] = 0.0;
     }
     block_partials<3>(v, part + (P.big ? 3 : 0), false);
@@ -1498,9 +1569,10 @@
         }
         dtau = (dkc / tau - bt + cx2 + hz2) / den;
         if (blockIdx.x == 0 && threadIdx.x == 0) {
+            const double dkap = (dkc - kap * dtau) / tau;
             Sc[mode == 0 ? S_DTAU_A : mode == 3 ? S_DTAU_C : S_DTAU] = dtau;
-            Sc[mode == 0 ? S_DKAP_A : mode == 3 ? S_DKAP_C : S_DKAP] = (dkc - kap * dtau) / tau;
-            if (mode == 1) { Sc[S_TAU0] = tau; Sc[S_KAP0] = kap; }
+            Sc[mode == 0 ? S_DKAP_A : mode == 3 ? S_DKAP_C : S_DKAP] = dkap;
+            if (mode == 1) { Sc[S_TAU0] = tau; Sc[S_KAP0] = kap; Sc[S_DTAU0] = dtau; Sc[S_DKAP0] = dkap; }
         }
     } else {
         dtau = mode == 0 ? Sc[S_DTAU_A] : mode == 3 ? Sc[S_DTAU_C] : Sc[S_DTAU];
@@ -1623,11 +1695,11 @@
     int t = blockIdx.x * blockDim.x + threadIdx.x;
     double sigma;
     if (spart) {
-        __shared__ double sh[17];
-        const double ts = fold_partials(spart, nsp, 2, 0, true, sh);
-        const double tz = fold_partials(spart, nsp, 2, 1, true, sh);
+        __shared__ double sh[2][17];
+        double tm[2];
+        fold_partials_k<2>(spart, nsp, 2, 0, true, tm, sh);
         const double tau = Sc[S_TAU], kap = Sc[S_KAPPA];
-        const double tt = fmax(0.0, fmax(fmax(ts, tz), fmax(-Sc[S_DTAU_A] / tau, -Sc[S_DKAP_A] / kap)));
+        const double tt = step_bound(tm[0], tm[1], tau, kap, Sc[S_DTAU_A], Sc[S_DKAP_A]);
         const double a = tt == 0.0 ? 1.0 : fmin(1.0, 1.0 / tt);
         sigma = fmin((1 - a) * (1 - a) * (1 - a), Sc[S_SIGMAX]);
         if (blockIdx.x == 0) {
@@ -1714,12 +1786,35 @@
     if (t < P.N) x[t] += a * (x2[t] + dtau * x1[t]);
     if (t < P.R) { s[t] += a * ds[t]; z[t] += a * dz[t]; }
 }
-__global__ __launch_bounds__(256) void k_update_pick(DProg P, const double* __restrict__ Sc, const double* __restrict__ x1,
+__global__ __launch_bounds__(256) void k_update_pick(DProg P, double* __restrict__ Sc, const double* __restrict__ x1,
                          const double* __restrict__ x2, const double* __restrict__ x2k, double* __restrict__ x,
                          const double* __restrict__ ds, const double* __restrict__ dz, const double* __restrict__ dsk,
-                         const double* __restrict__ dzk, double* __restrict__ s, double* __restrict__ z) {
-    LANES(P, Sc, x1, x2, x2k, x, ds, dz, dsk, dzk, s, z);
+                         const double* __restrict__ dzk, double* __restrict__ s, double* __restrict__ z,
+                         const double* __restrict__ part, int nb) {
+    LANES(P, Sc, x1, x2, x2k, x, ds, dz, dsk, dzk, s, z, part);
     int t = blockIdx.x * blockDim.x + threadIdx.x;
+    if (part) {
+        __shared__ double sh[2][17];
+        double tm[2];
+        fold_partials_k<2>(part, nb, 2, 0, true, tm, sh);
+        const double tau = Sc[S_TAU0], kap = Sc[S_KAP0], dtauc = Sc[S_DTAU_C], dkapc = Sc[S_DKAP_C];
+        const double tt = step_bound(tm[0], tm[1], tau, kap, dtauc, dkapc);
+        const double ac = tt == 0.0 ? 1.0 : fmin(1.0, STEP / tt);
+        const double a0 = Sc[S_ALPHA0];
+        const double tolk = fmax(REFTOL * Sc[S_NRMC], CORR_ETA * Sc[S_DRES] * tau * Sc[S_NRMC]);
+        double pickd = (ac >= CORR_ACCEPT * a0 && Sc[S_RNC] <= tolk) ? 1.0 : 0.0;
+        asm volatile("" : "+v"(pickd));
+        const bool pick = pickd != 0.0;
+        const double a = pick ? ac : a0, dtau = pick ? dtauc : Sc[S_DTAU0], dkap = pick ? dkapc : Sc[S_DKAP0];
+        if (blockIdx.x == 0 && threadIdx.x == 0) {
+            Sc[S_TMAX] = tt; Sc[S_PICK] = pickd; Sc[S_NCORR] += 1.0;
+            if (pick) { Sc[S_DTAU] = dtau; Sc[S_DKAP] = dkap; Sc[S_NPICK] += pickd; }
+            Sc[S_ALPHA] = a; Sc[S_TAU] = tau + a * dtau; Sc[S_KAPPA] = kap + a * dkap;
+        }
+        if (t < P.N) x[t] += a * ((pick ? x2k[t] : x2[t]) + dtau * x1[t]);
+        if (t < P.R) { s[t] += a * (pick ? dsk[t] : ds[t]); z[t] += a * (pick ? dzk[t] : dz[t]); }
+        return;
+    }
     const double a = Sc[S_ALPHA], dtau = Sc[S_DTAU];
     const bool pick = Sc[S_PICK] != 0.0;
     if (t < P.N) x[t] += a * ((pick ? x2k[t] : x2[t]) + dtau * x1[t]);
@@ -1731,12 +1826,24 @@
 }
 __global__ __launch_bounds__(256) void k_corr_rhs(DProg P, const double* __restrict__ wl, const double* __restrict__ dl,
                                                   const double* __restrict__ lam, const double* __restrict__ ds,
-                                                  const double* __restrict__ dz, const double* __restrict__ Sc,
-                                                  double* __restrict__ bz, double* __restrict__ wbz) {
-    LANES(P, wl, dl, lam, ds, dz, Sc, bz, wbz);
+                                                  const double* __restrict__ dz, double* __restrict__ Sc,
+                                                  double* __restrict__ bz, double* __restrict__ wbz,
+                                                  const double* __restrict__ part, int nb) {
+    LANES(P, wl, dl, lam, ds, dz, Sc, bz, wbz, part);
     int t = blockIdx.x * blockDim.x + threadIdx.x;
+    double alpha0;
+    if (part) {
+        __shared__ double sh[2][17];
+        double tm[2];
+        fold_partials_k<2>(part, nb, 2, 0, true, tm, sh);
+        const double tt = step_bound(tm[0], tm[1], Sc[S_TAU], Sc[S_KAPPA], Sc[S_DTAU], Sc[S_DKAP]);
+        alpha0 = tt == 0.0 ? 1.0 : fmin(1.0, STEP / tt);
+        if (blockIdx.x == 0 && threadIdx.x == 0) { Sc[S_TMAX] = tt; Sc[S_ALPHA0] = alpha0; }
+    } else {
+        alpha0 = Sc[S_ALPHA0];
+    }
     if (t < P.l) {
-        const double at = fmin(1.0, Sc[S_ALPHA0] + CORR_DELTA), mut = Sc[S_SIGMA] * Sc[S_MU];
+        const double at = fmin(1.0, alpha0 + CORR_DELTA), mut = Sc[S_SIGMA] * Sc[S_MU];
         const double l = lam[t], w = wl[t];
         const double dss = ds[t] / w, wdz = w * dz[t];
         const double v = (l + at * dss) * (l + at * wdz);
@@ -2602,7 +2709,8 @@
         apply_G<NV>(v, gout);
         winv2<NV>(gout, sub, wout, 0);
     }
-    void moments_array(int nv, const double* pp, const double4* seeds, int na, int nb, double* out) {
+    void moments_array(int nv, const double* pp, const double4* seeds, int na, int nb, double* out, int nfull = 0) {
+        if (nfull <= 0) nfull = nv;
         dim3 g(cdiv(na + nb, MPTS), cdiv(P.nchunk, P.cgrp)), b(256), gf(cdiv(P.nfold, 256));
         const bool pair = lane_pairs();
         if (pair) ++n_pair;
@@ -2610,14 +2718,15 @@
 #define MOM_CASE(NVX)                                                                                                          \
             case NVX:                                                                                                          \
                 if (pp) hipLaunchKernelGGL((k_freq_fold<NVX, false>), lane_grid(gf, nlanes), b, 0, st, P, pp, PPf);            \
-                if (pair) hipLaunchKernelGGL((k_trig_moments_pair<NVX, false>), lane_grid(g, cdiv(nlanes, 2)), b, 0, st, P, PPf, seeds, na, nb, partial, (const double*)nullptr, nlanes); \
-                else hipLaunchKernelGGL((k_trig_moments<NVX>), lane_grid(g, nlanes), b, 0, st, P, PPf, seeds, na, nb, partial); \
+                if (pair) hipLaunchKernelGGL((k_trig_moments_pair<NVX, false>), lane_grid(g, cdiv(nlanes, 2)), b, 0, st, P, PPf, seeds, na, nb, partial, (const double*)nullptr, nlanes, nfull); \
+                else hipLaunchKernelGGL((k_trig_moments<NVX>), lane_grid(g, nlanes), b, 0, st, P, PPf, seeds, na, nb, partial, (const double*)nullptr, nfull); \
                 break;
             MOM_CASE(1) MOM_CASE(2) MOM_CASE(3) MOM_CASE(4) MOM_CASE(6)
 #undef MOM_CASE
             default: throw HipError("moments: unsupported vector count");
         }
-        hipLaunchKernelGGL(k_fold_partials, lane_grid(dim3(cdiv(P.LDM, FPC), 2 * nv), nlanes), dim3(FPC, 16), 0, st, partial, cdiv(P.nchunk, P.cgrp), 2 * nv, P.LDM, P.LDM, out, lane_bytes, P.mask, P.dims, P.cgrp);
+        hipLaunchKernelGGL(k_fold_partials, lane_grid(dim3(cdiv(P.LDM, FPC), 2 * nv), nlanes), dim3(FPC, 16), 0, st, partial, cdiv(P.nchunk, P.cgrp), 2 * nv, P.LDM, P.LDM, out, lane_bytes, P.mask, P.dims, P.cgrp,
+                           nfull < nv ? 2 * nfull : 1 << 30, na);
     }
     void atmulti_array(int nvv, const double* pp) {
         dim3 g(P.ld / 128, nsplit_at), b(64, 4);
@@ -2703,7 +2812,7 @@
         auto z_and_start = [&](int first) {
             if (sw.fuse && fused_hsolve) {
                 hsolve_launch(M, P.np, r, nullptr, tmpN2, partial, NV, P.LDV, st, nlanes, lane_bytes, P.mask, false);
-                hipLaunchKernelGGL(k_fold_cg_start<NV>, g1, dim3(1024), 0, st, P, Sc, r, partial, pN, first);
+                hipLaunchKernelGGL(k_fold_cg_start<NV>, lane_grid(dim3(shard_size <= 1 ? NV : 1), nlanes), dim3(1024), 0, st, P, Sc, r, partial, pN, first);
             } else {
                 hsolve<NV>(r, tmpN2);
                 hipLaunchKernelGGL(k_cg_start<NV>, g1, dim3(SCAL_T), 0, st, P, Sc, r, tmpN2, pN, first);
@@ -2870,7 +2979,7 @@
             const double* momb = MomB;
             if (one_pass) {
                 hipLaunchKernelGGL(k_freq_blocks_fold, lane_grid(dim3(cdiv(P.nfold, 256)), nlanes), dim3(256), 0, st, P, dlw, w3, m3c, nwv + nvb, PPf);
-                moments_array(nwv + nvb, nullptr, P.seed_h, P.D1, 2 * P.D1 - 1, Mom);
+                moments_array(nwv + nvb, nullptr, P.seed_h, P.D1, 2 * P.D1 - 1, Mom, (sw.fuse && shard_size <= 1) ? nwv : 0);
                 momb = Mom + 2L * nwv * P.LDM;
             } else {
                 moments_array(nwv, Dw, P.seed_h, P.D1, 2 * P.D1 - 1, Mom);
@@ -3351,8 +3460,13 @@
         P.mask = live_row;
     }
     bool two_phase(int two) const { return two < 0 ? shard_size > 1 : two != 0; }
-    int dots(const double* xx2, const double* zz2, int mode, int two = -1) {
-        hipLaunchKernelGGL(k_dots_r, lane_grid(dim3(std::max(nbC, 1)), nlanes), dim3(256), 0, st, P, wl, w3, dz2, zz2, partR);
+    int dots(const double* xx2, const double* zz2, int mode, int two = -1, bool add_corr = false) {
+        const double* none = nullptr;
+        if (add_corr)
+            hipLaunchKernelGGL(k_dots_r<true>, lane_grid(dim3(std::max(nbC, 1)), nlanes), dim3(256), 0, st, P, wl, w3, dz2, none, partR, dxc, dzc, gdxc, kx, kz, kg);
+        else
+            hipLaunchKernelGGL(k_dots_r<false>, lane_grid(dim3(std::max(nbC, 1)), nlanes), dim3(256), 0, st, P, wl, w3, dz2, zz2, partR, none, none, none,
+                               (double*)nullptr, (double*)nullptr, (double*)nullptr);
         int nb = std::max(nbC, 1);
         if (P.big) {
             hipLaunchKernelGGL(k_big_dots, lane_grid(dim3(1), nlanes), dim3(1024), 0, st, P, wbb, Sc, dz2, zz2, scratch, partR);
@@ -3409,16 +3523,21 @@
                            (!two && sw.fuse) ? (const double*)partR2 : (const double*)nullptr, ns1);
     }
     void stage_corr_rhs(int ns1, int corr_cones, const int* corr_ddm, bool two) {
-        scal_step(2, ns1, true, two);
-        hipLaunchKernelGGL(k_corr_rhs, lane_grid(dim3(std::max(nbC, 1)), nlanes), dim3(256), 0, st, P, wl, dl, lam, ds, dz, Sc, kbz, wbz);
+        const bool fused = sw.fuse && !two;
+        if (!fused) scal_step(2, ns1, true, two);
+        hipLaunchKernelGGL(k_corr_rhs, lane_grid(dim3(std::max(nbC, 1)), nlanes), dim3(256), 0, st, P, wl, dl, lam, ds, dz, Sc, kbz, wbz,
+                           fused ? (const double*)partR2 : (const double*)nullptr, ns1);
         if (P.big) hipLaunchKernelGGL(k_big_corr_rhs, lane_grid(dim3(1), nlanes), dim3(1024), 0, st, P, wbb, lam, ds, dz, Sc, kbz, scratch, corr_cones, corr_ddm);
     }
     void stage_corr_tail(bool two) {
-        hipLaunchKernelGGL(k_corr_add, lane_grid(dim3(unknown_blocks()), nlanes), dim3(256), 0, st, P, dxc, dzc, gdxc, kx, kz, kg);
-        const int ndC = dots(kx, kz, 3, two);
+        const bool fused = sw.fuse && !two;
+        const bool add_in_dots = fused && !P.big;
+        if (!add_in_dots) hipLaunchKernelGGL(k_corr_add, lane_grid(dim3(unknown_blocks()), nlanes), dim3(256), 0, st, P, dxc, dzc, gdxc, kx, kz, kg);
+        const int ndC = dots(kx, kz, 3, two, add_in_dots);
         const int nsC = dir_post(kx, kz, kg, kds, kdz, 3, ndC, two);
-        scal_step(3, nsC, true, two);
-        hipLaunchKernelGGL(k_update_pick, lane_grid(dim3(unknown_blocks()), nlanes), dim3(256), 0, st, P, Sc, dx2, dxc, kx, x, ds, dz, kds, kdz, s, z);
+        if (!fused) scal_step(3, nsC, true, two);
+        hipLaunchKernelGGL(k_update_pick, lane_grid(dim3(unknown_blocks()), nlanes), dim3(256), 0, st, P, Sc, dx2, dxc, kx, x, ds, dz, kds, kdz, s, z,
+                           fused ? (const double*)partR2 : (const double*)nullptr, nsC);
     }
     void launch_iteration(std::vector<LaneHost>& LH, const SolveOpts& o, bool head_out, int nsweep, bool use_corr) {
         if (!head_out) launch_head(LH, o);
```

Result: faster. 334.7 (median of 6 runs) (+1.3%).
